# QingzhiWang/LIS-SLAM

Hardware: AMD Instinct MI355X
Metric: scan-to-submap registrations/sec (64x1800 pts, 200k submap) (higher is better)
Workload: dtype f32; 1 GPU; configs[1]: batch=64 synthetic 64x1800 scans vs one shared 200k-pt submap per GPU, semantic mask off, 10 fixed GN iterations, target index build inside the step; batch_per_gpu=64, submap_points=200000, gn_iters=10, parallelism=independent batches x1 + RCCL all-gather of results

## Files before the change

include/lisreg.h:

```cpp
#ifndef LISREG_H_
#define LISREG_H_

#include <stdint.h>

#ifdef __cplusplus
extern "C" {
#endif

#define LISREG_VERSION 1

#define LISREG_OK                        0
#define LISREG_NOT_ENOUGH_FEATURES       1
#define LISREG_TOO_FEW_CORRESPONDENCES   2
#define LISREG_LEAF_TOO_SMALL            3
#define LISREG_ERR_ARG                  -1
#define LISREG_ERR_HIP                  -2
#define LISREG_ERR_NO_TARGET            -3
#define LISREG_ERR_NOMEM                -4
#define LISREG_ERR_COMM                 -5

#define LISREG_FMT_XYZI    0
#define LISREG_FMT_XYZIL   1
#define LISREG_FMT_DEVICE  2
#define LISREG_FMT_DEVICE_XYZI 4
// ... 62 lines not shown
int  lisreg_create(int device, lisreg_ctx** out);
void lisreg_destroy(lisreg_ctx* ctx);
const char* lisreg_last_error(const lisreg_ctx* ctx);
int  lisreg_set_stream(lisreg_ctx* ctx, void* hip_stream);
void* lisreg_get_stream(const lisreg_ctx* ctx);

int  lisreg_default_params(int variant, lisreg_params* p);

int  lisreg_set_target(lisreg_ctx* ctx, const void* corner, int n_corner,
                       const void* surf, int n_surf, int stride_bytes, int fmt);
int  lisreg_set_target_slot(lisreg_ctx* ctx, int slot, const void* corner, int n_corner,
                            const void* surf, int n_surf, int stride_bytes, int fmt);
int  lisreg_target_from_classes(lisreg_ctx* ctx, int slot,
                                const void* pole, int n_pole, const void* ground, int n_ground,
                                const void* building, int n_building, const void* dynamic, int n_dynamic,
                                int stride_bytes, int fmt);

int  lisreg_align(lisreg_ctx* ctx,
                  const void* src_corner, int n_corner, const void* src_surf, int n_surf,
                  int stride_bytes, int fmt,
                  const lisreg_params* params, const lisreg_imu* imu ,
                  float T[6], lisreg_stats* stats );

int  lisreg_align_batch(lisreg_ctx* ctx, int n_items, const lisreg_item* items,
                        const lisreg_params* params, float* T, lisreg_stats* stats);

int  lisreg_batch_prepare(lisreg_ctx* ctx, int n_items, const lisreg_item* items,
                          const lisreg_params* params, const float* T_init);
int  lisreg_batch_run(lisreg_ctx* ctx);
int  lisreg_batch_fetch(lisreg_ctx* ctx, float* T, lisreg_stats* stats);
int  lisreg_stage_host_items(lisreg_ctx* ctx, int n_items, const lisreg_item* items, lisreg_item* items_out);

void* lisreg_batch_result_device(const lisreg_ctx* ctx);

int  lisreg_set_option(lisreg_ctx* ctx, const char* name, int value);
int  lisreg_get_option(const lisreg_ctx* ctx, const char* name, int* value);

int  lisreg_get_counters(lisreg_ctx* ctx, unsigned long long* out, int n);

int  lisreg_get_neighbors(lisreg_ctx* ctx, int* out, int n_elems);

int  lisreg_test_fit_models(lisreg_ctx* ctx, int kind, int n, const float* neighbours, const float* queries,
                            const lisreg_params* params, int exact, float* out);

int  lisreg_get_target_index(lisreg_ctx* ctx, int slot, int kind, int* dims, float* geom,
                             float* sorted_out, int sorted_capacity, int* cell_start_out, int cell_capacity);

int  lisreg_get_target_graph(lisreg_ctx* ctx, int slot, int kind, int* k, float* rows_out, float* meta_out, int capacity_points);

int  lisreg_get_target_cell_rows(lisreg_ctx* ctx, int slot, int kind, int* n_rows, int* k, int* table_out, int capacity_cells,
                                 float* rows_out, float* meta_out, int capacity_rows);

int  lisreg_get_trace(lisreg_ctx* ctx, float* buf, int max_iters);

int  lisreg_set_profiling(lisreg_ctx* ctx, int enable);
int  lisreg_get_timing(lisreg_ctx* ctx, double out[5]);

int  lisreg_voxel_downsample(lisreg_ctx* ctx, const void* in, int n, int stride_bytes, int fmt, float leaf,
                             void* out, int out_capacity, int* n_out);
int  lisreg_voxel_downsample_multi(lisreg_ctx* ctx, int k, const void* const* in, const int* n, const float* leaf, int fmt,
                                   void* const* out, const int* out_capacity, int* n_out);
int  lisreg_transform_cloud(lisreg_ctx* ctx, const void* in, int n, int stride_bytes, int fmt, const float T[6], void* out);

#define LISREG_FMT_XYZIRT  3
typedef struct lisreg_feature_params {
    int   n_scan;
    int   horizon_scan;
    int   downsample_rate;
    float min_range;
    float max_range;
    float edge_threshold;
    float surf_threshold;
} lisreg_feature_params;
typedef struct lisreg_feature_out {
    void* deskewed;      int cap_deskewed,      n_deskewed;
    void* corner;        int cap_corner,        n_corner;
    void* surface;       int cap_surface,       n_surface;
    void* corner_sharp;  int cap_corner_sharp,  n_corner_sharp;
    void* surface_sharp; int cap_surface_sharp, n_surface_sharp;
} lisreg_feature_out;
int  lisreg_extract_features(lisreg_ctx* ctx, const void* cloud, int n, int stride_bytes, int fmt,
                             const lisreg_feature_params* params, lisreg_feature_out* out);
int  lisreg_default_feature_params(lisreg_feature_params* p);
typedef struct lisreg_deskew {
    int    enabled;
    int    imu_pointer_cur;
    const double* imu_time;
    const double* imu_rot_x;
    const double* imu_rot_y;
    const double* imu_rot_z;
    double time_scan_cur;
    const float* time_device;
} lisreg_deskew;
int  lisreg_extract_features_deskew(lisreg_ctx* ctx, const void* cloud, int n, int stride_bytes, int fmt,
                                    const lisreg_feature_params* params, const lisreg_deskew* deskew, lisreg_feature_out* out);

int  lisreg_extract_features_batch(lisreg_ctx* ctx, int n_sweeps, const void* const* sweeps, const int* n,
                                   const lisreg_feature_params* params, lisreg_feature_out* outs);

#define LISREG_FMT_XYZI_PACKED 5
typedef struct lisreg_pretreat_params {
    int    n_scan;
    float  min_range;
    float  max_range;
    double scan_period;
} lisreg_pretreat_params;
// ... 267 lines not shown
```

lis-slam_amd/csrc/lisreg_api.hip:

```cpp
#include "lisreg_ctx.hpp"

#include <dlfcn.h>

#include <algorithm>
#include <chrono>
#include <cmath>
#include <cstdio>
#include <cstdlib>
#include <cstring>
#include <string>
#include <vector>

using namespace lisreg;

namespace lisreg {
thread_local std::string g_static_err;
int ctx_fail(lisreg_ctx* c, int code, const std::string& msg)
{
    if (c) c->err = msg; else g_static_err = msg;
    return code;
}

bool ensure_side_stream(lisreg_ctx* c)
{
// ... 453 lines not shown
        if (n > 0 && !(bb[0] <= bb[3] && bb[1] <= bb[4] && bb[2] <= bb[5]))
            return fail(c, LISREG_ERR_ARG, "set_target: the cloud has no finite point (every coordinate is NaN)");
        memcpy(t.bbox[k], bb, sizeof bb);
        t.grid_margin[k] = (c->search_mode == 5 || (c->search_mode == 4 && t.crow_chosen[k])) ? kCrowGridMargin : 0;
        make_grid(bb, n, &t.g[k], &t.n_cells[k], t.grid_margin[k]);
        prof_mark(c, 2);
        int rc = build_target_kind(c, t, k);
        t.graph_valid[k] = false;
        t.crow_valid[k] = false; t.crow_too_big[k] = false;
        t.g[k].crow = nullptr; t.g[k].crow_meta = nullptr; t.g[k].crow_tab = nullptr;
        if (!rc && c->search_mode == 3) rc = ensure_graph(c, t, k, true);
        if (!rc && c->search_mode == 5) rc = ensure_crows(c, t, k);
        prof_mark(c, -1);
        if (rc) return rc;
    }
    t.valid = true;
    c->grids_dirty = true;
    c->prepared = false;
    return LISREG_OK;
}

int lisreg_set_target_slot(lisreg_ctx* c, int slot, const void* corner, int n_corner, const void* surf, int n_surf,
                           int stride, int fmt)
{
    const void* clouds[2] = { corner, surf };
    const int counts[2] = { n_corner, n_surf };
    return set_target_impl(c, slot, clouds, counts, stride, fmt);
}

int lisreg_set_target(lisreg_ctx* c, const void* corner, int n_corner, const void* surf, int n_surf, int stride, int fmt)
{
    return lisreg_set_target_slot(c, 0, corner, n_corner, surf, n_surf, stride, fmt);
}

int lisreg_target_from_classes(lisreg_ctx* c, int slot, const void* pole, int n_pole, const void* ground, int n_ground,
                               const void* building, int n_building, const void* dynamic, int n_dynamic,
                               int stride, int fmt)
{
    if (!c) return LISREG_ERR_ARG;
    if (fmt == LISREG_FMT_DEVICE) return fail(c, LISREG_ERR_ARG, "target_from_classes: host clouds only");
    if (stride < 12) return fail(c, LISREG_ERR_ARG, "target_from_classes: stride < 12");
    const void* parts[3] = { ground, building, dynamic };
    const int cnt[3] = { std::max(n_ground, 0), std::max(n_building, 0), std::max(n_dynamic, 0) };
    std::vector<unsigned char> surf((size_t)(cnt[0] + cnt[1] + cnt[2]) * (size_t)stride + 1);
    size_t off = 0;
    for (int i = 0; i < 3; ++i) if (cnt[i] > 0 && parts[i]) {
        memcpy(surf.data() + off, parts[i], (size_t)cnt[i] * (size_t)stride);
        off += (size_t)cnt[i] * (size_t)stride;
    }
    return lisreg_set_target_slot(c, slot, pole, pole ? std::max(n_pole, 0) : 0, surf.data(), (int)(off / (size_t)stride), stride, fmt);
}

static bool xcd_order_wanted(const lisreg_ctx* c);

int lisreg_batch_prepare(lisreg_ctx* c, int n_items, const lisreg_item* items, const lisreg_params* params,
                         const float* T_init)
{
    if (!c) return LISREG_ERR_ARG;
    if (n_items < 0 || (n_items > 0 && (!items || !T_init)) || !params) return fail(c, LISREG_ERR_ARG, "batch_prepare: bad arguments");
    HIPCHK(c, hipSetDevice(c->device));
    c->prepared = false;
    c->params = *params;
    c->prm = make_dev_params(*params);
    c->prm.exact = c->exact ? 1 : 0;
    c->prm.ties = (c->canonical_ties || c->exact) ? 1 : 0;
    c->n_items = n_items;
    c->h_blocks.clear(); c->h_segs.clear(); c->h_items.assign((size_t)n_items, ItemState());
    c->batch_slots.clear();
    {
        long long total_src = 0;
        double t_pts = 0;
        std::vector<int> seen;
        for (int i = 0; i < n_items; ++i) {
            total_src += (long long)std::max(items[i].n_corner, 0) + (long long)std::max(items[i].n_surf, 0);
            const int sl = items[i].target;
            if (sl >= 0 && (size_t)sl < c->targets.size() && std::find(seen.begin(), seen.end(), sl) == seen.end()) {
                seen.push_back(sl);
                t_pts += (double)c->targets[(size_t)sl].n[0] + (double)c->targets[(size_t)sl].n[1];
            }
        }
        if (total_src > 2000000000LL) return fail(c, LISREG_ERR_ARG, "batch_prepare: more than 2e9 source points in one batch");
        c->mode_now = c->search_mode;
        if (c->search_mode == 4) {
            const double qi = (double)total_src * (double)c->prm.bound;
            c->mode_now = (t_pts > 0 && qi >= (double)c->graph_min_ratio * t_pts) ? 3 : 1;
            if (t_pts > 0 && qi >= (double)c->cell_min_ratio * t_pts && t_pts * 5120.0 <= (double)c->cell_rows_max_mb * 1048576.0) c->mode_now = 5;
        }
        c->lanes_q = (c->mode_now == 1 && c->lanes_per_query_auto && total_src > 0 && total_src <= 131072) ? 8 : 1;
        if (c->mode_now == 5) {
            bool declined = false;
            long long rows_left = (long long)std::max(c->cell_rows_max_mb, 1) * 1048576LL / (long long)(sizeof(float4) * kGraphK + sizeof(float2));
            for (int sl : seen)
                for (int k = 0; k < 2 && !declined; ++k) {
                    Target& t = c->targets[(size_t)sl];
                    if (!t.valid) continue;
                    const bool had = t.crow_valid[k] && t.g[k].crow_tab;
                    int rc = ensure_crows(c, t, k, c->search_mode == 4, c->search_mode == 4 ? &rows_left : nullptr);
                    if (rc) return rc;
                    if (!had) c->grids_dirty = true;
                    declined = c->search_mode == 4 && t.crow_too_big[k];
                }
            if (declined) {
                c->mode_now = 3;
                for (int sl : seen)
                    for (int k = 0; k < 2; ++k) {
                        Target& t = c->targets[(size_t)sl];
// ... 180 lines not shown
            off += (pt.bytes + 63) & ~(size_t)63;
        }
        HIPCHK(c, hipEventRecord(c->stage_done, c->stream));
    }
    c->sort_now = c->sort_sources == 1;
    if (c->sort_sources == 2 && c->n_elems >= 65536 && c->probe_items == n_items && c->probe_elems == c->n_elems && c->probe_age < 32) {
        ++c->probe_age;
        c->sort_now = c->probe_verdict;
    } else
    if (c->sort_sources == 2 && c->n_elems >= 65536) {
        launch_count_jumps(c->blocks.as<BlockDesc>(), c->n_blocks, c->segs.as<Segment>(), 1.5f, c->done_dev.as<int>(), c->stream);
        int jumps_stack = 0;
        int* jumps = c->done_host.p ? c->done_host.as<int>() : &jumps_stack;
        HIPCHK(c, hipMemcpyAsync(jumps, c->done_dev.p, sizeof(int), hipMemcpyDeviceToHost, c->stream));
        HIPCHK(c, hipStreamSynchronize(c->stream));
        c->sort_now = (double)*jumps > 0.25 * (double)c->n_elems;
        c->probe_verdict = c->sort_now; c->probe_items = n_items; c->probe_elems = c->n_elems; c->probe_age = 0;
    }
    {
        const size_t se = (size_t)std::max(c->rebuild_targets_each_run ? tflat : 1, c->sort_now ? flat : 1);
        const size_t sbk = (size_t)std::max(c->rebuild_targets_each_run ? c->t_buckets : 1, c->sort_now ? c->n_buckets : 1);
        rc = ensure_sort_scratch(c, se, sbk);
        if (rc) return rc;
    }
    launch_reset_items(c->items.as<ItemState>(), c->n_items, c->prm, c->done_dev.as<int>(), c->stream,
                       reinterpret_cast<int*>(c->results.as<float>() + (size_t)std::max(c->n_items, 1) * kResultSize));
    c->items_reset = true; c->reach_miss_seen = 0; c->runs_since_fetch = 0;
    c->reach_ready = false;
    if (c->reach_backoff > 0) --c->reach_backoff;
    else if (c->mode_now == 5 && c->rebuild_targets_each_run && c->row_reach != 0 && c->lanes_q == 1 && c->n_blocks > 0) {
        bool any = false;
        for (int slot : c->batch_slots) for (int k = 0; k < 2; ++k) any = any || (c->targets[(size_t)slot].g[k].qmark != nullptr && c->targets[(size_t)slot].n[k] > 0);
        if (any) {
            launch_query_marks(c->blocks.as<BlockDesc>(), c->n_blocks, c->segs.as<Segment>(), c->grids_dev.as<GridIndex>(), c->items.as<ItemState>(), c->stream);
            for (int slot : c->batch_slots)
                for (int k = 0; k < 2; ++k) {
                    Target& t = c->targets[(size_t)slot];
                    if (!t.g[k].qmark || t.n[k] <= 0) continue;
                    launch_reach_dilate(t.g[k], t.crow_reach[k].as<unsigned>(), c->stream);
                    HIPCHK(c, hipMemsetAsync(t.g[k].qmark, 0, sizeof(unsigned) * (size_t)t.g[k].nx * (size_t)t.g[k].ny * (size_t)t.g[k].qmark_w, c->stream));
                }
            HIPCHK(c, hipGetLastError());
            c->reach_ready = true;
        }
    }
    c->xcd_cached = false;
    if (xcd_order_wanted(c) && !c->sort_now && !c->exact && c->n_blocks > 0) {
        HIPCHK(c, c->xcd_tab.ensure(sizeof(int) * 2 * (size_t)c->n_blocks));
        launch_xcd_order(c->blocks.as<BlockDesc>(), c->n_blocks, c->segs.as<Segment>(), c->grids_dev.as<GridIndex>(), c->items.as<ItemState>(),
                         nullptr, c->batch_slots.size() >= 8 && c->xcd_order == 1, c->xcd_tab.as<int>(), c->xcd_tab.as<int>() + c->n_blocks, c->stream);
        HIPCHK(c, hipGetLastError());
        c->xcd_cached = true;
    }
    c->prepared = true;
    return LISREG_OK;
}

static int exact_pose_caches(lisreg_ctx* c)
{
    const size_t n = (size_t)c->n_items;
    if (n == 0) return LISREG_OK;
    HIPCHK(c, c->exact_trig.ensure(sizeof(float) * 6 * n));
    std::vector<float> T(6 * n), trig(6 * n);
    launch_pose_gather(c->items.as<ItemState>(), c->n_items, c->exact_trig.as<float>(), c->stream);
    HIPCHK(c, hipMemcpyAsync(T.data(), c->exact_trig.p, sizeof(float) * 6 * n, hipMemcpyDeviceToHost, c->stream));
    HIPCHK(c, hipStreamSynchronize(c->stream));
    for (size_t i = 0; i < n; ++i) {
        const float* t = &T[6 * i];
        float* g = &trig[6 * i];
        g[0] = cosf(t[2]); g[1] = sinf(t[2]); g[2] = cosf(t[1]); g[3] = sinf(t[1]); g[4] = cosf(t[0]); g[5] = sinf(t[0]);
    }
    HIPCHK(c, hipMemcpyAsync(c->exact_trig.p, trig.data(), sizeof(float) * 6 * n, hipMemcpyHostToDevice, c->stream));
    launch_pose_cache_from_trig(c->items.as<ItemState>(), c->n_items, c->exact_trig.as<float>(), c->stream);
    HIPCHK(c, hipStreamSynchronize(c->stream));
    return LISREG_OK;
}

constexpr int kWideFrom = 0, kWideFromSmall = 1, kWideUntil = 2, kGraphWideUntil = 1;
constexpr int kGraphHops = 3;

static bool xcd_order_wanted(const lisreg_ctx* c)
{
    const bool many_targets = c->batch_slots.size() >= 8 && c->xcd_order == 1;
    return c->lanes_q != 8 &&
           (((c->mode_now == 3 || c->mode_now == 5) && (c->xcd_order == 1 || (c->xcd_order == 2 && c->n_blocks >= 2048 && c->n_items >= 32))) ||
            (many_targets && c->xcd_order != 0 && c->n_blocks >= 2048));
}

static int run_impl(lisreg_ctx* c, bool early_stop)
{
    if (!c->prepared) return fail(c, LISREG_ERR_ARG, "batch_run: no prepared batch");
    HIPCHK(c, hipSetDevice(c->device));
    hipStream_t st = c->stream;
    const bool many_targets = c->batch_slots.size() >= 8 && c->xcd_order == 1;
    c->xcd_now = xcd_order_wanted(c);
    if (c->xcd_now) HIPCHK(c, c->xcd_tab.ensure(sizeof(int) * 2 * (size_t)c->n_blocks));
    const bool can_stop = early_stop && c->prm.fixed_iters <= 0 && c->done_host.p && c->early_stop_chunk != 0;
    int split_item = 0, split_blk = 0;
    if (c->interleave != 0 && !c->exact && !can_stop && c->lanes_q == 1 && c->n_items >= 2 && c->n_blocks >= c->interleave_min_blocks) {
        ensure_side_stream(c);
        if (c->side_stream && !c->ev_ab && (c->ev_ab.create(hipEventDisableTiming) != hipSuccess ||
                                            c->ev_ba.create(hipEventDisableTiming) != hipSuccess)) { c->ev_ab.reset(); c->ev_ba.reset(); }
        if (c->side_stream) {
            for (int i = 1; i < c->n_items; ++i)
                if (c->h_items[(size_t)i].blk_begin * 2 >= c->n_blocks) { split_item = i; split_blk = c->h_items[(size_t)i].blk_begin; break; }
            if (split_blk * 4 < c->n_blocks || (c->n_blocks - split_blk) * 4 < c->n_blocks) { split_item = 0; split_blk = 0; }
        }
    }
    c->reach_now = c->rebuild_targets_each_run && c->mode_now == 5 && c->reach_ready && !c->exact;
    int* const miss_dev = reinterpret_cast<int*>(c->results.as<float>() + (size_t)std::max(c->n_items, 1) * kResultSize);
    c->prm.reach_miss = c->reach_now ? miss_dev : nullptr;
    const bool reset_done = c->items_reset;
    c->items_reset = false;
    if (c->rebuild_targets_each_run) {
        prof_mark(c, 2);
        if (c->strip_now) {
            StripBuffers sl;
            sl.cnt = c->strip_tab.as<int>(); sl.fill = sl.cnt + (c->t_strips + 1); sl.start = sl.fill + (c->t_strips + 1);
            sl.scan_tmp = sl.start + (c->t_strips + 2);
            sl.tmp_pts = c->tmp_pts.as<float4>(); sl.slot_idx = c->elem_bucket.as<uint32_t>(); sl.slot_pos = c->elem_sub.as<uint32_t>();
            ensure_side_stream(c);
            sl.side = c->side_stream; sl.ev_fork = c->ev_fork; sl.ev_join = c->ev_join;
            if (launch_build_targets_strips(c->tchunk_dev.as<BlockDesc>(), (int)c->h_tchunks.size(), c->tseg_dev.as<TargetSeg>(),
                                            (int)c->h_tsegs.size(), c->t_strips, c->t_max_units, c->t_max_ucells, c->strip_cap, sl, st, &c->strip_zero_ints))
                return fail(c, LISREG_ERR_HIP, "strip index build: LDS configuration refused");
        } else
            launch_build_targets_batched(c->tblk_dev.as<BlockDesc>(), (int)c->h_tblocks.size(), c->tseg_dev.as<TargetSeg>(),
                                         (int)c->h_tsegs.size(), c->t_elems, c->t_buckets, sort_buffers(c), st);
        if (c->mode_now == 3)
            launch_build_graph(c->tblk_dev.as<BlockDesc>(), (int)c->h_tblocks.size(), c->tseg_dev.as<TargetSeg>(),
                               c->grids_dev.as<GridIndex>(), st);
        if (c->mode_now == 5) {
            for (int slot : c->batch_slots) {
                Target& t = c->targets[(size_t)slot];
                const GridIndex g2[2] = { t.g[0], t.g[1] };
                const int nc2[2] = { t.n_cells[0], t.n_cells[1] };
                const lisreg::CrowBuffers cb2[2] = { crow_buffers(t, 0, c->reach_now), crow_buffers(t, 1, c->reach_now) };
                int* oz2[2] = { &t.omask_zero[0], &t.omask_zero[1] };
                launch_crow_rows_pair(g2, nc2, cb2, st, oz2);
            }
        }
        prof_mark(c, -1);
    }
    if (!reset_done) launch_reset_items(c->items.as<ItemState>(), c->n_items, c->prm, c->done_dev.as<int>(), st);
    if (c->exact) { int rc = exact_pose_caches(c); if (rc) return rc; }
    prof_mark(c, 2);
    launch_sort_sources(c->blocks.as<BlockDesc>(), c->n_blocks, c->segs.as<Segment>(), c->n_segs, c->items.as<ItemState>(),
                        c->n_elems, c->sort_now ? c->n_buckets : 0, sort_buffers(c), c->sorted_all.as<float4>(), c->order_all.as<int>(), st);
    prof_mark(c, -1);
    if (c->xcd_now && !(c->xcd_cached && split_blk == 0)) {
        const int nb0 = split_blk ? split_blk : c->n_blocks;
        launch_xcd_order(c->blocks.as<BlockDesc>(), nb0, c->segs.as<Segment>(), c->grids_dev.as<GridIndex>(), c->items.as<ItemState>(),
                         c->sort_now ? c->sorted_all.as<float4>() : nullptr, many_targets, c->xcd_tab.as<int>(), c->xcd_tab.as<int>() + c->n_blocks, st);
        if (split_blk) {
            launch_xcd_order(c->blocks.as<BlockDesc>() + split_blk, c->n_blocks - split_blk, c->segs.as<Segment>(), c->grids_dev.as<GridIndex>(),
                             c->items.as<ItemState>(), c->sort_now ? c->sorted_all.as<float4>() : nullptr, many_targets,
                             c->xcd_tab.as<int>() + split_blk, c->xcd_tab.as<int>() + c->n_blocks + split_blk, st);
            c->xcd_cached = false;
        }
    }
    const int chunk = c->early_stop_chunk > 0 ? c->early_stop_chunk : (c->n_blocks <= 1024 ? 6 : 3);
    int next_check = chunk;
    if (c->early_stop_chunk <= 0 && c->last_launches > 0) next_check = std::max(2, std::min(c->last_launches, chunk));
    c->prm.cell_anchor_until = c->cell_anchor_until;
    auto iteration = [&](int it, int i0, int ni, int b0, int nb, hipStream_t s_, int sidx, hipEvent_t after_assoc) {
        if (!after_assoc) prof_mark(c, 0, sidx);
        (c->exact ? launch_assoc_exact : launch_assoc)(
                     c->blocks.as<BlockDesc>() + b0, nb, c->segs.as<Segment>(), c->grids_dev.as<GridIndex>(),
                     c->items.as<ItemState>(), c->prm, c->sort_now ? c->sorted_all.as<float4>() : nullptr, c->partials.as<double>() + (size_t)b0 * kNumAcc,
                     c->mode_now, c->nn.as<int>(), c->n_elems, c->first_pass_r * c->first_pass_r,
                     c->mode_now != 5 && it >= (c->lanes_q == 8 ? kWideFromSmall : kWideFrom) && it <= (c->mode_now == 3 ? kGraphWideUntil : kWideUntil), kGraphHops,
                     c->count_searches ? c->counters.as<unsigned long long>() : nullptr,
                     c->dump_neighbors ? c->dbg_nn.as<int>() : nullptr, c->lanes_q,
                     c->blocks_q.as<BlockDesc>(), (int)c->h_blocks_q.size(), c->coef.as<float4>(), c->coef_ok.as<int>(),
                     c->xcd_now ? c->xcd_tab.as<int>() + c->n_blocks + b0 : nullptr, s_);
        if (after_assoc) (void)hipEventRecord(after_assoc, s_);
        prof_mark(c, 1, sidx);
        launch_solve(c->items.as<ItemState>() + i0, ni, c->prm, c->partials.as<double>(),
                     c->trace_cap > 0 ? c->trace.as<float>() + (size_t)i0 * (size_t)c->trace_cap * kTraceStride : nullptr, c->trace_cap, c->done_dev.as<int>(), s_);
        prof_mark(c, -1, sidx);
    };
    c->interleaved_now = false;
    if (split_blk > 0 && hipEventRecord(c->ev_fork, st) == hipSuccess && hipStreamWaitEvent(c->side_stream, c->ev_fork, 0) == hipSuccess) {
        c->interleaved_now = true;
        const bool alternate = c->interleave == 1 && c->ev_ab && c->ev_ba;
        hipError_t ie = hipSuccess;
        for (int it = 0; it < c->prm.bound && ie == hipSuccess; ++it) {
            if (alternate && it > 0) ie = hipStreamWaitEvent(st, c->ev_ba, 0);
            if (ie != hipSuccess) break;
            if (alternate) prof_mark(c, 0, 0);
            iteration(it, 0, split_item, 0, split_blk, st, 0, alternate ? c->ev_ab : nullptr);
            if (alternate) ie = hipStreamWaitEvent(c->side_stream, c->ev_ab, 0);
            if (ie != hipSuccess) break;
            if (alternate) prof_mark(c, 0, 1);
            iteration(it, split_item, c->n_items - split_item, split_blk, c->n_blocks - split_blk, c->side_stream, 1, alternate ? c->ev_ba : nullptr);
        }
        if (ie == hipSuccess) ie = hipEventRecord(c->ev_join, c->side_stream);
        if (ie == hipSuccess) ie = hipStreamWaitEvent(st, c->ev_join, 0);
        if (ie != hipSuccess) {
            (void)hipStreamSynchronize(c->side_stream);
            c->interleaved_now = false;
            return lisreg::ctx_fail(c, LISREG_ERR_HIP, std::string("interleaved run: ") + hipGetErrorString(ie));
        }
    } else
    for (int it = 0; it < c->prm.bound; ++it) {
        iteration(it, 0, c->n_items, 0, c->n_blocks, st, 0, nullptr);
        if (c->exact && it + 1 < c->prm.bound) { int rc = exact_pose_caches(c); if (rc) return rc; }
        if (can_stop && it + 1 == next_check && it + 1 < c->prm.bound) {
            HIPCHK(c, hipMemcpyAsync(c->done_host.p, c->done_dev.p, sizeof(int), hipMemcpyDeviceToHost, st));
            HIPCHK(c, hipStreamSynchronize(st));
            if (*c->done_host.as<int>() >= c->n_items) break;
            next_check += c->early_stop_chunk > 0 ? chunk : std::min(chunk, 3);
        }
    }
    launch_finalize(c->items.as<ItemState>(), c->n_items, c->prm, c->results.as<float>(), st, c->done_dev.as<int>());
    c->items_reset = true; ++c->runs_since_fetch;
    HIPCHK(c, hipGetLastError());
    if (c->pack_in_use >= 0 && c->pack_free[c->pack_in_use])
        HIPCHK(c, hipEventRecord(c->pack_free[c->pack_in_use], st));
    return LISREG_OK;
}

int lisreg_batch_run(lisreg_ctx* c)
{
    if (!c) return LISREG_ERR_ARG;
    return run_impl(c, false);
}

int lisreg_batch_fetch(lisreg_ctx* c, float* T, lisreg_stats* stats)
{
    if (!c) return LISREG_ERR_ARG;
    if (!c->prepared) return fail(c, LISREG_ERR_ARG, "batch_fetch: no prepared batch");
    HIPCHK(c, hipSetDevice(c->device));
    const size_t res_floats = ((size_t)std::max(c->n_items, 1) + 1) * kResultSize;
    const size_t trace_floats = c->fetch_trace_records > 0 ? (size_t)kTraceStride * (size_t)c->fetch_trace_records : 0;
    const size_t fetch_bytes = (res_floats + trace_floats) * sizeof(float);
    HIPCHK(c, c->fetch_host.ensure(fetch_bytes, fetch_bytes * 2 + 4096));
    float* fetched = c->fetch_host.as<float>();
    const bool with_miss = c->n_items > 0 && c->reach_now;
    if (c->n_items) HIPCHK(c, hipMemcpyAsync(fetched, c->results.p, sizeof(float) * kResultSize * ((size_t)c->n_items + (with_miss ? 1 : 0)), hipMemcpyDeviceToHost, c->stream));
    if (trace_floats && c->trace.p) HIPCHK(c, hipMemcpyAsync(fetched + res_floats, c->trace.p, sizeof(float) * trace_floats, hipMemcpyDeviceToHost, c->stream));
    HIPCHK(c, hipStreamSynchronize(c->stream));
    c->h_results.assign(fetched, fetched + res_floats);
    if (with_miss) {
        int cum; memcpy(&cum, fetched + (size_t)c->n_items * kResultSize, sizeof cum);
        const int miss = cum - c->reach_miss_seen;
        c->reach_miss_seen = cum;
        c->reach_miss_last = miss;
        if ((long long)miss * 1000LL > (long long)c->n_elems * (long long)std::max(c->prm.bound, 1) * (long long)std::max(c->runs_since_fetch, 1)) { c->reach_ready = false; c->reach_backoff = 32; }
    }
    if (!c->ev.empty()) prof_collect(c);
    c->last_launches = 0;
    for (int i = 0; i < c->n_items; ++i) {
        const float* r = &c->h_results[(size_t)i * kResultSize];
        c->last_launches = std::max(c->last_launches, (int)r[6] + 1);
        if (T) memcpy(T + 6 * (size_t)i, r, 24);
        if (stats) {
            stats[i].iters = (int)r[6]; stats[i].deltaR = r[7]; stats[i].deltaT = r[8];
            stats[i].degenerate = (int)r[9]; stats[i].n_corr_last = (int)r[10]; stats[i].status = (int)r[11];
        }
    }
    c->runs_since_fetch = 0;
    return LISREG_OK;
}

void* lisreg_batch_result_device(const lisreg_ctx* c) { return c ? c->results.p : nullptr; }

int lisreg_set_option(lisreg_ctx* c, const char* name, int value)
{
    if (!c || !name) return LISREG_ERR_ARG;
    if (!strcmp(name, "rebuild_targets_each_run")) {
        c->rebuild_targets_each_run = value != 0;
        if (c->prepared && c->rebuild_targets_each_run) {
            int rc = ensure_sort_scratch(c, (size_t)std::max(c->t_elems, 1), (size_t)std::max(c->t_buckets, 1));
            if (rc) return rc;
        }
        return LISREG_OK;
    }
    if (!strcmp(name, "sort_sources")) { c->sort_sources = value; c->probe_items = -1; return LISREG_OK; }
    if (!strcmp(name, "cell_anchor_until")) { c->cell_anchor_until = std::max(value, 0); return LISREG_OK; }
    if (!strcmp(name, "search_mode")) {
        if (value < 1 || value > 5 || value == 2) return fail(c, LISREG_ERR_ARG, "search_mode: 1 cell walk, 3 k-NN graph scan, 4 auto, 5 cell rows");
        c->search_mode = value; c->prepared = false; return LISREG_OK;
    }
    if (!strcmp(name, "graph_min_ratio")) { c->graph_min_ratio = value; c->prepared = false; return LISREG_OK; }
    if (!strcmp(name, "cell_min_ratio")) { c->cell_min_ratio = value; c->prepared = false; return LISREG_OK; }
    if (!strcmp(name, "row_reach")) { c->row_reach = value; c->reach_backoff = 0; c->prepared = false; return LISREG_OK; }
    if (!strcmp(name, "cell_rows_max_mb")) {
        c->cell_rows_max_mb = value; c->prepared = false;
        for (auto& t : c->targets) for (int k = 0; k < 2; ++k) {
            t.crow_too_big[k] = false;
            if (t.crow_valid[k]) { t.crow_valid[k] = false; c->grids_dirty = true; }
        }
        return LISREG_OK;
    }
    if (!strcmp(name, "early_stop_chunk")) { c->early_stop_chunk = value; return LISREG_OK; }
    if (!strcmp(name, "xcd_order")) { if (value < 0 || value > 2) return fail(c, LISREG_ERR_ARG, "xcd_order: 0 off, 1 on, 2 auto"); c->xcd_order = value; c->xcd_cached = false; return LISREG_OK; }
    if (!strcmp(name, "index_build")) {
        if (value < 0 || value > 2) return fail(c, LISREG_ERR_ARG, "index_build: 0 bucket sort, 1 strip form, 2 auto");
        c->index_build = value; c->prepared = false;
        return LISREG_OK;
    }
    if (!strcmp(name, "index_strip_cells")) { c->strip_cells = std::max(value, 0); c->prepared = false; return LISREG_OK; }
    if (!strcmp(name, "index_strip_cap")) { c->strip_cap = std::min(std::max(value, 64), 16384); c->prepared = false; return LISREG_OK; }
    if (!strcmp(name, "count_searches")) {
        c->count_searches = value != 0;
        if (c->count_searches) { HIPCHK(c, c->counters.ensure(128 * 8)); HIPCHK(c, hipMemset(c->counters.p, 0, 128 * 8)); }
        return LISREG_OK;
    }
    if (!strcmp(name, "lanes_per_query")) { c->lanes_per_query_auto = value != 1; c->prepared = false; return LISREG_OK; }
    if (!strcmp(name, "dump_neighbors")) { c->dump_neighbors = value != 0; c->prepared = false; return LISREG_OK; }
    if (!strcmp(name, "exact_arithmetic")) { c->exact = value != 0; c->prepared = false; return LISREG_OK; }
    if (!strcmp(name, "feeder_copy_engine")) { c->feeder_engine = value; return LISREG_OK; }
    if (!strcmp(name, "canonical_ties")) { c->canonical_ties = value != 0; c->prepared = false; return LISREG_OK; }
    if (!strcmp(name, "first_pass_mm")) {
        if (value < 0) return fail(c, LISREG_ERR_ARG, "first_pass_mm: a radius in millimetres, >= 0");
        c->first_pass_r = 1e-3f * (float)value; return LISREG_OK;
    }
    if (!strcmp(name, "trace_cap")) { c->trace_cap = std::max(0, value); c->prepared = false; return LISREG_OK; }
    if (!strcmp(name, "feeder_threads")) { c->feeder_threads = std::min(std::max(value, 0), 64); return LISREG_OK; }
    if (!strcmp(name, "feeder_numa")) { c->feeder_numa = value != 0; return LISREG_OK; }
    if (!strcmp(name, "interleave_min_blocks")) { c->interleave_min_blocks = std::max(value, 2); return LISREG_OK; }
    if (!strcmp(name, "interleave")) { if (value < 0 || value > 2) return fail(c, LISREG_ERR_ARG, "interleave: 0 off, 1 alternating halves, 2 free-running halves"); c->interleave = value; return LISREG_OK; }
    return fail(c, LISREG_ERR_ARG, std::string("set_option: unknown option ") + name);
}

int lisreg_get_option(const lisreg_ctx* c, const char* name, int* value)
{
    if (!c || !name || !value) return LISREG_ERR_ARG;
    if (!strcmp(name, "search_mode")) { *value = c->search_mode; return LISREG_OK; }
    if (!strcmp(name, "exact_arithmetic")) { *value = c->exact ? 1 : 0; return LISREG_OK; }
    if (!strcmp(name, "feeder_chunks_by_copy_engine")) { *value = c->pack_stolen; return LISREG_OK; }
    if (!strcmp(name, "feeder_chunks")) { *value = c->pack_chunks_n; return LISREG_OK; }
    if (!strcmp(name, "canonical_ties")) { *value = (c->canonical_ties || c->exact) ? 1 : 0; return LISREG_OK; }
    if (!strcmp(name, "index_build")) { *value = c->index_build; return LISREG_OK; }
    if (!strcmp(name, "index_build_now")) { *value = c->strip_now ? 1 : 0; return LISREG_OK; }
    if (!strcmp(name, "front_end")) { *value = c->mode_now; return LISREG_OK; }
    if (!strcmp(name, "lanes_per_query")) { *value = c->lanes_q; return LISREG_OK; }
    if (!strcmp(name, "sort_sources")) { *value = c->sort_sources; return LISREG_OK; }
    if (!strcmp(name, "cell_anchor_until")) { *value = c->cell_anchor_until; return LISREG_OK; }
    if (!strcmp(name, "feeder_threads")) { *value = c->feeder_threads; return LISREG_OK; }
    if (!strcmp(name, "feeder_numa_node")) { *value = c->feeder_node; return LISREG_OK; }
    if (!strcmp(name, "feeder_numa_cpus")) { *value = c->feeder_cpus; return LISREG_OK; }
    if (!strcmp(name, "comm_nranks")) { *value = c->comm ? c->comm_nranks : 0; return LISREG_OK; }
    if (!strcmp(name, "sorted_now")) { *value = c->sort_now ? 1 : 0; return LISREG_OK; }
    if (!strcmp(name, "rebuild_targets_each_run")) { *value = c->rebuild_targets_each_run ? 1 : 0; return LISREG_OK; }
    if (!strcmp(name, "graph_min_ratio")) { *value = c->graph_min_ratio; return LISREG_OK; }
    if (!strcmp(name, "cell_min_ratio")) { *value = c->cell_min_ratio; return LISREG_OK; }
    if (!strcmp(name, "row_reach")) { *value = c->row_reach; return LISREG_OK; }
    if (!strcmp(name, "row_reach_now")) { *value = c->reach_now ? 1 : 0; return LISREG_OK; }
    if (!strcmp(name, "row_reach_misses")) { *value = c->reach_miss_last; return LISREG_OK; }
    if (!strcmp(name, "cell_rows_max_mb")) { *value = c->cell_rows_max_mb; return LISREG_OK; }
    if (!strcmp(name, "xcd_order")) { *value = c->xcd_order; return LISREG_OK; }
    if (!strcmp(name, "xcd_order_now")) { *value = c->xcd_now ? 1 : 0; return LISREG_OK; }
    if (!strcmp(name, "interleave")) { *value = c->interleave; return LISREG_OK; }
    if (!strcmp(name, "interleaved_now")) { *value = c->interleaved_now ? 1 : 0; return LISREG_OK; }
    if (!strcmp(name, "index_kib_front_end_built")) {
        if (c->mode_now != 5) return lisreg_get_option(c, "index_kib_front_end", value);
        unsigned long long fe = 0;
        for (int slot : c->batch_slots) {
            if (slot < 0 || (size_t)slot >= c->targets.size()) continue;
            const lisreg::Target& t = c->targets[(size_t)slot];
            for (int k = 0; k < 2; ++k) {
                if (t.n[k] <= 0 || !t.crow_scan[k].p) continue;
                int rows = 0;
                if (hipSetDevice(c->device) != hipSuccess || hipStreamSynchronize(c->stream) != hipSuccess ||
                    hipMemcpy(&rows, t.crow_scan[k].as<int>() + t.n_cells[k], sizeof(int), hipMemcpyDeviceToHost) != hipSuccess) return LISREG_ERR_HIP;
                rows = std::min(std::max(rows, 0), t.crow_cap[k]);
                fe += (unsigned long long)rows * (sizeof(float4) * lisreg::kGraphK + sizeof(float2)) + (unsigned long long)t.n_cells[k] * sizeof(int);
            }
        }
        *value = (int)std::min<unsigned long long>((fe + 1023) / 1024, 0x7fffffffULL);
        return LISREG_OK;
    }
    if (!strcmp(name, "index_kib_grid") || !strcmp(name, "index_kib_front_end") || !strcmp(name, "index_target_points")) {
        unsigned long long grid = 0, fe = 0, pts = 0;
        for (int slot : c->batch_slots) {
            if (slot < 0 || (size_t)slot >= c->targets.size()) continue;
            const lisreg::Target& t = c->targets[(size_t)slot];
            for (int k = 0; k < 2; ++k) {
                if (t.n[k] <= 0) continue;
                pts += (unsigned long long)t.n[k];
                grid += (unsigned long long)t.n[k] * sizeof(float4) + ((unsigned long long)t.n_cells[k] + 1) * sizeof(int);
                if (c->mode_now == 3) fe += (unsigned long long)t.n[k] * (sizeof(float4) * lisreg::kGraphK + sizeof(float2));
                if (c->mode_now == 5) fe += (unsigned long long)t.crow_cap[k] * (sizeof(float4) * lisreg::kGraphK + sizeof(float2)) +
                                            (unsigned long long)t.n_cells[k] * sizeof(int);
            }
        }
        const unsigned long long v = !strcmp(name, "index_target_points") ? pts : ((!strcmp(name, "index_kib_grid") ? grid : fe) + 1023) / 1024;
        *value = (int)std::min<unsigned long long>(v, 0x7fffffffULL);
        return LISREG_OK;
    }
    return LISREG_ERR_ARG;
}

int lisreg_align_batch(lisreg_ctx* c, int n_items, const lisreg_item* items, const lisreg_params* params, float* T,
                       lisreg_stats* stats)
{
    if (!c) return LISREG_ERR_ARG;
    if (n_items < 0 || (n_items > 0 && (!items || !T)) || !params) return fail(c, LISREG_ERR_ARG, "align_batch: bad arguments");
    const auto t_in = std::chrono::steady_clock::now();
    HIPCHK(c, hipSetDevice(c->device));
    size_t total = 0;
    for (int i = 0; i < n_items; ++i) {
        const lisreg_item& in = items[i];
        if (in.n_corner < 0 || in.n_surf < 0) return fail(c, LISREG_ERR_ARG, "align_batch: negative count");
        if (in.fmt != LISREG_FMT_DEVICE) {
            if (in.stride_bytes < 12 || (in.fmt == LISREG_FMT_XYZIL && in.stride_bytes < 22)) return fail(c, LISREG_ERR_ARG, "align_batch: bad stride");
            if ((in.n_corner > 0 && !in.src_corner) || (in.n_surf > 0 && !in.src_surf)) return fail(c, LISREG_ERR_ARG, "align_batch: NULL cloud");
            total += (size_t)in.n_corner + (size_t)in.n_surf;
        }
    }
    std::vector<lisreg_item> dev_items((size_t)n_items);
    if (total >= 262144 && c->feeder_threads > 0) {
        int rc = lisreg_stage_host_items(c, n_items, items, dev_items.data());
        if (rc) return rc;
        rc = lisreg_batch_prepare(c, n_items, dev_items.data(), params, T);
        if (rc) { (void)hipStreamSynchronize(c->stream); return rc; }
        rc = run_impl(c, true);
        if (rc) { (void)hipStreamSynchronize(c->stream); return rc; }
        return lisreg_batch_fetch(c, T, stats);
    }
    HIPCHK(c, c->src_upload.ensure(sizeof(lisreg_dpoint) * std::max<size_t>(total, 1)));
    size_t raw_bytes = 0;
    for (int i = 0; i < n_items; ++i)
        if (items[i].fmt != LISREG_FMT_DEVICE) raw_bytes += ((size_t)items[i].n_corner + (size_t)items[i].n_surf) * (size_t)items[i].stride_bytes + 32;
    HIPCHK(c, c->raw_upload.ensure(std::max<size_t>(raw_bytes, 16)));
    size_t off = 0, roff = 0;
    for (int i = 0; i < n_items; ++i) {
        dev_items[(size_t)i] = items[i];
        const lisreg_item& in = items[i];
        if (in.fmt == LISREG_FMT_DEVICE) continue;
        lisreg_item& d = dev_items[(size_t)i];
        const void* srcs[2] = { in.src_corner, in.src_surf };
        const int cnts[2] = { in.n_corner, in.n_surf };
        const void** dsts[2] = { &d.src_corner, &d.src_surf };
        for (int k = 0; k < 2; ++k) {
            lisreg_dpoint* dst = c->src_upload.as<lisreg_dpoint>() + off;
            *dsts[k] = dst;
            if (cnts[k] > 0) {
                unsigned char* rdst = static_cast<unsigned char*>(c->raw_upload.p) + roff;
                const size_t bytes = (size_t)cnts[k] * (size_t)in.stride_bytes;
                HIPCHK(c, hipMemcpyAsync(rdst, srcs[k], bytes, hipMemcpyHostToDevice, c->stream));
                launch_pack_cloud(rdst, (size_t)cnts[k], in.stride_bytes, in.fmt == LISREG_FMT_XYZIL, reinterpret_cast<float4*>(dst), c->stream);
                roff += (bytes + 15) & ~(size_t)15;
// ... 13 lines not shown
    if (rc) { (void)hipStreamSynchronize(c->stream); return rc; }
    const auto t2 = now();
    rc = lisreg_batch_fetch(c, T, stats);
    if (host_prof) {
        auto us = [](auto a, auto b) { return std::chrono::duration<double, std::micro>(b - a).count(); };
        fprintf(stderr, "[lisreg host] upload %.1f us, prepare %.1f us, enqueue %.1f us, fetch (incl. GPU wait) %.1f us\n",
                us(t_in, t0), us(t0, t1), us(t1, t2), us(t2, now()));
    }
    return rc;
}

int lisreg_align(lisreg_ctx* c, const void* src_corner, int n_corner, const void* src_surf, int n_surf, int stride,
                 int fmt, const lisreg_params* params, const lisreg_imu* imu, float T[6], lisreg_stats* stats)
{
    if (!c) return LISREG_ERR_ARG;
    if (!params || !T) return fail(c, LISREG_ERR_ARG, "align: params/T NULL");
    if (c->targets.empty() || !c->targets[0].valid) return fail(c, LISREG_ERR_NO_TARGET, "align: call lisreg_set_target first");
    lisreg_item item;
    memset(&item, 0, sizeof item);
    item.src_corner = src_corner; item.n_corner = n_corner;
    item.src_surf = src_surf; item.n_surf = n_surf;
    item.stride_bytes = stride; item.fmt = fmt; item.target = 0;
    item.degenerate_in = c->degenerate;
    if (imu) item.imu = *imu;
    const int bound = params->fixed_iters > 0 ? params->fixed_iters : params->max_iters;
    const int saved_cap = c->trace_cap;
    c->trace_cap = std::max(bound, 1);
    lisreg_stats st;
    memset(&st, 0, sizeof st);
    c->fetch_trace_records = c->trace_cap;
    int rc = lisreg_align_batch(c, 1, &item, params, T, &st);
    c->fetch_trace_records = 0;
    if (rc == LISREG_OK) {
        c->degenerate = st.degenerate;
        c->last_trace_n = std::min(bound, st.iters + 1);
        if (st.status == LISREG_NOT_ENOUGH_FEATURES) c->last_trace_n = 0;
        c->last_trace.assign((size_t)kTraceStride * (size_t)std::max(c->last_trace_n, 1), 0.f);
        if (c->last_trace_n > 0 && c->fetch_host.p)
            memcpy(c->last_trace.data(), c->fetch_host.as<float>() + 2 * (size_t)kResultSize, sizeof(float) * kTraceStride * (size_t)c->last_trace_n);
        if (stats) *stats = st;
        rc = st.status;
    }
    c->trace_cap = saved_cap;
    c->prepared = false;
    return rc;
}

int lisreg_get_trace(lisreg_ctx* c, float* buf, int max_iters)
{
    if (!c || !buf || max_iters <= 0) return 0;
    const int n = std::min(max_iters, c->last_trace_n);
    if (n > 0) memcpy(buf, c->last_trace.data(), sizeof(float) * kTraceStride * (size_t)n);
    return n;
}

int lisreg_get_counters(lisreg_ctx* c, unsigned long long* out, int n)
{
    if (!c || !out || n < 0) return LISREG_ERR_ARG;
    for (int i = 0; i < n; ++i) out[i] = 0;
    if (!c->counters.p) return LISREG_OK;
    HIPCHK(c, hipStreamSynchronize(c->stream));
    HIPCHK(c, hipMemcpy(out, c->counters.p, sizeof(unsigned long long) * (size_t)std::min(n, 128), hipMemcpyDeviceToHost));
    if (c->mode_now == 3 || c->mode_now == 5) {
        unsigned long long tmp[64] = { 0 };
        for (int i = 0; i < 32 && 2 * i + 1 < n; ++i) { tmp[2 * i] = out[i] >> 32; tmp[2 * i + 1] = out[i] & 0xffffffffull; }
        for (int i = 0; i < std::min(n, 64); ++i) out[i] = tmp[i];
    }
    return LISREG_OK;
}

int lisreg_get_target_index(lisreg_ctx* c, int slot, int kind, int* dims , float* geom ,
                            float* sorted_out, int sorted_capacity, int* cell_start_out, int cell_capacity)
{
    if (!c || slot < 0 || (size_t)slot >= c->targets.size() || kind < 0 || kind > 1 || !c->targets[(size_t)slot].valid)
        return fail(c, LISREG_ERR_ARG, "get_target_index: no such target");
    const Target& t = c->targets[(size_t)slot];
    const GridIndex& g = t.g[kind];
    if (dims) { dims[0] = t.n[kind]; dims[1] = g.nx; dims[2] = g.ny; dims[3] = g.nz; dims[4] = t.n_cells[kind]; }
    if (geom) { geom[0] = g.ox; geom[1] = g.oy; geom[2] = g.oz; geom[3] = g.cell; }
    HIPCHK(c, hipStreamSynchronize(c->stream));
    if (sorted_out) {
        if (sorted_capacity < t.n[kind]) return fail(c, LISREG_ERR_ARG, "get_target_index: sorted_capacity too small");
        if (t.n[kind] > 0) HIPCHK(c, hipMemcpy(sorted_out, t.sorted[kind].p, sizeof(float4) * (size_t)t.n[kind], hipMemcpyDeviceToHost));
    }
    if (cell_start_out) {
        if (cell_capacity < t.n_cells[kind] + 1) return fail(c, LISREG_ERR_ARG, "get_target_index: cell_capacity too small");
        HIPCHK(c, hipMemcpy(cell_start_out, t.cell_start[kind].p, sizeof(int) * ((size_t)t.n_cells[kind] + 1), hipMemcpyDeviceToHost));
    }
    return LISREG_OK;
}

int lisreg_get_target_graph(lisreg_ctx* c, int slot, int kind, int* k_out, float* rows_out, float* meta_out, int capacity_points)
{
    if (!c || slot < 0 || (size_t)slot >= c->targets.size() || kind < 0 || kind > 1 || !c->targets[(size_t)slot].valid)
        return fail(c, LISREG_ERR_ARG, "get_target_graph: no such target");
    Target& t = c->targets[(size_t)slot];
    if (k_out) *k_out = kGraphK;
    if (!rows_out && !meta_out) return LISREG_OK;
    if (capacity_points < t.n[kind]) return fail(c, LISREG_ERR_ARG, "get_target_graph: capacity_points too small");
    HIPCHK(c, hipSetDevice(c->device));
    if (!t.graph_valid[kind] || !t.g[kind].nbr) {
        int rc = ensure_graph(c, t, kind, true);
        if (rc) return rc;
        c->grids_dirty = true;
    }
    HIPCHK(c, hipStreamSynchronize(c->stream));
// ... 716 lines not shown
```

lis-slam_amd/csrc/lisreg_assoc.hip:

```cpp
#include "lisreg_internal.hpp"

#ifndef LISREG_EXACT
#define LISREG_EXACT 0
#endif
#if LISREG_EXACT
#define LISREG_ASSOC_NS exact_arith
#define LISREG_LAUNCH_ASSOC launch_assoc_exact
#define LISREG_LAUNCH_TEST_FIT launch_test_fit_exact
#else
#define LISREG_ASSOC_NS fast_arith
#define LISREG_LAUNCH_ASSOC launch_assoc
#define LISREG_LAUNCH_TEST_FIT launch_test_fit
#endif

namespace lisreg {

namespace {
namespace LISREG_ASSOC_NS {

constexpr bool kExactArith = LISREG_EXACT != 0;
constexpr int kRedWaveFloats = 1024;
__device__ __forceinline__ float fdiv(float a, float b) { return kExactArith ? a / b : a * __builtin_amdgcn_rcpf(b); }
__device__ __forceinline__ float fsqrt(float x) { return kExactArith ? sqrtf(x) : __builtin_amdgcn_sqrtf(x); }
__device__ __forceinline__ float fdiv5(float a) { return kExactArith ? a / 5.f : a * 0.2f; }

__device__ __forceinline__ float hypot_f(float a, float b)
{
    a = fabsf(a); b = fabsf(b);
    if (kExactArith) {
        if (a > b) { b /= a; return a * sqrtf(1.f + b * b); }
        if (b > 0.f) { a /= b; return b * sqrtf(1.f + a * a); }
        return 0.f;
    }
    const float mx = fmaxf(a, b), mn = fminf(a, b);
    const float r = mn * __builtin_amdgcn_rcpf(mx);
    return mx > 0.f ? mx * __builtin_amdgcn_sqrtf(1.f + r * r) : 0.f;
}

#define LISREG_ROT(v0, v1) do { const float a0_ = (v0), b0_ = (v1); (v0) = a0_ * c - b0_ * s; (v1) = a0_ * s + b0_ * c; } while (0)
#define LISREG_JACOBI_CST(p, y) \
        float t = fabsf(y) + hypot_f((p), (y)); \
        float s = hypot_f((p), t); \
        const float c = fdiv(t, s); \
        s = fdiv((p), s); t = fdiv((p), t) * (p); \
        if ((y) < 0.f) { s = -s; t = -t; }

__device__ __forceinline__ void eigen_sym3(float a11, float a12, float a13, float a22, float a23, float a33,
                                           float& l0, float& l1, float v0[3])
{
    float w0 = a11, w1 = a22, w2 = a33;
    float v00 = 1, v01 = 0, v02 = 0, v10 = 0, v11 = 1, v12 = 0, v20 = 0, v21 = 0, v22 = 1;
    if (kExactArith) {
        int indR0 = fabsf(a12) < fabsf(a13) ? 2 : 1;
        int indC2 = fabsf(a13) < fabsf(a23) ? 1 : 0;
#pragma unroll 1
        for (int it = 0; it < 270; ++it) {
            int k = 0, l = indR0;
            float mv = fabsf(indR0 == 1 ? a12 : a13);
            { const float v = fabsf(a23); if (mv < v) { mv = v; k = 1; l = 2; } }
            { const float v = fabsf(a12); if (mv < v) { mv = v; k = 0; l = 1; } }
            { const float v = fabsf(indC2 == 0 ? a13 : a23); if (mv < v) { mv = v; k = indC2; l = 2; } }
            if (k == 0 && l == 1) {
                const float p = a12;
                if (fabsf(p) <= 1.1920929e-7f) break;
                const float y = (w1 - w0) * 0.5f;
// ... 769 lines not shown
                const float thr_ = __builtin_amdgcn_sqrtf(b4) * 1.0001f + da_; thr2_ = thr_ * thr_; \
                if (l3_ > thr2_) stop_ = true; \
            } else { \
                LISREG_LIST_INIT(); \
                const float thr_ = __builtin_amdgcn_sqrtf(b4) * 1.0001f + da_; thr2_ = thr_ * thr_; \
                if (cnt_ > 0) LISREG_GRAPH_GROUP(r0_, r1_, r2_, r3_, LISREG_TRY_ND); \
            } \
            _Pragma("unroll 1") for (int g_ = 1; !stop_ && 4 * g_ < cnt_; ++g_) { \
                const v4f e0g_ = R_[4 * g_], e1g_ = R_[4 * g_ + 1], e2g_ = R_[4 * g_ + 2], e3g_ = R_[4 * g_ + 3]; \
                LISREG_GRAPH_GROUP(e0g_, e1g_, e2g_, e3g_, LISREG_TRY_ND); \
            } \
            if (!stop_) stop_ = rho2_ > thr2_;                  \
            certified = stop_; } while (0)

#define LISREG_CE5(a, b) do { const bool sw_ = sd[b] < sd[a]; const float ta_ = sd[a]; const int ia_ = sid[a]; \
                              sd[a] = sw_ ? sd[b] : ta_; sd[b] = sw_ ? ta_ : sd[b]; sid[a] = sw_ ? sid[b] : ia_; sid[b] = sw_ ? ia_ : sid[b]; } while (0)

#define LISREG_CANON_INSERT(d2_, o_, j_) do { \
        const bool c3_ = (d2_) < b3 || ((d2_) == b3 && (o_) < o3), c2_ = (d2_) < b2 || ((d2_) == b2 && (o_) < o2); \
        const bool c1_ = (d2_) < b1 || ((d2_) == b1 && (o_) < o1), c0_ = (d2_) < b0 || ((d2_) == b0 && (o_) < o0); \
        b4 = c3_ ? b3 : (d2_);               i4 = c3_ ? i3 : (j_);               o4 = c3_ ? o3 : (o_); \
        b3 = c3_ ? (c2_ ? b2 : (d2_)) : b3;  i3 = c3_ ? (c2_ ? i2 : (j_)) : i3;  o3 = c3_ ? (c2_ ? o2 : (o_)) : o3; \
        b2 = c2_ ? (c1_ ? b1 : (d2_)) : b2;  i2 = c2_ ? (c1_ ? i1 : (j_)) : i2;  o2 = c2_ ? (c1_ ? o1 : (o_)) : o2; \
        b1 = c1_ ? (c0_ ? b0 : (d2_)) : b1;  i1 = c1_ ? (c0_ ? i0 : (j_)) : i1;  o1 = c1_ ? (c0_ ? o0 : (o_)) : o1; \
        b0 = c0_ ? (d2_) : b0;               i0 = c0_ ? (j_) : i0;               o0 = c0_ ? (o_) : o0; } while (0)
#define LISREG_CANONICAL_FIVE() do { if (kTies) { \
         \
        if (kQ > 1) { _Pragma("unroll") for (int d_ = 1; d_ < kQ; d_ <<= 1) { const int o_ = __shfl_xor((int)tie, d_); tie = (int)tie | (int)(o_ != 0); } } \
        LISREG_LIST_TIES(); \
        if (tie && i4 >= 0) { \
            const float lim_ = b4; \
            const float rad_ = __builtin_amdgcn_sqrtf(lim_) * 1.0001f + kEps; \
            const int cx0_ = max(grid_coord(qx - rad_, g.ox, g.inv_cell), 0), cx1_ = min(grid_coord(qx + rad_, g.ox, g.inv_cell), g.nx - 1); \
            const int cy0_ = max(grid_coord(qy - rad_, g.oy, g.inv_cell), 0), cy1_ = min(grid_coord(qy + rad_, g.oy, g.inv_cell), g.ny - 1); \
            const int cz0_ = max(grid_coord(qz - rad_, g.oz, g.inv_cell), 0), cz1_ = min(grid_coord(qz + rad_, g.oz, g.inv_cell), g.nz - 1); \
            b0 = b1 = b2 = b3 = b4 = 3.0e38f; i0 = i1 = i2 = i3 = i4 = -1; \
            int o0 = 0x7fffffff, o1 = 0x7fffffff, o2 = 0x7fffffff, o3 = 0x7fffffff, o4 = 0x7fffffff; \
            if (cz0_ <= cz1_) \
            _Pragma("unroll 1") for (int ix_ = cx0_; ix_ <= cx1_; ++ix_) \
            _Pragma("unroll 1") for (int iy_ = cy0_; iy_ <= cy1_; ++iy_) { \
                const int base_ = (ix_ * g.ny + iy_) * g.nz; \
                const int js_ = cells[base_ + cz0_], je_ = cells[base_ + cz1_ + 1]; \
                _Pragma("unroll 1") for (int j_ = js_; j_ < je_; ++j_) { \
                    const v4f c_ = pts[j_]; \
                    const float ax_ = qx - c_.x, ay_ = qy - c_.y, az_ = qz - c_.z; \
                    const float e_ = ax_ * ax_ + ay_ * ay_ + az_ * az_; \
                    const int o_ = __float_as_int(c_.w); \
                    if (e_ <= lim_ && (e_ < b4 || (e_ == b4 && o_ < o4))) LISREG_CANON_INSERT(e_, o_, j_); \
                } \
            } \
            (void)o4; \
        } } } while (0)

template <bool kWide, int kGraph, int kQ, bool kTies, bool kShare = false>
__global__ __launch_bounds__(kBlockQ) __attribute__((amdgpu_waves_per_eu(kShare ? 4 : 8, kShare ? 4 : 8))) void k_assoc_walk(const BlockDesc* __restrict__ blocks,
                                                        const Segment* __restrict__ segs,
                                                        const GridIndex* __restrict__ grids,
                                                        const ItemState* __restrict__ items, const DevParams P,
                                                        const float4* __restrict__ sorted_all,
                                                        int* __restrict__ nn_, int n_elems, float first_pass_r2,
                                                        int graph_hops, unsigned long long* __restrict__ counters,
                                                        int* __restrict__ dbg_nn, float4* __restrict__ coef, int* __restrict__ coef_ok,
                                                        double* __restrict__ partials, const int* __restrict__ xcd_order)
{
    __shared__ __attribute__((aligned(16))) int2 s_runs_w[kBlockQ / 64][kWalkCap][64];
    static_assert(sizeof(int2) * kWalkCap * 64 == sizeof(float) * kRedWaveFloats, "one region per wavefront");
    float* s_red = reinterpret_cast<float*>(&s_runs_w[0][0][0]);
#define s_runs_at(r_, t_) s_runs_w[(t_) >> 6][(r_)][(t_) & 63]
    constexpr float kEps = 1e-3f;

    const int tid = threadIdx.x;
    int bid = blockIdx.x;
    if (xcd_order) {
        const int m = gridDim.x >> 3, t = gridDim.x & 7, x = blockIdx.x & 7;
        bid = xcd_order[x * m + min(x, t) + (int)(blockIdx.x >> 3)];
    }
    const BlockDesc bd = blocks[bid];
    const ItemState* it = &items[bd.item];
    if (it->done) return;
    const Segment sg = segs[bd.seg];
    const GridIndex g = grids[sg.target];
    double* out = partials + (size_t)bid * kNumAcc;
    if (g.n < 5) {
        if (kQ == 1 && tid < kNumAcc) out[tid] = 0.0;
        return;
    }
    const gptr_f4 pts = (gptr_f4)g.pts;
    const gptr_i32 cells = (gptr_i32)g.cell_start;
    const gptr_i32w nn = (gptr_i32w)nn_;
    const gptr_i4w nn4 = (gptr_i4w)nn_;
    const float* M = it->M;

    const int sub_q = tid & (kQ - 1); (void)sub_q;
    const bool valid = tid / kQ < bd.count;
    const int qflat = sg.flat_base + bd.start + tid / kQ;
    const float4* qsrc = sorted_all ? sorted_all : (const float4*)((uintptr_t)sg.src - (uintptr_t)sg.flat_base * sizeof(float4));
    float4 q0 = make_float4(0.f, 0.f, 0.f, 0.f);
    if (valid) q0 = qsrc[qflat];
    float qx = M[0] * q0.x + M[1] * q0.y + M[2] * q0.z + M[3];
    float qy = M[4] * q0.x + M[5] * q0.y + M[6] * q0.z + M[7];
    float qz = M[8] * q0.x + M[9] * q0.y + M[10] * q0.z + M[11];

    float b0, b1, b2, b3, b4;
    int   i0, i1, i2, i3, i4;
    bool  tie = false;
#define LISREG_LIST_INIT() do { b0 = b1 = b2 = b3 = b4 = P.tau; i0 = i1 = i2 = i3 = i4 = -1; } while (0)
    if (kGraph) {
        bool need_walk = valid, scanned = false;
        if (kGraph == 2) {
            int row_ = -1;
            float mx_ = 0.f, my_ = 0.f, mz_ = 0.f;
            if (valid && g.crow_tab) {
                const float tx = (qx - g.ox) * g.inv_cell, ty = (qy - g.oy) * g.inv_cell, tz = (qz - g.oz) * g.inv_cell;
                const int gx = (int)floorf(tx), gy = (int)floorf(ty), gz = (int)floorf(tz);
                const int hx = min(max(gx, 0), g.nx - 1), hy = min(max(gy, 0), g.ny - 1), hz = min(max(gz, 0), g.nz - 1);
                const int v = ((gptr_i32)g.crow_tab)[(hx * g.ny + hy) * g.nz + hz];
                if (P.reach_miss) {
                    const unsigned long long mm = __ballot(v == -1);
                    if (mm != 0ull && (int)(__ffsll((long long)mm) - 1) == (tid & 63)) atomicAdd(P.reach_miss, __popcll(mm));
                }
                if (v >= 0) {
                    float fx = 0.5f, fy = 0.5f, fz = 0.5f;
                    row_ = v >> 8;
                    {
                        const bool ux = tx - (float)hx >= 0.5f, uy = ty - (float)hy >= 0.5f, uz = tz - (float)hz >= 0.5f;
// ... 263 lines not shown
#pragma unroll
        for (int u = 0; u < kU; ++u) if (k[u] >= 0) atomicAdd(&s_cnt[k[u]], 1);
    }
    __syncthreads();
    const int lane = tid & 63, wave = tid >> 6;
    const int mine = s_cnt[tid];
    int v = mine;
#pragma unroll
    for (int d = 1; d < 64; d <<= 1) { const int o = __shfl_up(v, d); if (lane >= d) v += o; }
    if (lane == 63) s_tmp[wave] = v;
    __syncthreads();
    if (tid < 16) {
        int w = s_tmp[tid];
#pragma unroll
        for (int d = 1; d < 16; d <<= 1) { const int o = __shfl_up(w, d); if (tid >= d) w += o; }
        s_tmp[16 + tid] = w - s_tmp[tid];
    }
    __syncthreads();
    v += s_tmp[16 + wave];
    s_cnt[tid] = v - mine;
    __syncthreads();
    for (int base = 0; base < n_blocks; base += kU * 1024) {
        int k[kU];
#pragma unroll
        for (int u = 0; u < kU; ++u) { const int b = base + u * 1024 + tid; k[u] = b < n_blocks ? keys[b] : -1; }
#pragma unroll
        for (int u = 0; u < kU; ++u) {
            if (k[u] < 0) continue;
            const int r = atomicAdd(&s_cnt[k[u]], 1);
            order[r] = base + u * 1024 + tid;
        }
    }
}

#endif

}

#if !LISREG_EXACT
void launch_xcd_order(const BlockDesc* blocks, int n_blocks, const Segment* segs, const GridIndex* grids, const ItemState* items,
                      const float4* sorted_all, bool by_target, int* keys, int* order, hipStream_t st)
{
    if (n_blocks <= 0) return;
    k_xcd_keys<<<(n_blocks + 255) / 256, 256, 0, st>>>(blocks, n_blocks, segs, grids, items, sorted_all, by_target ? 1 : 0, keys);
    k_xcd_order<<<1, 1024, 0, st>>>(n_blocks, keys, order);
}
#endif

template <bool kTies>
static void launch_assoc_impl(const BlockDesc* blocks, int n_blocks, const Segment* segs, const GridIndex* grids,
                              const ItemState* items, DevParams prm, const float4* sorted_all, double* partials,
                              int mode, int* nn, int n_elems, float first_pass_r2, bool wide, int graph_hops,
                              unsigned long long* counters, int* dbg_nn, int lanes_q,
                              const BlockDesc* blocks_q, int n_blocks_q, float4* coef, int* coef_ok, const int* xcd_order, hipStream_t st)
{
    using namespace LISREG_ASSOC_NS;
    if (mode == 1 && lanes_q == 8) {
        const bool share = n_blocks_q <= 2048;
        if (wide && share)
            k_assoc_walk<true, 0, 8, kTies, true><<<n_blocks_q, kBlockQ, 0, st>>>(blocks_q, segs, grids, items, prm, sorted_all, nn, n_elems,
                                                                                      first_pass_r2, graph_hops, counters, dbg_nn, coef, coef_ok, partials, nullptr);
        else if (share)
            k_assoc_walk<false, 0, 8, kTies, true><<<n_blocks_q, kBlockQ, 0, st>>>(blocks_q, segs, grids, items, prm, sorted_all, nn, n_elems,
                                                                                       first_pass_r2, graph_hops, counters, dbg_nn, coef, coef_ok, partials, nullptr);
        else if (wide)
            k_assoc_walk<true, 0, 8, kTies><<<n_blocks_q, kBlockQ, 0, st>>>(blocks_q, segs, grids, items, prm, sorted_all, nn, n_elems,
                                                                                first_pass_r2, graph_hops, counters, dbg_nn, coef, coef_ok, partials, nullptr);
        else
            k_assoc_walk<false, 0, 8, kTies><<<n_blocks_q, kBlockQ, 0, st>>>(blocks_q, segs, grids, items, prm, sorted_all, nn, n_elems,
                                                                                 first_pass_r2, graph_hops, counters, dbg_nn, coef, coef_ok, partials, nullptr);
        k_rows_reduce<<<n_blocks, kBlockQ, 0, st>>>(blocks, segs, grids, items, prm, sorted_all, coef, coef_ok, partials);
        return;
    }
    if (mode == 1) {
        if (wide)
            k_assoc_walk<true, 0, 1, kTies><<<n_blocks, kBlockQ, 0, st>>>(blocks, segs, grids, items, prm, sorted_all, nn, n_elems,
                                                                              first_pass_r2, graph_hops, counters, dbg_nn, coef, coef_ok, partials, xcd_order);
        else
            k_assoc_walk<false, 0, 1, kTies><<<n_blocks, kBlockQ, 0, st>>>(blocks, segs, grids, items, prm, sorted_all, nn, n_elems,
                                                                               first_pass_r2, graph_hops, counters, dbg_nn, coef, coef_ok, partials, xcd_order);
    } else if (mode == 5) {
        k_assoc_walk<false, 2, 1, kTies><<<n_blocks, kBlockQ, 0, st>>>(blocks, segs, grids, items, prm, sorted_all, nn, n_elems,
                                                                       first_pass_r2, graph_hops, counters, dbg_nn, coef, coef_ok, partials, xcd_order);
    } else {
        if (wide)
            k_assoc_walk<true, 1, 1, kTies><<<n_blocks, kBlockQ, 0, st>>>(blocks, segs, grids, items, prm, sorted_all, nn, n_elems,
                                                                          first_pass_r2, graph_hops, counters, dbg_nn, coef, coef_ok, partials, xcd_order);
        else
            k_assoc_walk<false, 1, 1, kTies><<<n_blocks, kBlockQ, 0, st>>>(blocks, segs, grids, items, prm, sorted_all, nn, n_elems,
                                                                           first_pass_r2, graph_hops, counters, dbg_nn, coef, coef_ok, partials, xcd_order);
    }
}

void LISREG_LAUNCH_TEST_FIT(int kind, int n, const float* nb15, const float* q3, DevParams prm, float* out, hipStream_t st)
{
    using namespace LISREG_ASSOC_NS;
    if (n > 0) k_test_fit_models<<<(n + 63) / 64, 64, 0, st>>>(kind, n, nb15, q3, prm, out);
}

void LISREG_LAUNCH_ASSOC(const BlockDesc* blocks, int n_blocks, const Segment* segs, const GridIndex* grids,
                         const ItemState* items, DevParams prm, const float4* sorted_all, double* partials,
                         int mode, int* nn, int n_elems, float first_pass_r2, bool wide, int graph_hops,
                         unsigned long long* counters, int* dbg_nn, int lanes_q,
                         const BlockDesc* blocks_q, int n_blocks_q, float4* coef, int* coef_ok, const int* xcd_order, hipStream_t st)
{
    if (n_blocks <= 0) return;
#if LISREG_EXACT
    launch_assoc_impl<true>(blocks, n_blocks, segs, grids, items, prm, sorted_all, partials, mode, nn, n_elems, first_pass_r2, wide, graph_hops,
                            counters, dbg_nn, lanes_q, blocks_q, n_blocks_q, coef, coef_ok, xcd_order, st);
#else
    if (prm.ties)
        launch_assoc_impl<true>(blocks, n_blocks, segs, grids, items, prm, sorted_all, partials, mode, nn, n_elems, first_pass_r2, wide, graph_hops,
                                counters, dbg_nn, lanes_q, blocks_q, n_blocks_q, coef, coef_ok, xcd_order, st);
    else
        launch_assoc_impl<false>(blocks, n_blocks, segs, grids, items, prm, sorted_all, partials, mode, nn, n_elems, first_pass_r2, wide, graph_hops,
                                 counters, dbg_nn, lanes_q, blocks_q, n_blocks_q, coef, coef_ok, xcd_order, st);
#endif
}

}
```

lis-slam_amd/csrc/lisreg_ctx.hpp:

```cpp
#pragma once
#include <algorithm>
#include "lisreg_internal.hpp"

#include <atomic>
#include <map>
#include <memory>
#include <string>
#include <vector>

namespace lisreg {

template <hipError_t (*Free)(void*)>
struct OwnedMem {
    void*  p = nullptr;
    size_t cap = 0;
    OwnedMem() = default;
    OwnedMem(const OwnedMem&) = delete;
    OwnedMem& operator=(const OwnedMem&) = delete;
    OwnedMem(OwnedMem&& o) noexcept : p(o.p), cap(o.cap) { o.p = nullptr; o.cap = 0; }
    OwnedMem& operator=(OwnedMem&& o) noexcept { if (this != &o) { release(); p = o.p; cap = o.cap; o.p = nullptr; o.cap = 0; } return *this; }
    ~OwnedMem() { release(); }
    void release() { if (p) (void)Free(p); p = nullptr; cap = 0; }
    template <class T> T* as() const { return reinterpret_cast<T*>(p); }
};
// ... 74 lines not shown
};

struct LocalMap {
    bool   valid = false;
    DevBuf cls[5];
    int    n[5] = { 0, 0, 0, 0, 0 };
    DevBuf tgt[2];
    int    n_tgt[2] = { 0, 0 };
    int    feature_point_num = 0;
    double bound[6] = { 0, 0, 0, 0, 0, 0 };
};

struct KeyframeRing {
    bool valid = false;
    bool payload_is_label = false;
    struct Frame { DevBuf cloud[2]; int n[2] = { 0, 0 }; };
    std::vector<Frame> frames;
    DevBuf cat[2], tgt[2];
    int    n_tgt[2] = { 0, 0 };
    bool   built = false;
    float  built_leaf[2] = { 0.f, 0.f };
    int    built_slot = -1;
    unsigned long long built_gen = 0;
};

struct PackPool;
struct LoopDet;
struct PackPoolDelete { void operator()(PackPool* p) const; };
struct LoopDetDelete { void operator()(LoopDet* p) const; };
struct PackChunk { const unsigned char* src; lisreg_dpoint* dst; int n, stride, fmt; int pinned; };

struct RcclApi {
    void* handle = nullptr;
    int (*GetUniqueId)(void*) = nullptr;
    int (*CommInitRank)(void**, int, const void* , int) = nullptr;
    int (*AllGather)(const void*, void*, size_t, int, void*, hipStream_t) = nullptr;
    int (*CommDestroy)(void*) = nullptr;
};

}

struct lisreg_ctx {
    int          device = 0;
    lisreg::Stream own_stream;
    hipStream_t  stream = nullptr;
    std::string  err;
    std::vector<lisreg::Target> targets;
    unsigned long long   target_gen = 0;
    lisreg::DevBuf       grids_dev;
    bool         grids_dirty = true;
    lisreg::PinnedBuf grids_host;
    lisreg::Event grids_done;
    lisreg::DevBuf hist, bucket_start, scan_tmp, elem_bucket, elem_sub, tmp_bucket, tmp_sub, tmp_idx, tmp_pts, bbox_dev, bbox_scratch;
    lisreg::DevBuf blocks, segs, items, sorted_all, order_all, partials, results, trace, src_upload, raw_upload, dbg_nn, blocks_q, coef, coef_ok, nn, counters, tseg_dev, tblk_dev, tchunk_dev, strip_tab, done_dev, xcd_tab,
           vox_in, vox_lab, vox_order, vox_sidx, vox_head, vox_slot, vox_start, vox_out, vox_outlab, vox_M,
           ft_owner, ft_flag, ft_pos, ft_scan, ft_col, ft_range, ft_src, ft_curv, ft_picked, ft_label, ft_rlists, ft_rcounts,
           ft_lists, ft_counts, ft_rings, ft_gather, ft_cat, ft_bounds, ft_dsk_tab, ft_dsk_pts, ft_dsk_misc, ft_dsk_time;
    lisreg::DevBuf pt_ends, pt_ring, pt_ori, pt_blk, pt_hdr, pt_tab, pt_in, pt_out, pt_time;
    lisreg::PinnedBuf pt_hdr_host;
    lisreg::DevBuf rn_keys, rn_blk, rn_hdr, rn_tab, rn_in, rn_img;
    lisreg::PinnedBuf rn_hdr_host;
    bool         rn_keys_clean = false;
    std::unique_ptr<lisreg::PackPool, lisreg::PackPoolDelete> pack_pool;
    int          feeder_threads = 8;
    lisreg::PinnedBuf pack_host[2];
    lisreg::DevBuf pack_dev[2];
    int            feeder_engine = 1;
    int            pack_stolen = 0, pack_chunks_n = 0;
    lisreg::DevBuf pack_raw[2];
    lisreg::PinnedBuf up_host;
    lisreg::Event pack_copied[2];
    lisreg::Event pack_free[2];
    hipEvent_t   pack_pending = nullptr;
    lisreg::Event pack_raw_done;
    int          pack_flip = 0, pack_last = -1, pack_in_use = -1;
    lisreg::Stream copy_stream;
    lisreg::Stream pack_stream;
    lisreg::Event pack_kernels_done;
    std::vector<lisreg::PackChunk> pack_chunks;
    std::vector<std::atomic<int>> pack_done;
    std::map<int, lisreg::MapIndex> maps;
    std::vector<lisreg::LocalMap> localmaps;
    std::vector<lisreg::KeyframeRing> keyrings;
    lisreg::DevBuf lm_in, lm_tmp, lm_bbox, exact_trig;
    lisreg::DevBuf map_stage;
    lisreg::DevBuf mp_pts, mp_flag, mp_pos, mp_idx, mp_cnt, mp_d2, mp_out, icp_state, icp_partials, icp_cur, icp_items, map_tab, map_tsegs, map_tblocks;
    lisreg::PinnedBuf done_host;
    lisreg::PinnedBuf stage_host;
    lisreg::Event stage_done;
    lisreg::PinnedBuf fetch_host;
    int       early_stop_chunk = -1;
    int       fetch_trace_records = 0;
    std::vector<lisreg::TargetSeg> h_tsegs;
    std::vector<lisreg::BlockDesc> h_tblocks;
    std::vector<lisreg::BlockDesc> h_tchunks;
    int       t_strips = 0, t_max_units = 0, t_max_ucells = 0;
    int       index_build = 2;
    int       strip_cells = 0, strip_cap = 2048;
    bool      strip_now = false;
    int         row_reach = 1;
    bool        reach_ready = false;
    bool        xcd_cached = false;
    int         reach_backoff = 0;
    int         strip_zero_ints = 0;
    bool        items_reset = false;
    int         reach_miss_seen = 0, runs_since_fetch = 0;
    int         reach_miss_last = 0;
    bool        reach_now = false;
    lisreg::Stream side_stream;
    lisreg::Event ev_fork, ev_join;
    lisreg::Event ev_ab, ev_ba;
    int       t_elems = 0, t_buckets = 0;
    bool      count_searches = false;
    bool      dump_neighbors = false;
    int       search_mode = 4;
    int       mode_now = 1;
    int       lanes_q = 1;
    bool      lanes_per_query_auto = true;
    int       cell_min_ratio = 110;
    int       cell_rows_max_mb = 16384;
    int       graph_min_ratio = 60;
    int       interleave = 0;
    bool      interleaved_now = false;
    int       interleave_min_blocks = 8192;
    int       xcd_order = 2;
    bool      xcd_now = false;
    int       feeder_numa = 1;
    int       feeder_node = -1, feeder_cpus = 0;
    int       cell_anchor_until = 1;
    bool      canonical_ties = false;
    bool      exact = false;
    int       sort_sources = 2;
    bool      sort_now = false;
    int       probe_items = -1, probe_elems = -1, probe_age = 0; bool probe_verdict = false;
    float     first_pass_r = 0.45f;
    int       last_launches = 0;
    std::vector<lisreg::BlockDesc> h_blocks;
    std::vector<lisreg::BlockDesc> h_blocks_q;
    std::vector<lisreg::Segment>   h_segs;
    std::vector<lisreg::ItemState> h_items;
    std::vector<float>     h_results;
    int       n_items = 0, n_blocks = 0, n_segs = 0, n_elems = 0, n_buckets = 0, trace_cap = 0;
    lisreg::DevParams prm;
    lisreg_params params;
    bool      prepared = false;
    bool      rebuild_targets_each_run = false;
    std::vector<int> batch_slots;
    int       degenerate = 0;
    bool      profiling = false;
    std::vector<lisreg::Event> ev;
    std::vector<int>        ev_kind;
    std::vector<int>        ev_sidx;
    double    timing[5] = { 0, 0, 0, 0, 0 };
    std::vector<float> last_trace;
    int       last_trace_n = 0;
    lisreg::RcclApi   rccl;
    void*     comm = nullptr;
    int       comm_nranks = 0;
    std::unique_ptr<lisreg::LoopDet, lisreg::LoopDetDelete> loopdet;
};

namespace lisreg {
void feeder_stop(lisreg_ctx* c);
int  ctx_fail(lisreg_ctx* c, int code, const std::string& msg);
bool ensure_side_stream(lisreg_ctx* c);
void pack_cloud(const void* cloud, int n, int stride, int fmt, lisreg_dpoint* out);
constexpr int kPackIntensity = 0x100;
int  upload_records(lisreg_ctx* c, const void* cloud, int n, int stride_bytes, int fmt, void* dev_out);
void make_grid(const float bb[6], int n, GridIndex* g, int* n_cells, int margin_cells = 0);
SortBuffers sort_buffers(lisreg_ctx* c);
int  ensure_sort_scratch(lisreg_ctx* c, size_t n_elems, size_t n_buckets);
void ctx_prof_mark(lisreg_ctx* c, int kind_of_next_interval);
void ctx_prof_collect(lisreg_ctx* c);
}

#define HIPCHK(c, expr) do { hipError_t e_ = (expr); if (e_ != hipSuccess) \
// ... 2 lines not shown
```

lis-slam_amd/csrc/lisreg_internal.hpp:

```cpp
#pragma once
#include <hip/hip_runtime.h>
#include <stdint.h>
#include "../../include/lisreg.h"

namespace lisreg {

constexpr int kBlockQ     = 256;
constexpr int kNumAcc     = 28;
constexpr int kResultSize = 12;
constexpr int kTraceStride = LISREG_TRACE_STRIDE;
constexpr int kGraphK     = 64;

struct GridIndex {
    const float4* pts;
    const int*    cell_start;
    int   n;
    float ox, oy, oz;
    float cell, inv_cell;
    int   nx, ny, nz;
    const float4* nbr;
    const float2* nbr_meta;
    const float4* crow;
    const float2* crow_meta;
    const int*    crow_tab;
// ... 83 lines not shown
    int       k;
    int       off[kVoxelMultiMax + 1];
    int       bucket_base[kVoxelMultiMax + 1];
    uint32_t  idx_base[kVoxelMultiMax + 1];
    VoxelDesc d[kVoxelMultiMax];
};

struct SortBuffers {
    int*      hist;
    int*      bucket_start;
    int*      scan_tmp;
    uint32_t* elem_bucket;
    uint32_t* elem_sub;
    uint32_t* tmp_bucket;
    uint32_t* tmp_sub;
    int*      tmp_idx;
    float4*   tmp_pts;
};

void launch_bbox(const float4* pts, int n, float* bbox6, float* scratch , hipStream_t st);
void launch_build_target(const float4* pts, int n, GridIndex g, float4* sorted_out, int* cell_start_out,
                         int n_cells, SortBuffers sb, hipStream_t st);
void launch_build_targets_batched(const BlockDesc* blocks, int n_blocks, const TargetSeg* tsegs, int n_tsegs,
                                  int n_elems, int n_buckets, SortBuffers sb, hipStream_t st);
constexpr int    kPartChunkHost = 4096;
constexpr int    kMaxStrips     = 8192;
constexpr size_t kStripLdsLarge = 150 * 1024;
struct StripBuffers {
    int*      cnt;
    int*      fill;
    int*      start;
    int*      scan_tmp;
    float4*   tmp_pts;
    uint32_t* slot_idx;
    uint32_t* slot_pos;
    hipStream_t side;
    hipEvent_t  ev_fork, ev_join;
};
int  launch_build_targets_strips(const BlockDesc* chunks, int n_chunks, const TargetSeg* tsegs, int n_tsegs, int n_strips, int max_units,
                                 int max_strip_cells, int cap_small, StripBuffers sb, hipStream_t st, int* zero_ints_known = nullptr);
void launch_build_graph(const BlockDesc* blocks, int n_blocks, const TargetSeg* tsegs, const GridIndex* grids, hipStream_t st);
void launch_build_graph_one(GridIndex g, hipStream_t st);
struct CrowBuffers { int* need; int* omask; int* scan; int* scan_tmp; int cap_rows;
                     const unsigned* reach = nullptr; };
void launch_query_marks(const BlockDesc* blocks, int n_blocks, const Segment* segs, const GridIndex* grids, const ItemState* items, hipStream_t st);
void launch_reach_dilate(GridIndex g, unsigned* reach, hipStream_t st);
void launch_crow_classify(GridIndex g, int n_cells, CrowBuffers cb, hipStream_t st, int* omask_zero_cells = nullptr);
void launch_crow_build(GridIndex g, int n_cells, CrowBuffers cb, hipStream_t st, int* omask_zero_cells = nullptr);
void launch_crow_rows_pair(const GridIndex g[2], const int n_cells[2], const CrowBuffers cb[2], hipStream_t st, int* omask_zero_cells[2]);
void launch_sort_sources(const BlockDesc* blocks, int n_blocks, const Segment* segs, int n_segs,
                         const ItemState* items, int n_elems, int n_buckets, SortBuffers sb, float4* sorted_all, int* order_all,
                         hipStream_t st);
void launch_reset_items(ItemState* items, int n_items, DevParams prm, int* done_counter, hipStream_t st, int* zero_too = nullptr);
void launch_assoc(const BlockDesc* blocks, int n_blocks, const Segment* segs, const GridIndex* grids,
                  const ItemState* items, DevParams prm, const float4* sorted_all, double* partials,
                  int mode ,
                  int* nn, int n_elems, float first_pass_r2,
                  bool wide ,
                  int graph_hops ,
                  unsigned long long* counters ,
                  int* dbg_nn ,
                  int lanes_q ,
                  const BlockDesc* blocks_q, int n_blocks_q ,
                  float4* coef, int* coef_ok ,
                  const int* xcd_order , hipStream_t st);
void launch_assoc_exact(const BlockDesc* blocks, int n_blocks, const Segment* segs, const GridIndex* grids,
                        const ItemState* items, DevParams prm, const float4* sorted_all, double* partials,
                        int mode, int* nn, int n_elems, float first_pass_r2, bool wide, int graph_hops,
                        unsigned long long* counters, int* dbg_nn, int lanes_q, const BlockDesc* blocks_q, int n_blocks_q,
                        float4* coef, int* coef_ok, const int* xcd_order, hipStream_t st);
void launch_test_fit(int kind, int n, const float* nb15, const float* q3, DevParams prm, float* out, hipStream_t st);
void launch_test_fit_exact(int kind, int n, const float* nb15, const float* q3, DevParams prm, float* out, hipStream_t st);
void launch_xcd_order(const BlockDesc* blocks, int n_blocks, const Segment* segs, const GridIndex* grids, const ItemState* items,
                      const float4* sorted_all, bool by_target, int* keys, int* order, hipStream_t st);
void launch_pose_gather(const ItemState* items, int n_items, float* T_out, hipStream_t st);
void launch_pose_cache_from_trig(ItemState* items, int n_items, const float* trig, hipStream_t st);
void launch_solve(ItemState* items, int n_items, DevParams prm, const double* partials, float* trace,
                  int trace_cap, int* done_counter, hipStream_t st);
void launch_finalize(ItemState* items, int n_items, DevParams prm, float* results, hipStream_t st, int* reset_done_counter = nullptr);

void launch_voxel_sort(const float4* pts, int n, VoxelDesc d, int n_buckets, SortBuffers sb, int* order, uint32_t* sidx,
                       int* head, int* slot , hipStream_t st);
struct VoxelHandOut { int k; int vo[kVoxelMultiMax + 1]; float4* out[kVoxelMultiMax]; };
void launch_bbox_multi(const float4* cat, const VoxelMulti& m, float* bbox_out , float* scratch , hipStream_t st);
struct BboxJobs { int k; int n[kVoxelMultiMax]; const float4* pts[kVoxelMultiMax]; };
void launch_bbox_jobs(const BboxJobs& j, float* bbox_out , float* scratch , hipStream_t st);
struct CloudRef { const float4* pts; int n; int pad_; };
void launch_bbox_refs(const CloudRef* refs_dev, int k, float* bbox_out , float* scratch , hipStream_t st);
void launch_concat_jobs(const BboxJobs& j, const VoxelMulti& m, float4* cat, hipStream_t st);
void launch_multi_bounds(const int* slot, const VoxelMulti& m, int* out , hipStream_t st);
void launch_hand_out(const float4* src, const VoxelHandOut& h, hipStream_t st);
void launch_voxel_sort_multi(const float4* pts, int n, const VoxelMulti& m, int n_buckets, SortBuffers sb, int* order, uint32_t* sidx,
                             int* head, int* slot, hipStream_t st);
void launch_voxel_centroids(int n, int n_vox, const float4* pts, const uint32_t* labels, int w_mode, const int* order,
                            const int* head, const int* slot, int* vstart , float4* out_pts,
                            uint32_t* out_labels , hipStream_t st);
void launch_pack_cloud(const void* raw_dev, size_t n, int stride, int has_label, float4* out, hipStream_t st);
void launch_transform_cloud(const float4* in, int n, const float* M12_dev, float4* out, hipStream_t st);
struct Mat12 { float m[12]; };
void launch_transform_cloud_m(const float4* in, int n, const float M12_host[12], float4* out, hipStream_t st);
void launch_count_jumps(const BlockDesc* blocks, int n_blocks, const Segment* segs, float thr, int* jumps, hipStream_t st);
void launch_exclusive_scan(const int* in, int* out, int* tmp, int n, hipStream_t st);

struct FeatureBuffers {
    int*   owner;
    int*   flag;
    int*   pos;
    int*   scan_tmp;
    int*   col;
    float* range;
    int*   src;
    float* curv;
    int*   picked;
    int*   label;
    int*   ring_lists;
    int*   ring_counts;
    int*   lists;
    int*   counts;
};
void launch_extract_features(const float4* pts, const uint32_t* rings , int n,
                             lisreg_feature_params P, FeatureBuffers fb, hipStream_t st, int n_sweeps = 1);
void launch_feature_batch_rows(const float4* cat, int n, const int* offsets , int n_sweeps, int H, int rate,
                               uint32_t* rows, hipStream_t st);
// ... 51 lines not shown
```

lis-slam_amd/csrc/lisreg_solve.hip:

```cpp
#include "lisreg_internal.hpp"

namespace lisreg {

namespace {

__device__ float hyp(float a, float b)
{
    a = fabsf(a); b = fabsf(b);
    if (a > b) { b /= a; return a * sqrtf(1.f + b * b); }
    if (b > 0.f) { a /= b; return b * sqrtf(1.f + a * a); }
    return 0.f;
}

__device__ void eigen_sym6(float* A, float* W, float* V, int* indR, int* indC)
{
    const int n = 6;
    for (int i = 0; i < n; ++i) for (int j = 0; j < n; ++j) V[i * n + j] = (i == j) ? 1.f : 0.f;
    for (int k = 0; k < n; ++k) {
        W[k] = A[k * n + k];
        if (k < n - 1) {
            int m = k + 1; float mv = fabsf(A[k * n + m]);
            for (int i = k + 2; i < n; ++i) { float v = fabsf(A[k * n + i]); if (mv < v) { mv = v; m = i; } }
            indR[k] = m;
        }
        if (k > 0) {
            int m = 0; float mv = fabsf(A[k]);
            for (int i = 1; i < k; ++i) { float v = fabsf(A[i * n + k]); if (mv < v) { mv = v; m = i; } }
            indC[k] = m;
        }
    }
    for (int it = 0; it < n * n * 30; ++it) {
        int k = 0, l; float mv = fabsf(A[indR[0]]);
        for (int i = 1; i < n - 1; ++i) { float v = fabsf(A[i * n + indR[i]]); if (mv < v) { mv = v; k = i; } }
        l = indR[k];
        for (int i = 1; i < n; ++i) { float v = fabsf(A[indC[i] * n + i]); if (mv < v) { mv = v; k = indC[i]; l = i; } }
        const float p = A[k * n + l];
        if (fabsf(p) <= 1.1920929e-7f) break;
        const float y = (W[l] - W[k]) * 0.5f;
        float t = fabsf(y) + hyp(p, y);
        float s = hyp(p, t);
        const float c = t / s;
        s = p / s; t = (p / t) * p;
        if (y < 0.f) { s = -s; t = -t; }
        A[k * n + l] = 0.f;
        W[k] -= t; W[l] += t;
#define LR(v0, v1) do { const float a0_ = (v0), b0_ = (v1); (v0) = a0_ * c - b0_ * s; (v1) = a0_ * s + b0_ * c; } while (0)
        for (int i = 0; i < k; ++i)      LR(A[i * n + k], A[i * n + l]);
        for (int i = k + 1; i < l; ++i)  LR(A[k * n + i], A[i * n + l]);
        for (int i = l + 1; i < n; ++i)  LR(A[k * n + i], A[l * n + i]);
        for (int i = 0; i < n; ++i)      LR(V[k * n + i], V[l * n + i]);
#undef LR
        for (int j = 0; j < 2; ++j) {
            const int idx = j == 0 ? k : l;
            if (idx < n - 1) {
                int m = idx + 1; float mv2 = fabsf(A[idx * n + m]);
                for (int i = idx + 2; i < n; ++i) { float v = fabsf(A[idx * n + i]); if (mv2 < v) { mv2 = v; m = i; } }
                indR[idx] = m;
            }
            if (idx > 0) {
                int m = 0; float mv2 = fabsf(A[idx]);
                for (int i = 1; i < idx; ++i) { float v = fabsf(A[i * n + idx]); if (mv2 < v) { mv2 = v; m = i; } }
                indC[idx] = m;
            }
        }
    }
    for (int k = 0; k < n - 1; ++k) {
        int m = k;
        for (int i = k + 1; i < n; ++i) if (W[m] < W[i]) m = i;
        if (m != k) {
            float tw = W[m]; W[m] = W[k]; W[k] = tw;
            for (int i = 0; i < n; ++i) { float tv = V[m * n + i]; V[m * n + i] = V[k * n + i]; V[k * n + i] = tv; }
        }
    }
}

__device__ __forceinline__ float lane_value(float v, int l) { return __int_as_float(__builtin_amdgcn_readlane(__float_as_int(v), l)); }
__device__ __forceinline__ bool solve6_qr_lanes(float a[6], int lane, float x[6])
{
#pragma unroll
    for (int k = 0; k < 6; ++k) {
        const float c0 = a[k];
        float tail = 0.f;
#pragma unroll
        for (int i = k + 1; i < 6; ++i) tail += a[i] * a[i];
        float beta, tau, v[6];
        if (tail <= 1.17549435e-38f) {
            tau = 0.f; beta = c0;
#pragma unroll
            for (int i = 0; i < 6; ++i) v[i] = 0.f;
        } else {
            beta = sqrtf(c0 * c0 + tail);
            if (c0 >= 0.f) beta = -beta;
#pragma unroll
            for (int i = 0; i < 6; ++i) v[i] = (i > k) ? a[i] / (c0 - beta) : 0.f;
            tau = (beta - c0) / beta;
        }
        if (lane == k) a[k] = beta;
        tau = lane_value(tau, k);
#pragma unroll
        for (int i = k + 1; i < 6; ++i) v[i] = lane_value(v[i], k);
        if (tau != 0.f && lane > k) {
            float dot = a[k];
#pragma unroll
            for (int i = k + 1; i < 6; ++i) dot += v[i] * a[i];
            dot *= tau;
            a[k] -= dot;
#pragma unroll
            for (int i = k + 1; i < 6; ++i) a[i] -= dot * v[i];
        }
    }
    float R[6][6], c[6];
#pragma unroll
    for (int i = 0; i < 6; ++i) {
        c[i] = lane_value(a[i], 6);
#pragma unroll
        for (int j = i; j < 6; ++j) R[i][j] = lane_value(a[i], j);
    }
    bool singular = false;
#pragma unroll
    for (int i = 0; i < 6; ++i) singular = singular || (fabsf(R[i][i]) <= 1.17549435e-38f);
    float y[6];
#pragma unroll
    for (int i = 5; i >= 0; --i) {
        float s_ = c[i];
#pragma unroll
        for (int j = i + 1; j < 6; ++j) s_ -= R[i][j] * y[j];
        y[i] = s_ / R[i][i];
    }
#pragma unroll
    for (int i = 0; i < 6; ++i) x[i] = singular ? 0.f : y[i];
    return !singular;
}

__device__ void inv6_lu(float* A, float* B)
{
    const int N = 6;
    for (int i = 0; i < N; ++i) for (int j = 0; j < N; ++j) B[i * N + j] = (i == j) ? 1.f : 0.f;
    for (int i = 0; i < N; ++i) {
        int k = i;
        for (int j = i + 1; j < N; ++j) if (fabsf(A[j * N + i]) > fabsf(A[k * N + i])) k = j;
        if (fabsf(A[k * N + i]) < 1.1920929e-7f * 100) { for (int j = 0; j < N * N; ++j) B[j] = 0.f; return; }
        if (k != i) for (int j = 0; j < N; ++j) {
            float t = A[i * N + j]; A[i * N + j] = A[k * N + j]; A[k * N + j] = t;
            t = B[i * N + j]; B[i * N + j] = B[k * N + j]; B[k * N + j] = t;
        }
        const float d = -1.f / A[i * N + i];
        for (int j = i + 1; j < N; ++j) {
            const float alpha = A[j * N + i] * d;
            for (int m = i + 1; m < N; ++m) A[j * N + m] += alpha * A[i * N + m];
            for (int m = 0; m < N; ++m) B[j * N + m] += alpha * B[i * N + m];
        }
    }
    for (int i = N - 1; i >= 0; --i)
        for (int j = 0; j < N; ++j) {
            float s = B[i * N + j];
            for (int k = i + 1; k < N; ++k) s -= A[i * N + k] * B[k * N + j];
            B[i * N + j] = s / A[i * N + i];
        }
}

__device__ void write_pose_cache(ItemState* it, const float* trig = nullptr)
{
    const float* T = it->T;
    float A, B, C, D, E, F;
    if (trig) { A = trig[0]; B = trig[1]; C = trig[2]; D = trig[3]; E = trig[4]; F = trig[5]; }
    else { A = cosf(T[2]); B = sinf(T[2]); C = cosf(T[1]); D = sinf(T[1]); E = cosf(T[0]); F = sinf(T[0]); }
    const float DE = D * E, DF = D * F;
    float* M = it->M;
    M[0] = A * C;  M[1] = A * DF - B * E;  M[2]  = B * F + A * DE;  M[3]  = T[3];
    M[4] = B * C;  M[5] = A * E + B * DF;  M[6]  = B * DE - A * F;  M[7]  = T[4];
    M[8] = -D;     M[9] = C * F;           M[10] = C * E;           M[11] = T[5];
    it->sc[0] = D; it->sc[1] = C;
    it->sc[2] = B; it->sc[3] = A;
    it->sc[4] = F; it->sc[5] = E;
    const float srx = D, crx = C, sry = B, cry = A, srz = F, crz = E;
    float* K = it->jk;
    K[0] = crx * sry * srz;  K[1] = crx * crz * sry;  K[2] = srx * sry;
    K[3] = -srx * srz;       K[4] = crz * srx;        K[5] = crx;
    K[6] = crx * cry * srz;  K[7] = crx * cry * crz;  K[8] = cry * srx;
    K[9] = cry * srx * srz - crz * sry;    K[10] = sry * srz + cry * crz * srx;   K[11] = crx * cry;
    K[12] = -cry * crz - srx * sry * srz;  K[13] = cry * srz - crz * srx * sry;   K[14] = crx * sry;
    K[15] = crz * srx * sry - cry * srz;   K[16] = crx * crz;                      K[17] = crx * srz;
    K[18] = crz * sry - cry * srx * srz;   K[19] = 0.f;                            K[20] = 0.f;
}

__device__ __forceinline__ void reset_item(ItemState* it, const DevParams& P)
{
    for (int k = 0; k < 6; ++k) it->T[k] = it->T_init[k];
    for (int k = 0; k < 36; ++k) it->P[k] = 0.f;
    const bool guard_ok = (it->n_sc > P.edge_min) && (it->n_ss > P.surf_min);
    it->iter = 0;
    it->guard_failed = guard_ok ? 0 : 1;
    it->done = guard_ok ? 0 : 1;
    it->iters_out = 0;
    it->deltaR = 100.f; it->deltaT = 100.f;
    it->degenerate = it->degenerate_in;
    it->n_corr = 0;
    it->any_solved = 0;
    write_pose_cache(it);
}

__global__ __launch_bounds__(64) void k_reset_items(ItemState* __restrict__ items, int n_items, const DevParams P,
                                                    int* __restrict__ done_counter, int* __restrict__ zero_too)
{
    const int i = blockIdx.x * 64 + threadIdx.x;
    if (i == 0) { *done_counter = P.n_guard_failed; if (zero_too) *zero_too = 0; }
    if (i >= n_items) return;
    reset_item(&items[i], P);
}

constexpr int kSolveThreads = 512;

__global__ __launch_bounds__(kSolveThreads) void k_solve(ItemState* __restrict__ items, const DevParams P,
                                                         const double* __restrict__ partials,
                                                         float* __restrict__ trace, int trace_cap,
                                                         int* __restrict__ done_counter)
{
    __shared__ float s_AtA[36], s_AtB[6], s_X[6], s_A[36];
    __shared__ float s_E[6], s_V[36], s_V2[36], s_Vi[36];
    __shared__ int   s_ind[12];
    __shared__ double s_part[kSolveThreads / 32][32];
    __shared__ double s_sum[kNumAcc];
    __shared__ double s_L[36];

    ItemState* it = &items[blockIdx.x];
    if (it->done) return;
    {
        const int col = threadIdx.x & 31, grp = threadIdx.x >> 5;
        double s = 0.0;
        if (col < kNumAcc) {
            const double* p = partials + (size_t)it->blk_begin * kNumAcc + col;
            const int nb = it->blk_count;
            constexpr int kG = kSolveThreads / 32;
            for (int b = grp; b < nb; b += 32 * kG) {
                double v[32];
#pragma unroll
                for (int u = 0; u < 32; ++u) v[u] = (b + u * kG < nb) ? p[(size_t)(b + u * kG) * kNumAcc] : 0.0;
#pragma unroll
                for (int u = 0; u < 32; ++u) s += v[u];
            }
        }
        s_part[grp][col] = s;
    }
    __syncthreads();
    if (threadIdx.x < kNumAcc) {
        double s = 0.0;
#pragma unroll
        for (int g = 0; g < kSolveThreads / 32; ++g) s += s_part[g][threadIdx.x];
        s_sum[threadIdx.x] = s;
    }
    __syncthreads();
    if (threadIdx.x >= 64) return;
    const int lane = threadIdx.x;
    const bool l0 = lane == 0;

    const int iter = it->iter;
    const int n_sel = (int)(s_sum[27] + 0.5);
    float* tr = (trace && iter < trace_cap) ? trace + ((size_t)blockIdx.x * trace_cap + iter) * kTraceStride : nullptr;
    if (l0) {
        it->n_corr = n_sel;
        if (tr) {
            for (int k = 0; k < kTraceStride; ++k) tr[k] = 0.f;
            tr[0] = (float)n_sel;
            for (int k = 0; k < 6; ++k) tr[49 + k] = it->T[k];
        }
    }
    bool finished = false;
    if (n_sel >= P.min_corr) {
        if (lane < 36) {
            const int r_ = lane / 6, c_ = lane % 6, lo = min(r_, c_), hi = max(r_, c_);
            s_AtA[lane] = (float)s_sum[lo * 6 - (lo * (lo - 1)) / 2 + (hi - lo)];
        } else if (lane < 42) s_AtB[lane - 36] = (float)s_sum[21 + lane - 36];
        __builtin_amdgcn_fence(__ATOMIC_RELEASE, "wavefront");
        __builtin_amdgcn_wave_barrier();
        __builtin_amdgcn_fence(__ATOMIC_ACQUIRE, "wavefront");
        {
            float a[6], xs[6];
#pragma unroll
            for (int i = 0; i < 6; ++i) a[i] = lane < 6 ? s_AtA[i * 6 + lane] : (lane == 6 ? s_AtB[i] : 0.f);
            solve6_qr_lanes(a, lane, xs);
            if (l0) {
#pragma unroll
                for (int i = 0; i < 6; ++i) s_X[i] = xs[i];
            }
        }
        int isDeg = 0;
        float Tn[6] = { 0.f, 0.f, 0.f, 0.f, 0.f, 0.f };
        if (l0) {
            isDeg = it->degenerate;
            bool well_conditioned = false;
            if (iter == 0) {
                double* L = s_L;
                double trace = 0.0;
                for (int i = 0; i < 6; ++i) trace += (double)s_AtA[i * 6 + i];
                const double shift = (double)P.eig_thresh + 2e-5 * trace;
                well_conditioned = trace > 0.0;
                for (int r = 0; r < 6 && well_conditioned; ++r)
                    for (int c = 0; c <= r; ++c) {
                        double v = (double)s_AtA[r * 6 + c] - (r == c ? shift : 0.0);
                        for (int k = 0; k < c; ++k) v -= L[r * 6 + k] * L[c * 6 + k];
                        if (r == c) { if (!(v > 0.0)) { well_conditioned = false; break; } L[r * 6 + r] = sqrt(v); }
                        else L[r * 6 + c] = v / L[c * 6 + c];
                    }
            }
            if (iter == 0 && well_conditioned) {
                isDeg = 0;
                for (int i = 0; i < 36; ++i) it->P[i] = (i % 7 == 0) ? 1.f : 0.f;
            } else if (iter == 0) {
                for (int i = 0; i < 36; ++i) s_A[i] = s_AtA[i];
                eigen_sym6(s_A, s_E, s_V, s_ind, s_ind + 6);
                for (int i = 0; i < 36; ++i) s_V2[i] = s_V[i];
                isDeg = 0;
                for (int i = 5; i >= 0; --i) {
                    if (s_E[i] < P.eig_thresh) { for (int j = 0; j < 6; ++j) s_V2[i * 6 + j] = 0.f; isDeg = 1; }
                    else break;
                }
                for (int i = 0; i < 36; ++i) s_A[i] = s_V[i];
                inv6_lu(s_A, s_Vi);
                for (int r = 0; r < 6; ++r) for (int c = 0; c < 6; ++c) {
                    double s = 0; for (int m = 0; m < 6; ++m) s += (double)s_Vi[r * 6 + m] * (double)s_V2[m * 6 + c];
                    it->P[r * 6 + c] = (float)s;
                }
            } else if (P.emulate_shadow) {
                for (int i = 0; i < 36; ++i) it->P[i] = 0.f;
            }
            if (isDeg) {
                float X2[6];
                for (int r = 0; r < 6; ++r) X2[r] = s_X[r];
                for (int r = 0; r < 6; ++r) {
                    double s = 0; for (int m = 0; m < 6; ++m) s += (double)it->P[r * 6 + m] * (double)X2[m];
                    s_X[r] = (float)s;
                }
            }
#pragma unroll
            for (int m = 0; m < 6; ++m) { Tn[m] = it->T[m] + s_X[m]; it->T[m] = Tn[m]; }
        }
        const float ang = lane == 0 ? lane_value(Tn[2], 0) : (lane == 1 ? lane_value(Tn[1], 0) : lane_value(Tn[0], 0));
        const float cs = cosf(ang), sn = sinf(ang);
        const float trig[6] = { lane_value(cs, 0), lane_value(sn, 0), lane_value(cs, 1), lane_value(sn, 1), lane_value(cs, 2), lane_value(sn, 2) };
        if (l0) write_pose_cache(it, trig);
        if (l0) {
            const double r0 = (double)(s_X[0] * 57.29578f), r1 = (double)(s_X[1] * 57.29578f), r2 = (double)(s_X[2] * 57.29578f);
            const double t0 = (double)(s_X[3] * 100.f), t1 = (double)(s_X[4] * 100.f), t2 = (double)(s_X[5] * 100.f);
            const float dR = (float)sqrt(r0 * r0 + r1 * r1 + r2 * r2);
            const float dT = (float)sqrt(t0 * t0 + t1 * t1 + t2 * t2);
            it->deltaR = dR; it->deltaT = dT;
            it->degenerate = isDeg;
            it->any_solved = 1;
            if (tr) {
                for (int i = 0; i < 36; ++i) tr[1 + i] = s_AtA[i];
                for (int i = 0; i < 6; ++i) { tr[37 + i] = s_AtB[i]; tr[43 + i] = s_X[i]; tr[49 + i] = it->T[i]; }
                tr[55] = 1.f;
            }
            if (dR < P.conv_deg && dT < P.conv_cm && P.fixed_iters <= 0) {
                it->iters_out = iter;
                finished = true;
            }
        }
    }
    if (l0) {
        it->iter = iter + 1;
        if (!finished && iter + 1 >= P.bound) { it->iters_out = P.bound; finished = true; }
        if (finished) { it->done = 1; atomicAdd(done_counter, 1); }
    }
}

struct Quat { double x, y, z, w; };
__device__ Quat q_rpy(double roll, double pitch, double yaw)
{
    const double hy = yaw * 0.5, hp = pitch * 0.5, hr = roll * 0.5;
    const double cy = cos(hy), sy = sin(hy), cp = cos(hp), sp = sin(hp), cr = cos(hr), sr = sin(hr);
    return Quat{ sr * cp * cy - cr * sp * sy, cr * sp * cy + sr * cp * sy, cr * cp * sy - sr * sp * cy,
                 cr * cp * cy + sr * sp * sy };
}
__device__ double q_dot(Quat a, Quat b) { return a.x * b.x + a.y * b.y + a.z * b.z + a.w * b.w; }
__device__ Quat q_slerp(Quat a, Quat b, double t)
{
    const double s = sqrt(q_dot(a, a) * q_dot(b, b));
    const double d = q_dot(a, b);
    const double theta = (d < 0 ? acos(-d / s) * 2.0 : acos(d / s) * 2.0) / 2.0;
    if (theta != 0.0) {
        const double dd = 1.0 / sin(theta), s0 = sin((1.0 - t) * theta), s1 = sin(t * theta);
        const double sg = d < 0 ? -1.0 : 1.0;
        return Quat{ (a.x * s0 + sg * b.x * s1) * dd, (a.y * s0 + sg * b.y * s1) * dd,
                     (a.z * s0 + sg * b.z * s1) * dd, (a.w * s0 + sg * b.w * s1) * dd };
    }
    return a;
}
__device__ void q_get_rpy(Quat q, double& roll, double& pitch, double& yaw)
{
    const double d = q_dot(q, q), s = 2.0 / d;
    const double xs = q.x * s, ys = q.y * s, zs = q.z * s;
    const double wx = q.w * xs, wy = q.w * ys, wz = q.w * zs;
    const double xx = q.x * xs, xy = q.x * ys, xz = q.x * zs, yy = q.y * ys, yz = q.y * zs, zz = q.z * zs;
    const double m00 = 1.0 - (yy + zz), m10 = xy + wz, m20 = xz - wy, m21 = yz + wx, m22 = 1.0 - (xx + yy);
    if (fabs(m20) >= 1) {
        yaw = 0;
        roll = atan2(m21, m22);
        pitch = m20 < 0 ? 1.5707963267948966 : -1.5707963267948966;
    } else {
        pitch = -asin(m20);
        const double cp = cos(pitch);
        roll = atan2(m21 / cp, m22 / cp);
        yaw = atan2(m10 / cp, m00 / cp);
    }
}
__device__ float clampf(float v, float lim) { v = v < -lim ? -lim : v; return v > lim ? lim : v; }

__global__ __launch_bounds__(64) void k_finalize(ItemState* __restrict__ items, int n_items, const DevParams P,
                                                 float* __restrict__ results, int* __restrict__ reset_done_counter)
{
    const int i = blockIdx.x * 64 + threadIdx.x;
    if (i == 0 && reset_done_counter) *reset_done_counter = P.n_guard_failed;
    if (i >= n_items) return;
    ItemState* it = &items[i];
    float T[6];
    for (int k = 0; k < 6; ++k) T[k] = it->T[k];
// ... 65 lines not shown
```

lis-slam_amd/lisreg/__init__.py:

```python
from __future__ import annotations

import ctypes as C
import os
import subprocess

import numpy as np

_PKG = os.path.dirname(os.path.dirname(os.path.abspath(__file__)))
LIB_PATH = os.path.join(_PKG, "lib", "liblisreg.so")
CSRC = os.path.join(_PKG, "csrc")

OK, NOT_ENOUGH_FEATURES, TOO_FEW_CORRESPONDENCES, LEAF_TOO_SMALL = 0, 1, 2, 3
ERR_ARG, ERR_HIP, ERR_NO_TARGET, ERR_NOMEM, ERR_COMM = -1, -2, -3, -4, -5
FMT_XYZI, FMT_XYZIL, FMT_DEVICE, FMT_XYZIRT, FMT_DEVICE_XYZI, FMT_XYZI_PACKED = 0, 1, 2, 3, 4, 5
VARIANT_ODOM, VARIANT_KEYFRAME, VARIANT_SUBMAP = 1, 2, 3
TRACE_STRIDE = 56
RESULT_SIZE = 12

ABI_SYMBOLS = [
    "lisreg_device_count", "lisreg_create", "lisreg_destroy", "lisreg_last_error", "lisreg_set_stream",
    "lisreg_get_stream", "lisreg_default_params", "lisreg_set_target", "lisreg_set_target_slot",
    "lisreg_target_from_classes", "lisreg_align", "lisreg_align_batch", "lisreg_batch_prepare", "lisreg_batch_run",
    "lisreg_batch_fetch", "lisreg_stage_host_items", "lisreg_upload_cloud", "lisreg_concat_device", "lisreg_batch_result_device", "lisreg_set_option", "lisreg_get_option", "lisreg_get_counters", "lisreg_get_neighbors", "lisreg_test_fit_models", "lisreg_get_target_index", "lisreg_get_target_graph", "lisreg_get_target_cell_rows", "lisreg_keyframes_reset", "lisreg_keyframes_push", "lisreg_keyframes_target", "lisreg_get_trace",
    "lisreg_set_profiling", "lisreg_get_timing", "lisreg_pose_to_matrix", "lisreg_transform_update",
    "lisreg_comm_unique_id", "lisreg_comm_init", "lisreg_gather_results", "lisreg_comm_destroy",
    "lisreg_voxel_downsample", "lisreg_voxel_downsample_multi", "lisreg_transform_cloud",
    "lisreg_extract_features", "lisreg_extract_features_deskew", "lisreg_extract_features_batch", "lisreg_default_feature_params", "lisreg_semantic_split",
    "lisreg_map_index_set", "lisreg_map_index_set_batch", "lisreg_nearest", "lisreg_dynamic_filter", "lisreg_bbx_filter", "lisreg_cloud_bounds",
    "lisreg_localmap_default_params", "lisreg_localmap_reset", "lisreg_localmap_insert", "lisreg_localmap_extract",
    "lisreg_localmap_get", "lisreg_predict_pose", "lisreg_guess_state_init", "lisreg_update_initial_guess", "lisreg_submap_insert", "lisreg_submap_extract", "lisreg_submap_crop_boxes",
    "lisreg_icp_default_params", "lisreg_icp_align", "lisreg_icp_align_batch", "lisreg_icp_gn_match",
    "lisreg_loopdet_default_params", "lisreg_loopdet_reset", "lisreg_loopdet_detect", "lisreg_loopdet_candidates",
    "lisreg_loopdet_get", "lisreg_loop_descriptor",
    "lisreg_loopdet_configure", "lisreg_loopdet_matches", "lisreg_loopdet_candidate_scores", "lisreg_loopdet_get_descriptor",
    "lisreg_loop_descriptor_kind",
    "lisreg_default_pretreat_params", "lisreg_pretreat", "lisreg_pretreat_batch",
    "lisreg_default_rangenet_params", "lisreg_rangenet_project", "lisreg_rangenet_project_batch", "lisreg_rangenet_label",
    "lisreg_rangenet_label_batch",
]


ICP_NOT_CONVERGED, ICP_ITERATIONS, ICP_TRANSFORM, ICP_ABS_MSE, ICP_REL_MSE, ICP_NO_CORRESPONDENCES = range(6)


class IcpParams(C.Structure):
    _fields_ = [("max_corr_dist", C.c_double), ("max_iters", C.c_int), ("reserved", C.c_int),
                ("transformation_epsilon", C.c_double), ("euclidean_fitness_epsilon", C.c_double), ("prev_mse", C.c_double)]


class IcpResult(C.Structure):
    _fields_ = [("final_transform", C.c_float * 16), ("converged", C.c_int), ("iters", C.c_int), ("state", C.c_int),
                ("n_corr_last", C.c_int), ("fitness", C.c_double), ("prev_mse", C.c_double)]

    def as_dict(self):
        return dict(T=np.array(list(self.final_transform), np.float32).reshape(4, 4), converged=bool(self.converged),
                    iters=self.iters, state=self.state, n_corr_last=self.n_corr_last, fitness=self.fitness, prev_mse=self.prev_mse)


class GuessInput(C.Structure):
    _fields_ = [("odom_available", C.c_int), ("imu_available", C.c_int),
                ("imu_roll_init", C.c_float), ("imu_pitch_init", C.c_float), ("imu_yaw_init", C.c_float),
                ("initial_guess_x", C.c_float), ("initial_guess_y", C.c_float), ("initial_guess_z", C.c_float),
                ("initial_guess_roll", C.c_float), ("initial_guess_pitch", C.c_float), ("initial_guess_yaw", C.c_float)]


class GuessState(C.Structure):
    _fields_ = [("first_trans_available", C.c_int), ("last_imu_pre_trans_available", C.c_int), ("first", C.c_int), ("reserved", C.c_int),
                ("last_imu_transformation", C.c_float * 12), ("last_imu_pre_transformation", C.c_float * 12),
                ("last_transform_tobe_mapped", C.c_float * 6)]


class IcpItem(C.Structure):
    _fields_ = [("source", C.c_void_p), ("n", C.c_int), ("slot", C.c_int), ("guess", C.POINTER(C.c_float))]


LOOPDET_MAX_DB = 16
# ... 178 lines not shown
        self.code = code


def build(verbose: bool = False) -> str:
    subprocess.check_call(["make", "-C", CSRC] + ([] if verbose else ["-s"]))
    return LIB_PATH


_lib = None


def lib():
    global _lib
    if _lib is None:
        if not os.path.exists(LIB_PATH):
            raise FileNotFoundError(f"{LIB_PATH} not built — run `make -C {CSRC}` (there is no fallback path)")
        L = C.CDLL(LIB_PATH)
        vp, fp, ip = C.c_void_p, C.POINTER(C.c_float), C.POINTER(C.c_int)
        L.lisreg_device_count.restype = C.c_int
        L.lisreg_create.argtypes = [C.c_int, C.POINTER(vp)]
        L.lisreg_destroy.argtypes = [vp]
        L.lisreg_destroy.restype = None
        L.lisreg_last_error.argtypes = [vp]
        L.lisreg_last_error.restype = C.c_char_p
        L.lisreg_set_stream.argtypes = [vp, vp]
        L.lisreg_get_stream.argtypes = [vp]
        L.lisreg_get_stream.restype = vp
        L.lisreg_default_params.argtypes = [C.c_int, C.POINTER(Params)]
        L.lisreg_set_target.argtypes = [vp, vp, C.c_int, vp, C.c_int, C.c_int, C.c_int]
        L.lisreg_set_target_slot.argtypes = [vp, C.c_int, vp, C.c_int, vp, C.c_int, C.c_int, C.c_int]
        L.lisreg_target_from_classes.argtypes = [vp, C.c_int, vp, C.c_int, vp, C.c_int, vp, C.c_int, vp, C.c_int,
                                                 C.c_int, C.c_int]
        L.lisreg_align.argtypes = [vp, vp, C.c_int, vp, C.c_int, C.c_int, C.c_int, C.POINTER(Params),
                                   C.POINTER(Imu), fp, C.POINTER(Stats)]
        L.lisreg_align_batch.argtypes = [vp, C.c_int, C.POINTER(Item), C.POINTER(Params), fp, C.POINTER(Stats)]
        L.lisreg_batch_prepare.argtypes = [vp, C.c_int, C.POINTER(Item), C.POINTER(Params), fp]
        L.lisreg_stage_host_items.argtypes = [vp, C.c_int, C.POINTER(Item), C.POINTER(Item)]
        L.lisreg_batch_run.argtypes = [vp]
        L.lisreg_batch_fetch.argtypes = [vp, fp, C.POINTER(Stats)]
        L.lisreg_batch_result_device.argtypes = [vp]
        L.lisreg_batch_result_device.restype = vp
        L.lisreg_set_option.argtypes = [vp, C.c_char_p, C.c_int]
        L.lisreg_upload_cloud.argtypes = [vp, vp, C.c_int, C.c_int, C.c_int, vp]
        L.lisreg_concat_device.argtypes = [vp, C.c_int, C.POINTER(C.c_void_p), C.POINTER(C.c_int), vp, C.POINTER(C.c_int)]
        L.lisreg_get_option.argtypes = [vp, C.c_char_p, C.POINTER(C.c_int)]
        L.lisreg_get_neighbors.argtypes = [vp, C.POINTER(C.c_int), C.c_int]
        if hasattr(L, "lisreg_test_fit_models"): L.lisreg_test_fit_models.argtypes = [vp, C.c_int, C.c_int, C.POINTER(C.c_float), C.POINTER(C.c_float), C.POINTER(Params), C.c_int, C.POINTER(C.c_float)]
        L.lisreg_get_target_index.argtypes = [vp, C.c_int, C.c_int, C.POINTER(C.c_int), C.POINTER(C.c_float), C.c_void_p, C.c_int, C.c_void_p, C.c_int]
        L.lisreg_get_target_graph.argtypes = [vp, C.c_int, C.c_int, C.POINTER(C.c_int), C.POINTER(C.c_float), C.POINTER(C.c_float), C.c_int]
        L.lisreg_get_target_cell_rows.argtypes = [vp, C.c_int, C.c_int, C.POINTER(C.c_int), C.POINTER(C.c_int), C.POINTER(C.c_int), C.c_int,
                                                  C.POINTER(C.c_float), C.POINTER(C.c_float), C.c_int]
        L.lisreg_get_counters.argtypes = [vp, C.POINTER(C.c_ulonglong), C.c_int]
        L.lisreg_get_trace.argtypes = [vp, fp, C.c_int]
        L.lisreg_set_profiling.argtypes = [vp, C.c_int]
        L.lisreg_get_timing.argtypes = [vp, C.POINTER(C.c_double)]
        L.lisreg_pose_to_matrix.argtypes = [fp, fp]
        L.lisreg_pose_to_matrix.restype = None
        L.lisreg_transform_update.argtypes = [C.POINTER(Params), C.POINTER(Imu), fp]
        L.lisreg_transform_update.restype = None
        L.lisreg_comm_unique_id.argtypes = [C.POINTER(C.c_ubyte)]
        L.lisreg_comm_init.argtypes = [vp, C.c_int, C.c_int, C.POINTER(C.c_ubyte)]
        L.lisreg_gather_results.argtypes = [vp, vp, C.c_int, vp]
        L.lisreg_comm_destroy.argtypes = [vp]
        L.lisreg_comm_destroy.restype = None
        L.lisreg_voxel_downsample_multi.argtypes = [vp, C.c_int, C.POINTER(C.c_void_p), C.POINTER(C.c_int), C.POINTER(C.c_float), C.c_int,
                                                    C.POINTER(C.c_void_p), C.POINTER(C.c_int), C.POINTER(C.c_int)]
        L.lisreg_voxel_downsample.argtypes = [vp, vp, C.c_int, C.c_int, C.c_int, C.c_float, vp, C.c_int, ip]
        L.lisreg_transform_cloud.argtypes = [vp, vp, C.c_int, C.c_int, C.c_int, fp, vp]
        L.lisreg_extract_features.argtypes = [vp, vp, C.c_int, C.c_int, C.c_int, C.POINTER(FeatureParams), C.POINTER(FeatureOut)]
        L.lisreg_default_feature_params.argtypes = [C.POINTER(FeatureParams)]
        L.lisreg_extract_features_batch.argtypes = [vp, C.c_int, C.POINTER(C.c_void_p), C.POINTER(C.c_int), C.POINTER(FeatureParams),
                                                    C.POINTER(FeatureOut)]
        L.lisreg_extract_features_deskew.argtypes = [vp, vp, C.c_int, C.c_int, C.c_int, C.POINTER(FeatureParams), C.POINTER(Deskew),
                                                     C.POINTER(FeatureOut)]
        L.lisreg_default_pretreat_params.argtypes = [C.POINTER(PretreatParams)]
        L.lisreg_pretreat.argtypes = [vp, vp, C.c_int, C.c_int, C.c_int, C.POINTER(PretreatParams), C.POINTER(PretreatOut)]
        L.lisreg_pretreat_batch.argtypes = [vp, C.c_int, C.POINTER(C.c_void_p), C.POINTER(C.c_int), C.POINTER(PretreatParams),
                                            C.POINTER(PretreatOut)]
        L.lisreg_default_rangenet_params.argtypes = [C.POINTER(RangenetParams)]
        L.lisreg_rangenet_project.argtypes = [vp, vp, C.c_int, C.c_int, C.c_int, C.POINTER(RangenetParams), C.POINTER(RangenetOut)]
        L.lisreg_rangenet_project_batch.argtypes = [vp, C.c_int, C.POINTER(C.c_void_p), C.POINTER(C.c_int), C.POINTER(RangenetParams),
                                                    C.POINTER(RangenetOut)]
        L.lisreg_rangenet_label.argtypes = [vp, vp, C.c_int, C.c_int, vp, vp, vp, C.POINTER(RangenetParams), vp, vp]
        L.lisreg_rangenet_label_batch.argtypes = [vp, C.c_int, C.POINTER(C.c_void_p), C.POINTER(C.c_int), C.POINTER(C.c_void_p),
                                                  C.POINTER(C.c_void_p), C.POINTER(C.c_void_p), C.POINTER(RangenetParams),
                                                  C.POINTER(C.c_void_p), C.POINTER(C.c_void_p)]
        L.lisreg_semantic_split.argtypes = [vp, vp, C.c_int, C.c_int, C.c_int, C.POINTER(C.c_uint32), C.POINTER(SemanticOut)]
        ip, dp = C.POINTER(C.c_int), C.POINTER(C.c_double)
        L.lisreg_map_index_set.argtypes = [vp, C.c_int, vp, C.c_int, C.c_int, C.c_int]
        L.lisreg_map_index_set_batch.argtypes = [vp, C.c_int, C.POINTER(C.c_int), C.POINTER(C.c_void_p), C.POINTER(C.c_int), C.c_int, C.c_int]
        L.lisreg_nearest.argtypes = [vp, C.c_int, vp, C.c_int, C.c_int, C.c_int, C.c_float, vp, vp]
        L.lisreg_dynamic_filter.argtypes = [vp, C.c_int, vp, C.c_int, C.c_int, C.c_int, C.c_float, C.c_float, C.c_float,
                                            C.c_float, vp, ip]
        L.lisreg_bbx_filter.argtypes = [vp, vp, C.c_int, C.c_int, C.c_int, dp, C.c_int, vp, ip]
        L.lisreg_cloud_bounds.argtypes = [vp, vp, C.c_int, C.c_int, C.c_int, dp]
        L.lisreg_localmap_default_params.argtypes = [C.POINTER(LocalMapParams)]
        L.lisreg_localmap_reset.argtypes = [vp, C.c_int]
        L.lisreg_keyframes_reset.argtypes = [vp, C.c_int]
        L.lisreg_keyframes_push.argtypes = [vp, C.c_int, vp, C.c_int, vp, C.c_int, C.c_int, C.c_int, C.POINTER(C.c_float), C.c_int, C.POINTER(KeyframesInfo)]
        L.lisreg_keyframes_target.argtypes = [vp, C.c_int, C.c_float, C.c_float, C.c_int, C.POINTER(KeyframesInfo)]
        L.lisreg_localmap_insert.argtypes = [vp, C.c_int, C.POINTER(C.c_void_p), C.POINTER(C.c_int), C.c_int, C.c_int, fp,
                                             C.POINTER(LocalMapParams), C.POINTER(LocalMapInfo)]
        L.lisreg_localmap_extract.argtypes = [vp, C.c_int, fp, C.POINTER(LocalMapParams), C.c_int, C.POINTER(LocalMapInfo)]
        L.lisreg_localmap_get.argtypes = [vp, C.c_int, C.c_int, vp, C.c_int, ip]
        L.lisreg_submap_insert.argtypes = [vp, C.c_int, C.POINTER(C.c_void_p), C.POINTER(C.c_int), C.c_int, C.c_int, fp, fp,
                                           C.POINTER(LocalMapParams), C.POINTER(SubmapInfo)]
# ... 167 lines not shown
        return self.get_option("front_end")

    def set_profiling_paused(self, paused: bool):
        self._chk(self._L.lisreg_set_profiling(self._h, 0 if paused else 1))

    def set_target(self, corner: np.ndarray, surf: np.ndarray, slot: int = 0):
        corner = np.ascontiguousarray(corner); surf = np.ascontiguousarray(surf)
        self._chk(self._L.lisreg_set_target_slot(self._h, slot, _vp(corner), len(corner), _vp(surf), len(surf),
                                                 corner.dtype.itemsize, _fmt_of(corner)))

    def set_target_device(self, corner_ptr: int, n_corner: int, surf_ptr: int, n_surf: int, slot: int = 0):
        self._chk(self._L.lisreg_set_target_slot(self._h, slot, C.c_void_p(corner_ptr), n_corner,
                                                 C.c_void_p(surf_ptr), n_surf, 16, FMT_DEVICE))

    def target_from_classes(self, pole, ground, building, dynamic, slot: int = 0):
        arrs = [np.ascontiguousarray(a) for a in (pole, ground, building, dynamic)]
        self._chk(self._L.lisreg_target_from_classes(self._h, slot, _vp(arrs[0]), len(arrs[0]), _vp(arrs[1]),
                                                     len(arrs[1]), _vp(arrs[2]), len(arrs[2]), _vp(arrs[3]),
                                                     len(arrs[3]), arrs[0].dtype.itemsize, _fmt_of(arrs[0])))

    def align(self, src_corner: np.ndarray, src_surf: np.ndarray, T_init, params: Params, imu: Imu | None = None):
        sc = np.ascontiguousarray(src_corner); ss = np.ascontiguousarray(src_surf)
        T = np.array(T_init, np.float32).copy()
        st = Stats()
        rc = self._L.lisreg_align(self._h, _vp(sc), len(sc), _vp(ss), len(ss), sc.dtype.itemsize, _fmt_of(sc),
                                  C.byref(params), C.byref(imu) if imu is not None else None,
                                  T.ctypes.data_as(C.POINTER(C.c_float)), C.byref(st))
        self._chk(rc, allow=(OK, NOT_ENOUGH_FEATURES, TOO_FEW_CORRESPONDENCES))
        bound = params.fixed_iters if params.fixed_iters > 0 else params.max_iters
        buf = np.zeros((max(bound, 1), TRACE_STRIDE), np.float32)
        n = self._L.lisreg_get_trace(self._h, buf.ctypes.data_as(C.POINTER(C.c_float)), max(bound, 1))
        d = stats_dict(st)
        if rc == NOT_ENOUGH_FEATURES:
            d["status"] = NOT_ENOUGH_FEATURES
        return T, d, buf[:n]

    def align_batch(self, items: list[dict], T_init: np.ndarray, params: Params):
        n = len(items)
        arr = (Item * max(n, 1))()
        keep = []
        for i, it in enumerate(items):
            sc = np.ascontiguousarray(it["src_corner"]); ss = np.ascontiguousarray(it["src_surf"])
            keep += [sc, ss]
            arr[i].src_corner = _vp(sc); arr[i].n_corner = len(sc)
            arr[i].src_surf = _vp(ss); arr[i].n_surf = len(ss)
            arr[i].stride_bytes = sc.dtype.itemsize; arr[i].fmt = _fmt_of(sc)
            arr[i].target = it.get("target", 0); arr[i].degenerate_in = it.get("degenerate_in", 0)
            if it.get("imu") is not None:
                arr[i].imu = it["imu"]
        T = np.ascontiguousarray(T_init, np.float32).reshape(n, 6).copy()
        st = (Stats * max(n, 1))()
        self._chk(self._L.lisreg_align_batch(self._h, n, arr, C.byref(params),
                                             T.ctypes.data_as(C.POINTER(C.c_float)), st))
        return T, [stats_dict(st[i]) for i in range(n)]

    def batch_prepare_device(self, items: list[dict], T_init: np.ndarray, params: Params):
        n = len(items)
        arr = (Item * max(n, 1))()
        for i, it in enumerate(items):
            arr[i].src_corner = C.c_void_p(it["corner_ptr"]) if it["n_corner"] else None
            arr[i].n_corner = it["n_corner"]
            arr[i].src_surf = C.c_void_p(it["surf_ptr"]) if it["n_surf"] else None
            arr[i].n_surf = it["n_surf"]
            arr[i].stride_bytes = 16; arr[i].fmt = FMT_DEVICE
            arr[i].target = it.get("target", 0); arr[i].degenerate_in = it.get("degenerate_in", 0)
            if it.get("imu") is not None:
                arr[i].imu = it["imu"]
        T = np.ascontiguousarray(T_init, np.float32).reshape(n, 6)
        self._n_items = n
        self._chk(self._L.lisreg_batch_prepare(self._h, n, arr, C.byref(params),
                                               T.ctypes.data_as(C.POINTER(C.c_float))))

    def batch_run(self):
        self._chk(self._L.lisreg_batch_run(self._h))

    def batch_fetch(self):
        n = self._n_items
        T = np.zeros((n, 6), np.float32)
        st = (Stats * max(n, 1))()
        self._chk(self._L.lisreg_batch_fetch(self._h, T.ctypes.data_as(C.POINTER(C.c_float)), st))
        return T, [stats_dict(st[i]) for i in range(n)]

    @property
    def result_device_ptr(self) -> int:
        return self._L.lisreg_batch_result_device(self._h) or 0

    def counters(self) -> np.ndarray:
        out = (C.c_ulonglong * 64)()
        self._chk(self._L.lisreg_get_counters(self._h, out, 64))
        return np.array(out[:], np.int64).reshape(32, 2)

    def target_index(self, slot: int = 0, kind: int = 1) -> dict:
        dims = (C.c_int * 5)(); geom = (C.c_float * 4)()
        self._chk(self._L.lisreg_get_target_index(self._h, slot, kind, dims, geom, None, 0, None, 0))
        n, nx, ny, nz, nc = [int(v) for v in dims]
        pts = np.zeros((max(n, 1), 4), np.float32); cs = np.zeros(nc + 1, np.int32)
        self._chk(self._L.lisreg_get_target_index(self._h, slot, kind, dims, geom, pts.ctypes.data, n, cs.ctypes.data, nc + 1))
        return dict(n=n, nx=nx, ny=ny, nz=nz, n_cells=nc, origin=np.array(geom[:3], np.float32), cell=float(geom[3]),
                    sorted=pts[:n], cell_start=cs)

    def target_graph(self, slot: int = 0, kind: int = 1) -> dict:
        n = self.target_index(slot, kind)["n"]
        k = C.c_int()
        self._chk(self._L.lisreg_get_target_graph(self._h, slot, kind, C.byref(k), None, None, 0))
        rows = np.zeros((max(n, 1), k.value, 4), np.float32); meta = np.zeros((max(n, 1), 2), np.float32)
        self._chk(self._L.lisreg_get_target_graph(self._h, slot, kind, C.byref(k), rows.ctypes.data_as(C.POINTER(C.c_float)),
                                                  meta.ctypes.data_as(C.POINTER(C.c_float)), n))
        return dict(k=k.value, ids=rows[:n, :, 3].copy().view(np.int32), xyz=rows[:n, :, :3], rho2=meta[:n, 0],
                    count=meta[:n, 1].copy().view(np.int32))

    def target_cell_rows(self, slot: int = 0, kind: int = 1) -> dict:
        n_rows, k = C.c_int(), C.c_int()
        self._chk(self._L.lisreg_get_target_cell_rows(self._h, slot, kind, C.byref(n_rows), C.byref(k), None, 0, None, None, 0))
        nc = self.target_index(slot, kind)["n_cells"]
        table = np.zeros(max(nc, 1), np.int32)
        rows = np.zeros((max(n_rows.value, 1), k.value, 4), np.float32); meta = np.zeros((max(n_rows.value, 1), 2), np.float32)
        self._chk(self._L.lisreg_get_target_cell_rows(self._h, slot, kind, C.byref(n_rows), C.byref(k), table.ctypes.data_as(C.POINTER(C.c_int)), nc,
                                                      rows.ctypes.data_as(C.POINTER(C.c_float)), meta.ctypes.data_as(C.POINTER(C.c_float)), n_rows.value))
        r = n_rows.value
        return dict(k=k.value, n_rows=r, table=table[:nc], ids=rows[:r, :, 3].copy().view(np.int32), xyz=rows[:r, :, :3], rho2=meta[:r, 0],
                    count=meta[:r, 1].copy().view(np.int32))

    def raw_counters(self):
        out = (C.c_ulonglong * 128)()
        self._chk(self._L.lisreg_get_counters(self._h, out, 128))
        return [int(v) for v in out]

# ... 695 lines not shown
```

Measured before the change: 30330 registrations/s.

## Fuse each half-batch's GN solve into the other half's association kernel

The batch is split into two halves of blocks. Each iteration's association launches alternate between the halves, and every launch after the first carries extra leading workgroups. Those workgroups run the Gauss-Newton solve step for the other half, so the small, serial solve kernel overlaps with association work instead of running as its own launch. XCD ordering tables are built per half so block remapping stays valid within each sub-grid. The change also adds a batch trace readback API, at the cost of more template instantiations, extra shared-memory reuse and a more complex schedule.

```diff
diff --git a/include/lisreg.h b/include/lisreg.h
--- a/include/lisreg.h
+++ b/include/lisreg.h
@@ -138,6 +138,7 @@
                                  float* rows_out, float* meta_out, int capacity_rows);
 
 int  lisreg_get_trace(lisreg_ctx* ctx, float* buf, int max_iters);
+int  lisreg_batch_trace(lisreg_ctx* ctx, float* out, int capacity_records);
 
 int  lisreg_set_profiling(lisreg_ctx* ctx, int enable);
 int  lisreg_get_timing(lisreg_ctx* ctx, double out[5]);
diff --git a/lis-slam_amd/csrc/lisreg_api.hip b/lis-slam_amd/csrc/lisreg_api.hip
--- a/lis-slam_amd/csrc/lisreg_api.hip
+++ b/lis-slam_amd/csrc/lisreg_api.hip
@@ -529,6 +529,8 @@
 }
 
 static bool xcd_order_wanted(const lisreg_ctx* c);
+static void half_cut(const lisreg_ctx* c, int* item, int* blk);
+static int make_half_tables(lisreg_ctx* c, int cut_blk, hipStream_t st);
 
 int lisreg_batch_prepare(lisreg_ctx* c, int n_items, const lisreg_item* items, const lisreg_params* params,
                          const float* T_init)
@@ -815,6 +817,12 @@
         HIPCHK(c, hipGetLastError());
         c->xcd_cached = true;
     }
+    c->xcd_half_split = 0;
+    if (c->xcd_cached && c->solve_overlap != 0 && c->interleave == 0 && c->lanes_q == 1) {
+        int cut_item = 0, cut_blk = 0;
+        half_cut(c, &cut_item, &cut_blk);
+        if (cut_blk > 0) { rc = make_half_tables(c, cut_blk, c->stream); if (rc) return rc; }
+    }
     c->prepared = true;
     return LISREG_OK;
 }
@@ -848,6 +856,32 @@
     return c->lanes_q != 8 &&
            (((c->mode_now == 3 || c->mode_now == 5) && (c->xcd_order == 1 || (c->xcd_order == 2 && c->n_blocks >= 2048 && c->n_items >= 32))) ||
             (many_targets && c->xcd_order != 0 && c->n_blocks >= 2048));
+}
+
+static void half_cut(const lisreg_ctx* c, int* item, int* blk)
+{
+    *item = 0; *blk = 0;
+    if (c->n_items < 2 || c->n_blocks < c->interleave_min_blocks) return;
+    for (int i = 1; i < c->n_items; ++i)
+        if (c->h_items[(size_t)i].blk_begin * 2 >= c->n_blocks) { *item = i; *blk = c->h_items[(size_t)i].blk_begin; break; }
+    if (*blk * 4 < c->n_blocks || (c->n_blocks - *blk) * 4 < c->n_blocks) { *item = 0; *blk = 0; }
+}
+
+static int make_half_tables(lisreg_ctx* c, int cut_blk, hipStream_t st)
+{
+    const bool many_targets = c->batch_slots.size() >= 8 && c->xcd_order == 1;
+    c->xcd_half_split = 0;
+    HIPCHK(c, c->xcd_half.ensure(sizeof(int) * 2 * (size_t)c->n_blocks));
+    int* const keys = c->xcd_half.as<int>();
+    int* const order = keys + c->n_blocks;
+    const float4* sorted = c->sort_now ? c->sorted_all.as<float4>() : nullptr;
+    launch_xcd_order(c->blocks.as<BlockDesc>(), cut_blk, c->segs.as<Segment>(), c->grids_dev.as<GridIndex>(), c->items.as<ItemState>(),
+                     sorted, many_targets, keys, order, st);
+    launch_xcd_order(c->blocks.as<BlockDesc>() + cut_blk, c->n_blocks - cut_blk, c->segs.as<Segment>(), c->grids_dev.as<GridIndex>(),
+                     c->items.as<ItemState>(), sorted, many_targets, keys + cut_blk, order + cut_blk, st);
+    HIPCHK(c, hipGetLastError());
+    if (!c->sort_now) c->xcd_half_split = cut_blk;
+    return LISREG_OK;
 }
 
 static int run_impl(lisreg_ctx* c, bool early_stop)
@@ -864,12 +898,12 @@
         ensure_side_stream(c);
         if (c->side_stream && !c->ev_ab && (c->ev_ab.create(hipEventDisableTiming) != hipSuccess ||
                                             c->ev_ba.create(hipEventDisableTiming) != hipSuccess)) { c->ev_ab.reset(); c->ev_ba.reset(); }
-        if (c->side_stream) {
-            for (int i = 1; i < c->n_items; ++i)
-                if (c->h_items[(size_t)i].blk_begin * 2 >= c->n_blocks) { split_item = i; split_blk = c->h_items[(size_t)i].blk_begin; break; }
-            if (split_blk * 4 < c->n_blocks || (c->n_blocks - split_blk) * 4 < c->n_blocks) { split_item = 0; split_blk = 0; }
-        }
-    }
+        if (c->side_stream) half_cut(c, &split_item, &split_blk);
+    }
+    int ov_item = 0, ov_blk = 0;
+    if (c->solve_overlap != 0 && c->interleave == 0 && !c->exact && !can_stop && c->lanes_q == 1 && c->prm.bound >= 1)
+        half_cut(c, &ov_item, &ov_blk);
+    const bool overlap = ov_blk > 0;
     c->reach_now = c->rebuild_targets_each_run && c->mode_now == 5 && c->reach_ready && !c->exact;
     int* const miss_dev = reinterpret_cast<int*>(c->results.as<float>() + (size_t)std::max(c->n_items, 1) * kResultSize);
     c->prm.reach_miss = c->reach_now ? miss_dev : nullptr;
@@ -911,6 +945,9 @@
     launch_sort_sources(c->blocks.as<BlockDesc>(), c->n_blocks, c->segs.as<Segment>(), c->n_segs, c->items.as<ItemState>(),
                         c->n_elems, c->sort_now ? c->n_buckets : 0, sort_buffers(c), c->sorted_all.as<float4>(), c->order_all.as<int>(), st);
     prof_mark(c, -1);
+    if (c->xcd_now && overlap) {
+        if (c->xcd_half_split != ov_blk || c->sort_now) { int rc = make_half_tables(c, ov_blk, st); if (rc) return rc; }
+    } else
     if (c->xcd_now && !(c->xcd_cached && split_blk == 0)) {
         const int nb0 = split_blk ? split_blk : c->n_blocks;
         launch_xcd_order(c->blocks.as<BlockDesc>(), nb0, c->segs.as<Segment>(), c->grids_dev.as<GridIndex>(), c->items.as<ItemState>(),
@@ -936,7 +973,7 @@
                      c->count_searches ? c->counters.as<unsigned long long>() : nullptr,
                      c->dump_neighbors ? c->dbg_nn.as<int>() : nullptr, c->lanes_q,
                      c->blocks_q.as<BlockDesc>(), (int)c->h_blocks_q.size(), c->coef.as<float4>(), c->coef_ok.as<int>(),
-                     c->xcd_now ? c->xcd_tab.as<int>() + c->n_blocks + b0 : nullptr, s_);
+                     c->xcd_now ? c->xcd_tab.as<int>() + c->n_blocks + b0 : nullptr, s_, nullptr);
         if (after_assoc) (void)hipEventRecord(after_assoc, s_);
         prof_mark(c, 1, sidx);
         launch_solve(c->items.as<ItemState>() + i0, ni, c->prm, c->partials.as<double>(),
@@ -944,6 +981,31 @@
         prof_mark(c, -1, sidx);
     };
     c->interleaved_now = false;
+    c->solve_overlap_now = false;
+    if (overlap) {
+        c->solve_overlap_now = true;
+        const int i0[2] = { 0, ov_item }, ni[2] = { ov_item, c->n_items - ov_item }, b0[2] = { 0, ov_blk }, nb[2] = { ov_blk, c->n_blocks - ov_blk };
+        FuseSolve fs[2];
+        for (int h = 0; h < 2; ++h)
+            fs[h] = FuseSolve{ c->items.as<ItemState>() + i0[h], c->partials.as<double>(),
+                               c->trace_cap > 0 ? c->trace.as<float>() + (size_t)i0[h] * (size_t)c->trace_cap * kTraceStride : nullptr,
+                               c->done_dev.as<int>(), c->trace_cap, ni[h], (ni[h] + 7) & ~7 };
+        for (int l = 0; l < 2 * c->prm.bound; ++l) {
+            const int h = l & 1, it = l >> 1;
+            prof_mark(c, 0);
+            launch_assoc(c->blocks.as<BlockDesc>() + b0[h], nb[h], c->segs.as<Segment>(), c->grids_dev.as<GridIndex>(),
+                         c->items.as<ItemState>(), c->prm, c->sort_now ? c->sorted_all.as<float4>() : nullptr, c->partials.as<double>() + (size_t)b0[h] * kNumAcc,
+                         c->mode_now, c->nn.as<int>(), c->n_elems, c->first_pass_r * c->first_pass_r,
+                         c->mode_now != 5 && it >= kWideFrom && it <= (c->mode_now == 3 ? kGraphWideUntil : kWideUntil), kGraphHops,
+                         c->count_searches ? c->counters.as<unsigned long long>() : nullptr,
+                         c->dump_neighbors ? c->dbg_nn.as<int>() : nullptr, 1,
+                         c->blocks_q.as<BlockDesc>(), (int)c->h_blocks_q.size(), c->coef.as<float4>(), c->coef_ok.as<int>(),
+                         c->xcd_now ? c->xcd_half.as<int>() + c->n_blocks + b0[h] : nullptr, st, l > 0 ? &fs[h ^ 1] : nullptr);
+        }
+        prof_mark(c, 1);
+        launch_solve(fs[1].items, fs[1].n, c->prm, fs[1].partials, fs[1].trace, c->trace_cap, c->done_dev.as<int>(), st);
+        prof_mark(c, -1);
+    } else
     if (split_blk > 0 && hipEventRecord(c->ev_fork, st) == hipSuccess && hipStreamWaitEvent(c->side_stream, c->ev_fork, 0) == hipSuccess) {
         c->interleaved_now = true;
         const bool alternate = c->interleave == 1 && c->ev_ab && c->ev_ba;
@@ -1029,6 +1091,17 @@
 
 void* lisreg_batch_result_device(const lisreg_ctx* c) { return c ? c->results.p : nullptr; }
 
+static int schedule_option(lisreg_ctx* c, const char* name, const int* set, int* get)
+{
+    if (!strcmp(name, "solve_overlap")) {
+        if (set) { if (*set < 0 || *set > 1) return fail(c, LISREG_ERR_ARG, "solve_overlap: 0 off, 1 on"); c->solve_overlap = *set; }
+        else *get = c->solve_overlap;
+        return LISREG_OK;
+    }
+    if (!set && !strcmp(name, "solve_overlap_now")) { *get = c->solve_overlap_now ? 1 : 0; return LISREG_OK; }
+    return -1;
+}
+
 int lisreg_set_option(lisreg_ctx* c, const char* name, int value)
 {
     if (!c || !name) return LISREG_ERR_ARG;
@@ -1058,7 +1131,7 @@
         return LISREG_OK;
     }
     if (!strcmp(name, "early_stop_chunk")) { c->early_stop_chunk = value; return LISREG_OK; }
-    if (!strcmp(name, "xcd_order")) { if (value < 0 || value > 2) return fail(c, LISREG_ERR_ARG, "xcd_order: 0 off, 1 on, 2 auto"); c->xcd_order = value; c->xcd_cached = false; return LISREG_OK; }
+    if (!strcmp(name, "xcd_order")) { if (value < 0 || value > 2) return fail(c, LISREG_ERR_ARG, "xcd_order: 0 off, 1 on, 2 auto"); c->xcd_order = value; c->xcd_cached = false; c->xcd_half_split = 0; return LISREG_OK; }
     if (!strcmp(name, "index_build")) {
         if (value < 0 || value > 2) return fail(c, LISREG_ERR_ARG, "index_build: 0 bucket sort, 1 strip form, 2 auto");
         c->index_build = value; c->prepared = false;
@@ -1085,6 +1158,7 @@
     if (!strcmp(name, "feeder_numa")) { c->feeder_numa = value != 0; return LISREG_OK; }
     if (!strcmp(name, "interleave_min_blocks")) { c->interleave_min_blocks = std::max(value, 2); return LISREG_OK; }
     if (!strcmp(name, "interleave")) { if (value < 0 || value > 2) return fail(c, LISREG_ERR_ARG, "interleave: 0 off, 1 alternating halves, 2 free-running halves"); c->interleave = value; return LISREG_OK; }
+    { const int rc = schedule_option(c, name, &value, nullptr); if (rc >= 0) return rc; }
     return fail(c, LISREG_ERR_ARG, std::string("set_option: unknown option ") + name);
 }
 
@@ -1154,6 +1228,7 @@
         *value = (int)std::min<unsigned long long>(v, 0x7fffffffULL);
         return LISREG_OK;
     }
+    { const int rc = schedule_option(const_cast<lisreg_ctx*>(c), name, nullptr, value); if (rc >= 0) return rc; }
     return LISREG_ERR_ARG;
 }
 
@@ -1273,6 +1348,19 @@
     const int n = std::min(max_iters, c->last_trace_n);
     if (n > 0) memcpy(buf, c->last_trace.data(), sizeof(float) * kTraceStride * (size_t)n);
     return n;
+}
+
+int lisreg_batch_trace(lisreg_ctx* c, float* out, int capacity_records)
+{
+    if (!c || !out || capacity_records < 0) return LISREG_ERR_ARG;
+    if (!c->prepared || c->trace_cap <= 0 || !c->trace.p || c->n_items <= 0) return 0;
+    const size_t n = (size_t)c->n_items * (size_t)c->trace_cap;
+    if ((size_t)capacity_records < n) { fail(c, LISREG_ERR_ARG, "batch_trace: capacity below n_items x trace_cap records"); return LISREG_ERR_ARG; }
+    if (hipSetDevice(c->device) != hipSuccess || hipStreamSynchronize(c->stream) != hipSuccess ||
+        hipMemcpy(out, c->trace.p, sizeof(float) * kTraceStride * n, hipMemcpyDeviceToHost) != hipSuccess) {
+        fail(c, LISREG_ERR_HIP, "batch_trace: copy failed"); return LISREG_ERR_HIP;
+    }
+    return c->trace_cap;
 }
 
 int lisreg_get_counters(lisreg_ctx* c, unsigned long long* out, int n)
diff --git a/lis-slam_amd/csrc/lisreg_assoc.hip b/lis-slam_amd/csrc/lisreg_assoc.hip
--- a/lis-slam_amd/csrc/lisreg_assoc.hip
+++ b/lis-slam_amd/csrc/lisreg_assoc.hip
@@ -11,6 +11,7 @@
 #define LISREG_ASSOC_NS fast_arith
 #define LISREG_LAUNCH_ASSOC launch_assoc
 #define LISREG_LAUNCH_TEST_FIT launch_test_fit
+#include "lisreg_solve_body.hpp"
 #endif
 
 namespace lisreg {
@@ -886,7 +887,7 @@
             (void)o4; \
         } } } while (0)
 
-template <bool kWide, int kGraph, int kQ, bool kTies, bool kShare = false>
+template <bool kWide, int kGraph, int kQ, bool kTies, bool kShare = false, typename... Fuse>
 __global__ __launch_bounds__(kBlockQ) __attribute__((amdgpu_waves_per_eu(kShare ? 4 : 8, kShare ? 4 : 8))) void k_assoc_walk(const BlockDesc* __restrict__ blocks,
                                                         const Segment* __restrict__ segs,
                                                         const GridIndex* __restrict__ grids,
@@ -895,7 +896,7 @@
                                                         int* __restrict__ nn_, int n_elems, float first_pass_r2,
                                                         int graph_hops, unsigned long long* __restrict__ counters,
                                                         int* __restrict__ dbg_nn, float4* __restrict__ coef, int* __restrict__ coef_ok,
-                                                        double* __restrict__ partials, const int* __restrict__ xcd_order)
+                                                        double* __restrict__ partials, const int* __restrict__ xcd_order, const Fuse... fuse)
 {
     __shared__ __attribute__((aligned(16))) int2 s_runs_w[kBlockQ / 64][kWalkCap][64];
     static_assert(sizeof(int2) * kWalkCap * 64 == sizeof(float) * kRedWaveFloats, "one region per wavefront");
@@ -905,6 +906,48 @@
 
     const int tid = threadIdx.x;
     int bid = blockIdx.x;
+#if !LISREG_EXACT
+    if constexpr (sizeof...(Fuse) > 0) {
+        static_assert(sizeof...(Fuse) == 1 && kQ == 1 && !kShare && kBlockQ == 256, "one FuseSolve, one lane per query");
+        const FuseSolve fs = (fuse, ...);
+        if ((int)blockIdx.x < fs.n_pad) {
+            if ((int)blockIdx.x >= fs.n) return;
+            constexpr int kStepThreads = kBlockQ;
+            ItemState* const sv_it = fs.items + blockIdx.x;
+            const unsigned sv_idx = blockIdx.x;
+            const double* const sv_partials = fs.partials;
+            float* const sv_trace = fs.trace;
+            const int sv_trace_cap = fs.trace_cap;
+            int* const sv_done = fs.done_counter;
+            double* const lds = reinterpret_cast<double*>(&s_runs_w[0][0][0]);
+            static_assert(sizeof(s_runs_w) >= sizeof(double) * (kSolveGroups * 32 + 32 + 36) + sizeof(float) * (36 * 5 + 6 * 3 + 12), "the step's LDS fits");
+            double (*const s_part)[32] = reinterpret_cast<double (*)[32]>(lds);
+            double* const s_sum = lds + kSolveGroups * 32;
+            double* const s_L = s_sum + 32;
+            float* const s_AtA = reinterpret_cast<float*>(s_L + 36);
+            float* const s_AtB = s_AtA + 36;
+            float* const s_X = s_AtB + 6;
+            float* const s_A = s_X + 6;
+            float* const s_E = s_A + 36;
+            float* const s_V = s_E + 6;
+            float* const s_V2 = s_V + 36;
+            float* const s_Vi = s_V2 + 36;
+            int* const s_ind = reinterpret_cast<int*>(s_Vi + 36);
+#define LISREG_STEP_CALL [[clang::always_inline]]
+#define LISREG_STEP_ROLL _Pragma("nounroll")
+#include "lisreg_solve_step.inc"
+#undef LISREG_STEP_ROLL
+#undef LISREG_STEP_CALL
+            return;
+        }
+        bid = (int)blockIdx.x - fs.n_pad;
+        if (xcd_order) {
+            const int nb = (int)gridDim.x - fs.n_pad;
+            const int m = nb >> 3, t = nb & 7, x = bid & 7;
+            bid = xcd_order[x * m + min(x, t) + (bid >> 3)];
+        }
+    } else
+#endif
     if (xcd_order) {
         const int m = gridDim.x >> 3, t = gridDim.x & 7, x = blockIdx.x & 7;
         bid = xcd_order[x * m + min(x, t) + (int)(blockIdx.x >> 3)];
@@ -1274,9 +1317,22 @@
                               const ItemState* items, DevParams prm, const float4* sorted_all, double* partials,
                               int mode, int* nn, int n_elems, float first_pass_r2, bool wide, int graph_hops,
                               unsigned long long* counters, int* dbg_nn, int lanes_q,
-                              const BlockDesc* blocks_q, int n_blocks_q, float4* coef, int* coef_ok, const int* xcd_order, hipStream_t st)
+                              const BlockDesc* blocks_q, int n_blocks_q, float4* coef, int* coef_ok, const int* xcd_order, hipStream_t st,
+                              const FuseSolve* fuse)
 {
     using namespace LISREG_ASSOC_NS;
+#if !LISREG_EXACT
+    if (fuse) {
+        const int grid = n_blocks + fuse->n_pad;
+#define LISREG_FUSED(W_, G_) k_assoc_walk<W_, G_, 1, kTies, false, FuseSolve><<<grid, kBlockQ, 0, st>>>(blocks, segs, grids, items, prm, sorted_all, nn, n_elems, \
+                                 first_pass_r2, graph_hops, counters, dbg_nn, coef, coef_ok, partials, xcd_order, *fuse)
+        if (mode == 1) { if (wide) LISREG_FUSED(true, 0); else LISREG_FUSED(false, 0); }
+        else if (mode == 5) LISREG_FUSED(false, 2);
+        else { if (wide) LISREG_FUSED(true, 1); else LISREG_FUSED(false, 1); }
+#undef LISREG_FUSED
+        return;
+    }
+#endif
     if (mode == 1 && lanes_q == 8) {
         const bool share = n_blocks_q <= 2048;
         if (wide && share)
@@ -1324,19 +1380,20 @@
                          const ItemState* items, DevParams prm, const float4* sorted_all, double* partials,
                          int mode, int* nn, int n_elems, float first_pass_r2, bool wide, int graph_hops,
                          unsigned long long* counters, int* dbg_nn, int lanes_q,
-                         const BlockDesc* blocks_q, int n_blocks_q, float4* coef, int* coef_ok, const int* xcd_order, hipStream_t st)
+                         const BlockDesc* blocks_q, int n_blocks_q, float4* coef, int* coef_ok, const int* xcd_order, hipStream_t st,
+                         const FuseSolve* fuse)
 {
     if (n_blocks <= 0) return;
 #if LISREG_EXACT
     launch_assoc_impl<true>(blocks, n_blocks, segs, grids, items, prm, sorted_all, partials, mode, nn, n_elems, first_pass_r2, wide, graph_hops,
-                            counters, dbg_nn, lanes_q, blocks_q, n_blocks_q, coef, coef_ok, xcd_order, st);
+                            counters, dbg_nn, lanes_q, blocks_q, n_blocks_q, coef, coef_ok, xcd_order, st, fuse);
 #else
     if (prm.ties)
         launch_assoc_impl<true>(blocks, n_blocks, segs, grids, items, prm, sorted_all, partials, mode, nn, n_elems, first_pass_r2, wide, graph_hops,
-                                counters, dbg_nn, lanes_q, blocks_q, n_blocks_q, coef, coef_ok, xcd_order, st);
+                                counters, dbg_nn, lanes_q, blocks_q, n_blocks_q, coef, coef_ok, xcd_order, st, fuse);
     else
         launch_assoc_impl<false>(blocks, n_blocks, segs, grids, items, prm, sorted_all, partials, mode, nn, n_elems, first_pass_r2, wide, graph_hops,
-                                 counters, dbg_nn, lanes_q, blocks_q, n_blocks_q, coef, coef_ok, xcd_order, st);
+                                 counters, dbg_nn, lanes_q, blocks_q, n_blocks_q, coef, coef_ok, xcd_order, st, fuse);
 #endif
 }
 
diff --git a/lis-slam_amd/csrc/lisreg_ctx.hpp b/lis-slam_amd/csrc/lisreg_ctx.hpp
--- a/lis-slam_amd/csrc/lisreg_ctx.hpp
+++ b/lis-slam_amd/csrc/lisreg_ctx.hpp
@@ -150,7 +150,7 @@
     lisreg::PinnedBuf grids_host;
     lisreg::Event grids_done;
     lisreg::DevBuf hist, bucket_start, scan_tmp, elem_bucket, elem_sub, tmp_bucket, tmp_sub, tmp_idx, tmp_pts, bbox_dev, bbox_scratch;
-    lisreg::DevBuf blocks, segs, items, sorted_all, order_all, partials, results, trace, src_upload, raw_upload, dbg_nn, blocks_q, coef, coef_ok, nn, counters, tseg_dev, tblk_dev, tchunk_dev, strip_tab, done_dev, xcd_tab,
+    lisreg::DevBuf blocks, segs, items, sorted_all, order_all, partials, results, trace, src_upload, raw_upload, dbg_nn, blocks_q, coef, coef_ok, nn, counters, tseg_dev, tblk_dev, tchunk_dev, strip_tab, done_dev, xcd_tab, xcd_half,
            vox_in, vox_lab, vox_order, vox_sidx, vox_head, vox_slot, vox_start, vox_out, vox_outlab, vox_M,
            ft_owner, ft_flag, ft_pos, ft_scan, ft_col, ft_range, ft_src, ft_curv, ft_picked, ft_label, ft_rlists, ft_rcounts,
            ft_lists, ft_counts, ft_rings, ft_gather, ft_cat, ft_bounds, ft_dsk_tab, ft_dsk_pts, ft_dsk_misc, ft_dsk_time;
@@ -220,6 +220,9 @@
     int       graph_min_ratio = 60;
     int       interleave = 0;
     bool      interleaved_now = false;
+    int       solve_overlap = 1;
+    bool      solve_overlap_now = false;
+    int       xcd_half_split = 0;
     int       interleave_min_blocks = 8192;
     int       xcd_order = 2;
     bool      xcd_now = false;
diff --git a/lis-slam_amd/csrc/lisreg_internal.hpp b/lis-slam_amd/csrc/lisreg_internal.hpp
--- a/lis-slam_amd/csrc/lisreg_internal.hpp
+++ b/lis-slam_amd/csrc/lisreg_internal.hpp
@@ -159,6 +159,7 @@
                          const ItemState* items, int n_elems, int n_buckets, SortBuffers sb, float4* sorted_all, int* order_all,
                          hipStream_t st);
 void launch_reset_items(ItemState* items, int n_items, DevParams prm, int* done_counter, hipStream_t st, int* zero_too = nullptr);
+struct FuseSolve { ItemState* items; const double* partials; float* trace; int* done_counter; int trace_cap, n, n_pad; };
 void launch_assoc(const BlockDesc* blocks, int n_blocks, const Segment* segs, const GridIndex* grids,
                   const ItemState* items, DevParams prm, const float4* sorted_all, double* partials,
                   int mode ,
@@ -170,12 +171,13 @@
                   int lanes_q ,
                   const BlockDesc* blocks_q, int n_blocks_q ,
                   float4* coef, int* coef_ok ,
-                  const int* xcd_order , hipStream_t st);
+                  const int* xcd_order , hipStream_t st,
+                  const FuseSolve* fuse = nullptr );
 void launch_assoc_exact(const BlockDesc* blocks, int n_blocks, const Segment* segs, const GridIndex* grids,
                         const ItemState* items, DevParams prm, const float4* sorted_all, double* partials,
                         int mode, int* nn, int n_elems, float first_pass_r2, bool wide, int graph_hops,
                         unsigned long long* counters, int* dbg_nn, int lanes_q, const BlockDesc* blocks_q, int n_blocks_q,
-                        float4* coef, int* coef_ok, const int* xcd_order, hipStream_t st);
+                        float4* coef, int* coef_ok, const int* xcd_order, hipStream_t st, const FuseSolve* fuse = nullptr );
 void launch_test_fit(int kind, int n, const float* nb15, const float* q3, DevParams prm, float* out, hipStream_t st);
 void launch_test_fit_exact(int kind, int n, const float* nb15, const float* q3, DevParams prm, float* out, hipStream_t st);
 void launch_xcd_order(const BlockDesc* blocks, int n_blocks, const Segment* segs, const GridIndex* grids, const ItemState* items,
diff --git a/lis-slam_amd/csrc/lisreg_solve.hip b/lis-slam_amd/csrc/lisreg_solve.hip
--- a/lis-slam_amd/csrc/lisreg_solve.hip
+++ b/lis-slam_amd/csrc/lisreg_solve.hip
@@ -1,188 +1,8 @@
-#include "lisreg_internal.hpp"
+#include "lisreg_solve_body.hpp"
 
 namespace lisreg {
 
 namespace {
-
-__device__ float hyp(float a, float b)
-{
-    a = fabsf(a); b = fabsf(b);
-    if (a > b) { b /= a; return a * sqrtf(1.f + b * b); }
-    if (b > 0.f) { a /= b; return b * sqrtf(1.f + a * a); }
-    return 0.f;
-}
-
-__device__ void eigen_sym6(float* A, float* W, float* V, int* indR, int* indC)
-{
-    const int n = 6;
-    for (int i = 0; i < n; ++i) for (int j = 0; j < n; ++j) V[i * n + j] = (i == j) ? 1.f : 0.f;
-    for (int k = 0; k < n; ++k) {
-        W[k] = A[k * n + k];
-        if (k < n - 1) {
-            int m = k + 1; float mv = fabsf(A[k * n + m]);
-            for (int i = k + 2; i < n; ++i) { float v = fabsf(A[k * n + i]); if (mv < v) { mv = v; m = i; } }
-            indR[k] = m;
-        }
-        if (k > 0) {
-            int m = 0; float mv = fabsf(A[k]);
-            for (int i = 1; i < k; ++i) { float v = fabsf(A[i * n + k]); if (mv < v) { mv = v; m = i; } }
-            indC[k] = m;
-        }
-    }
-    for (int it = 0; it < n * n * 30; ++it) {
-        int k = 0, l; float mv = fabsf(A[indR[0]]);
-        for (int i = 1; i < n - 1; ++i) { float v = fabsf(A[i * n + indR[i]]); if (mv < v) { mv = v; k = i; } }
-        l = indR[k];
-        for (int i = 1; i < n; ++i) { float v = fabsf(A[indC[i] * n + i]); if (mv < v) { mv = v; k = indC[i]; l = i; } }
-        const float p = A[k * n + l];
-        if (fabsf(p) <= 1.1920929e-7f) break;
-        const float y = (W[l] - W[k]) * 0.5f;
-        float t = fabsf(y) + hyp(p, y);
-        float s = hyp(p, t);
-        const float c = t / s;
-        s = p / s; t = (p / t) * p;
-        if (y < 0.f) { s = -s; t = -t; }
-        A[k * n + l] = 0.f;
-        W[k] -= t; W[l] += t;
-#define LR(v0, v1) do { const float a0_ = (v0), b0_ = (v1); (v0) = a0_ * c - b0_ * s; (v1) = a0_ * s + b0_ * c; } while (0)
-        for (int i = 0; i < k; ++i)      LR(A[i * n + k], A[i * n + l]);
-        for (int i = k + 1; i < l; ++i)  LR(A[k * n + i], A[i * n + l]);
-        for (int i = l + 1; i < n; ++i)  LR(A[k * n + i], A[l * n + i]);
-        for (int i = 0; i < n; ++i)      LR(V[k * n + i], V[l * n + i]);
-#undef LR
-        for (int j = 0; j < 2; ++j) {
-            const int idx = j == 0 ? k : l;
-            if (idx < n - 1) {
-                int m = idx + 1; float mv2 = fabsf(A[idx * n + m]);
-                for (int i = idx + 2; i < n; ++i) { float v = fabsf(A[idx * n + i]); if (mv2 < v) { mv2 = v; m = i; } }
-                indR[idx] = m;
-            }
-            if (idx > 0) {
-                int m = 0; float mv2 = fabsf(A[idx]);
-                for (int i = 1; i < idx; ++i) { float v = fabsf(A[i * n + idx]); if (mv2 < v) { mv2 = v; m = i; } }
-                indC[idx] = m;
-            }
-        }
-    }
-    for (int k = 0; k < n - 1; ++k) {
-        int m = k;
-        for (int i = k + 1; i < n; ++i) if (W[m] < W[i]) m = i;
-        if (m != k) {
-            float tw = W[m]; W[m] = W[k]; W[k] = tw;
-            for (int i = 0; i < n; ++i) { float tv = V[m * n + i]; V[m * n + i] = V[k * n + i]; V[k * n + i] = tv; }
-        }
-    }
-}
-
-__device__ __forceinline__ float lane_value(float v, int l) { return __int_as_float(__builtin_amdgcn_readlane(__float_as_int(v), l)); }
-__device__ __forceinline__ bool solve6_qr_lanes(float a[6], int lane, float x[6])
-{
-#pragma unroll
-    for (int k = 0; k < 6; ++k) {
-        const float c0 = a[k];
-        float tail = 0.f;
-#pragma unroll
-        for (int i = k + 1; i < 6; ++i) tail += a[i] * a[i];
-        float beta, tau, v[6];
-        if (tail <= 1.17549435e-38f) {
-            tau = 0.f; beta = c0;
-#pragma unroll
-            for (int i = 0; i < 6; ++i) v[i] = 0.f;
-        } else {
-            beta = sqrtf(c0 * c0 + tail);
-            if (c0 >= 0.f) beta = -beta;
-#pragma unroll
-            for (int i = 0; i < 6; ++i) v[i] = (i > k) ? a[i] / (c0 - beta) : 0.f;
-            tau = (beta - c0) / beta;
-        }
-        if (lane == k) a[k] = beta;
-        tau = lane_value(tau, k);
-#pragma unroll
-        for (int i = k + 1; i < 6; ++i) v[i] = lane_value(v[i], k);
-        if (tau != 0.f && lane > k) {
-            float dot = a[k];
-#pragma unroll
-            for (int i = k + 1; i < 6; ++i) dot += v[i] * a[i];
-            dot *= tau;
-            a[k] -= dot;
-#pragma unroll
-            for (int i = k + 1; i < 6; ++i) a[i] -= dot * v[i];
-        }
-    }
-    float R[6][6], c[6];
-#pragma unroll
-    for (int i = 0; i < 6; ++i) {
-        c[i] = lane_value(a[i], 6);
-#pragma unroll
-        for (int j = i; j < 6; ++j) R[i][j] = lane_value(a[i], j);
-    }
-    bool singular = false;
-#pragma unroll
-    for (int i = 0; i < 6; ++i) singular = singular || (fabsf(R[i][i]) <= 1.17549435e-38f);
-    float y[6];
-#pragma unroll
-    for (int i = 5; i >= 0; --i) {
-        float s_ = c[i];
-#pragma unroll
-        for (int j = i + 1; j < 6; ++j) s_ -= R[i][j] * y[j];
-        y[i] = s_ / R[i][i];
-    }
-#pragma unroll
-    for (int i = 0; i < 6; ++i) x[i] = singular ? 0.f : y[i];
-    return !singular;
-}
-
-__device__ void inv6_lu(float* A, float* B)
-{
-    const int N = 6;
-    for (int i = 0; i < N; ++i) for (int j = 0; j < N; ++j) B[i * N + j] = (i == j) ? 1.f : 0.f;
-    for (int i = 0; i < N; ++i) {
-        int k = i;
-        for (int j = i + 1; j < N; ++j) if (fabsf(A[j * N + i]) > fabsf(A[k * N + i])) k = j;
-        if (fabsf(A[k * N + i]) < 1.1920929e-7f * 100) { for (int j = 0; j < N * N; ++j) B[j] = 0.f; return; }
-        if (k != i) for (int j = 0; j < N; ++j) {
-            float t = A[i * N + j]; A[i * N + j] = A[k * N + j]; A[k * N + j] = t;
-            t = B[i * N + j]; B[i * N + j] = B[k * N + j]; B[k * N + j] = t;
-        }
-        const float d = -1.f / A[i * N + i];
-        for (int j = i + 1; j < N; ++j) {
-            const float alpha = A[j * N + i] * d;
-            for (int m = i + 1; m < N; ++m) A[j * N + m] += alpha * A[i * N + m];
-            for (int m = 0; m < N; ++m) B[j * N + m] += alpha * B[i * N + m];
-        }
-    }
-    for (int i = N - 1; i >= 0; --i)
-        for (int j = 0; j < N; ++j) {
-            float s = B[i * N + j];
-            for (int k = i + 1; k < N; ++k) s -= A[i * N + k] * B[k * N + j];
-            B[i * N + j] = s / A[i * N + i];
-        }
-}
-
-__device__ void write_pose_cache(ItemState* it, const float* trig = nullptr)
-{
-    const float* T = it->T;
-    float A, B, C, D, E, F;
-    if (trig) { A = trig[0]; B = trig[1]; C = trig[2]; D = trig[3]; E = trig[4]; F = trig[5]; }
-    else { A = cosf(T[2]); B = sinf(T[2]); C = cosf(T[1]); D = sinf(T[1]); E = cosf(T[0]); F = sinf(T[0]); }
-    const float DE = D * E, DF = D * F;
-    float* M = it->M;
-    M[0] = A * C;  M[1] = A * DF - B * E;  M[2]  = B * F + A * DE;  M[3]  = T[3];
-    M[4] = B * C;  M[5] = A * E + B * DF;  M[6]  = B * DE - A * F;  M[7]  = T[4];
-    M[8] = -D;     M[9] = C * F;           M[10] = C * E;           M[11] = T[5];
-    it->sc[0] = D; it->sc[1] = C;
-    it->sc[2] = B; it->sc[3] = A;
-    it->sc[4] = F; it->sc[5] = E;
-    const float srx = D, crx = C, sry = B, cry = A, srz = F, crz = E;
-    float* K = it->jk;
-    K[0] = crx * sry * srz;  K[1] = crx * crz * sry;  K[2] = srx * sry;
-    K[3] = -srx * srz;       K[4] = crz * srx;        K[5] = crx;
-    K[6] = crx * cry * srz;  K[7] = crx * cry * crz;  K[8] = cry * srx;
-    K[9] = cry * srx * srz - crz * sry;    K[10] = sry * srz + cry * crz * srx;   K[11] = crx * cry;
-    K[12] = -cry * crz - srx * sry * srz;  K[13] = cry * srz - crz * srx * sry;   K[14] = crx * sry;
-    K[15] = crz * srx * sry - cry * srz;   K[16] = crx * crz;                      K[17] = crx * srz;
-    K[18] = crz * sry - cry * srx * srz;   K[19] = 0.f;                            K[20] = 0.f;
-}
 
 __device__ __forceinline__ void reset_item(ItemState* it, const DevParams& P)
 {
@@ -223,146 +43,18 @@
     __shared__ double s_sum[kNumAcc];
     __shared__ double s_L[36];
 
-    ItemState* it = &items[blockIdx.x];
-    if (it->done) return;
-    {
-        const int col = threadIdx.x & 31, grp = threadIdx.x >> 5;
-        double s = 0.0;
-        if (col < kNumAcc) {
-            const double* p = partials + (size_t)it->blk_begin * kNumAcc + col;
-            const int nb = it->blk_count;
-            constexpr int kG = kSolveThreads / 32;
-            for (int b = grp; b < nb; b += 32 * kG) {
-                double v[32];
-#pragma unroll
-                for (int u = 0; u < 32; ++u) v[u] = (b + u * kG < nb) ? p[(size_t)(b + u * kG) * kNumAcc] : 0.0;
-#pragma unroll
-                for (int u = 0; u < 32; ++u) s += v[u];
-            }
-        }
-        s_part[grp][col] = s;
-    }
-    __syncthreads();
-    if (threadIdx.x < kNumAcc) {
-        double s = 0.0;
-#pragma unroll
-        for (int g = 0; g < kSolveThreads / 32; ++g) s += s_part[g][threadIdx.x];
-        s_sum[threadIdx.x] = s;
-    }
-    __syncthreads();
-    if (threadIdx.x >= 64) return;
-    const int lane = threadIdx.x;
-    const bool l0 = lane == 0;
-
-    const int iter = it->iter;
-    const int n_sel = (int)(s_sum[27] + 0.5);
-    float* tr = (trace && iter < trace_cap) ? trace + ((size_t)blockIdx.x * trace_cap + iter) * kTraceStride : nullptr;
-    if (l0) {
-        it->n_corr = n_sel;
-        if (tr) {
-            for (int k = 0; k < kTraceStride; ++k) tr[k] = 0.f;
-            tr[0] = (float)n_sel;
-            for (int k = 0; k < 6; ++k) tr[49 + k] = it->T[k];
-        }
-    }
-    bool finished = false;
-    if (n_sel >= P.min_corr) {
-        if (lane < 36) {
-            const int r_ = lane / 6, c_ = lane % 6, lo = min(r_, c_), hi = max(r_, c_);
-            s_AtA[lane] = (float)s_sum[lo * 6 - (lo * (lo - 1)) / 2 + (hi - lo)];
-        } else if (lane < 42) s_AtB[lane - 36] = (float)s_sum[21 + lane - 36];
-        __builtin_amdgcn_fence(__ATOMIC_RELEASE, "wavefront");
-        __builtin_amdgcn_wave_barrier();
-        __builtin_amdgcn_fence(__ATOMIC_ACQUIRE, "wavefront");
-        {
-            float a[6], xs[6];
-#pragma unroll
-            for (int i = 0; i < 6; ++i) a[i] = lane < 6 ? s_AtA[i * 6 + lane] : (lane == 6 ? s_AtB[i] : 0.f);
-            solve6_qr_lanes(a, lane, xs);
-            if (l0) {
-#pragma unroll
-                for (int i = 0; i < 6; ++i) s_X[i] = xs[i];
-            }
-        }
-        int isDeg = 0;
-        float Tn[6] = { 0.f, 0.f, 0.f, 0.f, 0.f, 0.f };
-        if (l0) {
-            isDeg = it->degenerate;
-            bool well_conditioned = false;
-            if (iter == 0) {
-                double* L = s_L;
-                double trace = 0.0;
-                for (int i = 0; i < 6; ++i) trace += (double)s_AtA[i * 6 + i];
-                const double shift = (double)P.eig_thresh + 2e-5 * trace;
-                well_conditioned = trace > 0.0;
-                for (int r = 0; r < 6 && well_conditioned; ++r)
-                    for (int c = 0; c <= r; ++c) {
-                        double v = (double)s_AtA[r * 6 + c] - (r == c ? shift : 0.0);
-                        for (int k = 0; k < c; ++k) v -= L[r * 6 + k] * L[c * 6 + k];
-                        if (r == c) { if (!(v > 0.0)) { well_conditioned = false; break; } L[r * 6 + r] = sqrt(v); }
-                        else L[r * 6 + c] = v / L[c * 6 + c];
-                    }
-            }
-            if (iter == 0 && well_conditioned) {
-                isDeg = 0;
-                for (int i = 0; i < 36; ++i) it->P[i] = (i % 7 == 0) ? 1.f : 0.f;
-            } else if (iter == 0) {
-                for (int i = 0; i < 36; ++i) s_A[i] = s_AtA[i];
-                eigen_sym6(s_A, s_E, s_V, s_ind, s_ind + 6);
-                for (int i = 0; i < 36; ++i) s_V2[i] = s_V[i];
-                isDeg = 0;
-                for (int i = 5; i >= 0; --i) {
-                    if (s_E[i] < P.eig_thresh) { for (int j = 0; j < 6; ++j) s_V2[i * 6 + j] = 0.f; isDeg = 1; }
-                    else break;
-                }
-                for (int i = 0; i < 36; ++i) s_A[i] = s_V[i];
-                inv6_lu(s_A, s_Vi);
-                for (int r = 0; r < 6; ++r) for (int c = 0; c < 6; ++c) {
-                    double s = 0; for (int m = 0; m < 6; ++m) s += (double)s_Vi[r * 6 + m] * (double)s_V2[m * 6 + c];
-                    it->P[r * 6 + c] = (float)s;
-                }
-            } else if (P.emulate_shadow) {
-                for (int i = 0; i < 36; ++i) it->P[i] = 0.f;
-            }
-            if (isDeg) {
-                float X2[6];
-                for (int r = 0; r < 6; ++r) X2[r] = s_X[r];
-                for (int r = 0; r < 6; ++r) {
-                    double s = 0; for (int m = 0; m < 6; ++m) s += (double)it->P[r * 6 + m] * (double)X2[m];
-                    s_X[r] = (float)s;
-                }
-            }
-#pragma unroll
-            for (int m = 0; m < 6; ++m) { Tn[m] = it->T[m] + s_X[m]; it->T[m] = Tn[m]; }
-        }
-        const float ang = lane == 0 ? lane_value(Tn[2], 0) : (lane == 1 ? lane_value(Tn[1], 0) : lane_value(Tn[0], 0));
-        const float cs = cosf(ang), sn = sinf(ang);
-        const float trig[6] = { lane_value(cs, 0), lane_value(sn, 0), lane_value(cs, 1), lane_value(sn, 1), lane_value(cs, 2), lane_value(sn, 2) };
-        if (l0) write_pose_cache(it, trig);
-        if (l0) {
-            const double r0 = (double)(s_X[0] * 57.29578f), r1 = (double)(s_X[1] * 57.29578f), r2 = (double)(s_X[2] * 57.29578f);
-            const double t0 = (double)(s_X[3] * 100.f), t1 = (double)(s_X[4] * 100.f), t2 = (double)(s_X[5] * 100.f);
-            const float dR = (float)sqrt(r0 * r0 + r1 * r1 + r2 * r2);
-            const float dT = (float)sqrt(t0 * t0 + t1 * t1 + t2 * t2);
-            it->deltaR = dR; it->deltaT = dT;
-            it->degenerate = isDeg;
-            it->any_solved = 1;
-            if (tr) {
-                for (int i = 0; i < 36; ++i) tr[1 + i] = s_AtA[i];
-                for (int i = 0; i < 6; ++i) { tr[37 + i] = s_AtB[i]; tr[43 + i] = s_X[i]; tr[49 + i] = it->T[i]; }
-                tr[55] = 1.f;
-            }
-            if (dR < P.conv_deg && dT < P.conv_cm && P.fixed_iters <= 0) {
-                it->iters_out = iter;
-                finished = true;
-            }
-        }
-    }
-    if (l0) {
-        it->iter = iter + 1;
-        if (!finished && iter + 1 >= P.bound) { it->iters_out = P.bound; finished = true; }
-        if (finished) { it->done = 1; atomicAdd(done_counter, 1); }
-    }
+    constexpr int kStepThreads = kSolveThreads;
+    ItemState* const sv_it = &items[blockIdx.x];
+    const unsigned sv_idx = blockIdx.x;
+    const double* const sv_partials = partials;
+    float* const sv_trace = trace;
+    const int sv_trace_cap = trace_cap;
+    int* const sv_done = done_counter;
+#define LISREG_STEP_CALL
+#define LISREG_STEP_ROLL
+#include "lisreg_solve_step.inc"
+#undef LISREG_STEP_ROLL
+#undef LISREG_STEP_CALL
 }
 
 struct Quat { double x, y, z, w; };
diff --git a/lis-slam_amd/csrc/lisreg_solve_body.hpp b/lis-slam_amd/csrc/lisreg_solve_body.hpp
--- /dev/null
+++ b/lis-slam_amd/csrc/lisreg_solve_body.hpp
@@ -0,0 +1,199 @@
+#pragma once
+#include "lisreg_internal.hpp"
+
+#define LISREG_NO_CONTRACT _Pragma("clang fp contract(off)")
+
+namespace lisreg {
+
+namespace {
+
+__device__ float hyp(float a, float b)
+{
+    LISREG_NO_CONTRACT
+    a = fabsf(a); b = fabsf(b);
+    if (a > b) { b /= a; return a * sqrtf(1.f + b * b); }
+    if (b > 0.f) { a /= b; return b * sqrtf(1.f + a * a); }
+    return 0.f;
+}
+
+__device__ void eigen_sym6(float* A, float* W, float* V, int* indR, int* indC)
+{
+    LISREG_NO_CONTRACT
+    const int n = 6;
+    for (int i = 0; i < n; ++i) for (int j = 0; j < n; ++j) V[i * n + j] = (i == j) ? 1.f : 0.f;
+    for (int k = 0; k < n; ++k) {
+        W[k] = A[k * n + k];
+        if (k < n - 1) {
+            int m = k + 1; float mv = fabsf(A[k * n + m]);
+            for (int i = k + 2; i < n; ++i) { float v = fabsf(A[k * n + i]); if (mv < v) { mv = v; m = i; } }
+            indR[k] = m;
+        }
+        if (k > 0) {
+            int m = 0; float mv = fabsf(A[k]);
+            for (int i = 1; i < k; ++i) { float v = fabsf(A[i * n + k]); if (mv < v) { mv = v; m = i; } }
+            indC[k] = m;
+        }
+    }
+    for (int it = 0; it < n * n * 30; ++it) {
+        int k = 0, l; float mv = fabsf(A[indR[0]]);
+        for (int i = 1; i < n - 1; ++i) { float v = fabsf(A[i * n + indR[i]]); if (mv < v) { mv = v; k = i; } }
+        l = indR[k];
+        for (int i = 1; i < n; ++i) { float v = fabsf(A[indC[i] * n + i]); if (mv < v) { mv = v; k = indC[i]; l = i; } }
+        const float p = A[k * n + l];
+        if (fabsf(p) <= 1.1920929e-7f) break;
+        const float y = (W[l] - W[k]) * 0.5f;
+        float t = fabsf(y) + hyp(p, y);
+        float s = hyp(p, t);
+        const float c = t / s;
+        s = p / s; t = (p / t) * p;
+        if (y < 0.f) { s = -s; t = -t; }
+        A[k * n + l] = 0.f;
+        W[k] -= t; W[l] += t;
+#define LR(v0, v1) do { const float a0_ = (v0), b0_ = (v1); (v0) = a0_ * c - b0_ * s; (v1) = a0_ * s + b0_ * c; } while (0)
+        for (int i = 0; i < k; ++i)      LR(A[i * n + k], A[i * n + l]);
+        for (int i = k + 1; i < l; ++i)  LR(A[k * n + i], A[i * n + l]);
+        for (int i = l + 1; i < n; ++i)  LR(A[k * n + i], A[l * n + i]);
+        for (int i = 0; i < n; ++i)      LR(V[k * n + i], V[l * n + i]);
+#undef LR
+        for (int j = 0; j < 2; ++j) {
+            const int idx = j == 0 ? k : l;
+            if (idx < n - 1) {
+                int m = idx + 1; float mv2 = fabsf(A[idx * n + m]);
+                for (int i = idx + 2; i < n; ++i) { float v = fabsf(A[idx * n + i]); if (mv2 < v) { mv2 = v; m = i; } }
+                indR[idx] = m;
+            }
+            if (idx > 0) {
+                int m = 0; float mv2 = fabsf(A[idx]);
+                for (int i = 1; i < idx; ++i) { float v = fabsf(A[i * n + idx]); if (mv2 < v) { mv2 = v; m = i; } }
+                indC[idx] = m;
+            }
+        }
+    }
+    for (int k = 0; k < n - 1; ++k) {
+        int m = k;
+        for (int i = k + 1; i < n; ++i) if (W[m] < W[i]) m = i;
+        if (m != k) {
+            float tw = W[m]; W[m] = W[k]; W[k] = tw;
+            for (int i = 0; i < n; ++i) { float tv = V[m * n + i]; V[m * n + i] = V[k * n + i]; V[k * n + i] = tv; }
+        }
+    }
+}
+
+__device__ __forceinline__ float lane_value(float v, int l) { return __int_as_float(__builtin_amdgcn_readlane(__float_as_int(v), l)); }
+__device__ __forceinline__ bool solve6_qr_lanes(float a[6], int lane, float x[6])
+{
+    LISREG_NO_CONTRACT
+#pragma unroll
+    for (int k = 0; k < 6; ++k) {
+        const float c0 = a[k];
+        float tail = 0.f;
+#pragma unroll
+        for (int i = k + 1; i < 6; ++i) tail += a[i] * a[i];
+        float beta, tau, v[6];
+        if (tail <= 1.17549435e-38f) {
+            tau = 0.f; beta = c0;
+#pragma unroll
+            for (int i = 0; i < 6; ++i) v[i] = 0.f;
+        } else {
+            beta = sqrtf(c0 * c0 + tail);
+            if (c0 >= 0.f) beta = -beta;
+#pragma unroll
+            for (int i = 0; i < 6; ++i) v[i] = (i > k) ? a[i] / (c0 - beta) : 0.f;
+            tau = (beta - c0) / beta;
+        }
+        if (lane == k) a[k] = beta;
+        tau = lane_value(tau, k);
+#pragma unroll
+        for (int i = k + 1; i < 6; ++i) v[i] = lane_value(v[i], k);
+        if (tau != 0.f && lane > k) {
+            float dot = a[k];
+#pragma unroll
+            for (int i = k + 1; i < 6; ++i) dot += v[i] * a[i];
+            dot *= tau;
+            a[k] -= dot;
+#pragma unroll
+            for (int i = k + 1; i < 6; ++i) a[i] -= dot * v[i];
+        }
+    }
+    float R[6][6], c[6];
+#pragma unroll
+    for (int i = 0; i < 6; ++i) {
+        c[i] = lane_value(a[i], 6);
+#pragma unroll
+        for (int j = i; j < 6; ++j) R[i][j] = lane_value(a[i], j);
+    }
+    bool singular = false;
+#pragma unroll
+    for (int i = 0; i < 6; ++i) singular = singular || (fabsf(R[i][i]) <= 1.17549435e-38f);
+    float y[6];
+#pragma unroll
+    for (int i = 5; i >= 0; --i) {
+        float s_ = c[i];
+#pragma unroll
+        for (int j = i + 1; j < 6; ++j) s_ -= R[i][j] * y[j];
+        y[i] = s_ / R[i][i];
+    }
+#pragma unroll
+    for (int i = 0; i < 6; ++i) x[i] = singular ? 0.f : y[i];
+    return !singular;
+}
+
+__device__ void inv6_lu(float* A, float* B)
+{
+    LISREG_NO_CONTRACT
+    const int N = 6;
+    for (int i = 0; i < N; ++i) for (int j = 0; j < N; ++j) B[i * N + j] = (i == j) ? 1.f : 0.f;
+    for (int i = 0; i < N; ++i) {
+        int k = i;
+        for (int j = i + 1; j < N; ++j) if (fabsf(A[j * N + i]) > fabsf(A[k * N + i])) k = j;
+        if (fabsf(A[k * N + i]) < 1.1920929e-7f * 100) { for (int j = 0; j < N * N; ++j) B[j] = 0.f; return; }
+        if (k != i) for (int j = 0; j < N; ++j) {
+            float t = A[i * N + j]; A[i * N + j] = A[k * N + j]; A[k * N + j] = t;
+            t = B[i * N + j]; B[i * N + j] = B[k * N + j]; B[k * N + j] = t;
+        }
+        const float d = -1.f / A[i * N + i];
+        for (int j = i + 1; j < N; ++j) {
+            const float alpha = A[j * N + i] * d;
+            for (int m = i + 1; m < N; ++m) A[j * N + m] += alpha * A[i * N + m];
+            for (int m = 0; m < N; ++m) B[j * N + m] += alpha * B[i * N + m];
+        }
+    }
+    for (int i = N - 1; i >= 0; --i)
+        for (int j = 0; j < N; ++j) {
+            float s = B[i * N + j];
+            for (int k = i + 1; k < N; ++k) s -= A[i * N + k] * B[k * N + j];
+            B[i * N + j] = s / A[i * N + i];
+        }
+}
+
+__device__ void write_pose_cache(ItemState* it, const float* trig = nullptr)
+{
+    LISREG_NO_CONTRACT
+    const float* T = it->T;
+    float A, B, C, D, E, F;
+    if (trig) { A = trig[0]; B = trig[1]; C = trig[2]; D = trig[3]; E = trig[4]; F = trig[5]; }
+    else { A = cosf(T[2]); B = sinf(T[2]); C = cosf(T[1]); D = sinf(T[1]); E = cosf(T[0]); F = sinf(T[0]); }
+    const float DE = D * E, DF = D * F;
+    float* M = it->M;
+    M[0] = A * C;  M[1] = A * DF - B * E;  M[2]  = B * F + A * DE;  M[3]  = T[3];
+    M[4] = B * C;  M[5] = A * E + B * DF;  M[6]  = B * DE - A * F;  M[7]  = T[4];
+    M[8] = -D;     M[9] = C * F;           M[10] = C * E;           M[11] = T[5];
+    it->sc[0] = D; it->sc[1] = C;
+    it->sc[2] = B; it->sc[3] = A;
+    it->sc[4] = F; it->sc[5] = E;
+    const float srx = D, crx = C, sry = B, cry = A, srz = F, crz = E;
+    float* K = it->jk;
+    K[0] = crx * sry * srz;  K[1] = crx * crz * sry;  K[2] = srx * sry;
+    K[3] = -srx * srz;       K[4] = crz * srx;        K[5] = crx;
+    K[6] = crx * cry * srz;  K[7] = crx * cry * crz;  K[8] = cry * srx;
+    K[9] = cry * srx * srz - crz * sry;    K[10] = sry * srz + cry * crz * srx;   K[11] = crx * cry;
+    K[12] = -cry * crz - srx * sry * srz;  K[13] = cry * srz - crz * srx * sry;   K[14] = crx * sry;
+    K[15] = crz * srx * sry - cry * srz;   K[16] = crx * crz;                      K[17] = crx * srz;
+    K[18] = crz * sry - cry * srx * srz;   K[19] = 0.f;                            K[20] = 0.f;
+}
+
+constexpr int kSolveGroups = 16;
+
+}
+
+}
diff --git a/lis-slam_amd/csrc/lisreg_solve_step.inc b/lis-slam_amd/csrc/lisreg_solve_step.inc
--- /dev/null
+++ b/lis-slam_amd/csrc/lisreg_solve_step.inc
@@ -0,0 +1,163 @@
+{
+    LISREG_NO_CONTRACT
+    static_assert(kStepThreads == 512 || kStepThreads == 256, "16 row groups: one or two per 32 threads");
+    if (sv_it->done) return;
+    if constexpr (kStepThreads == 512) {
+        const int col = threadIdx.x & 31, grp = threadIdx.x >> 5;
+        double s = 0.0;
+        if (col < kNumAcc) {
+            const double* p = sv_partials + (size_t)sv_it->blk_begin * kNumAcc + col;
+            const int nb = sv_it->blk_count;
+            constexpr int kG = kStepThreads / 32;
+            for (int b = grp; b < nb; b += 32 * kG) {
+                double v[32];
+#pragma unroll
+                for (int u = 0; u < 32; ++u) v[u] = (b + u * kG < nb) ? p[(size_t)(b + u * kG) * kNumAcc] : 0.0;
+#pragma unroll
+                for (int u = 0; u < 32; ++u) s += v[u];
+            }
+        }
+        s_part[grp][col] = s;
+    } else {
+        const int col = threadIdx.x & 31, grp = threadIdx.x >> 5;
+        double s0 = 0.0, s1 = 0.0;
+        if (col < kNumAcc) {
+            const double* p = sv_partials + (size_t)sv_it->blk_begin * kNumAcc + col;
+            const int nb = sv_it->blk_count;
+            constexpr int kG = kSolveGroups, kU = 4;
+            for (int b = grp; b < nb; b += kU * kG) {
+                double v0[kU], v1[kU];
+#pragma unroll
+                for (int u = 0; u < kU; ++u) {
+                    v0[u] = (b + u * kG < nb) ? p[(size_t)(b + u * kG) * kNumAcc] : 0.0;
+                    v1[u] = (b + 8 + u * kG < nb) ? p[(size_t)(b + 8 + u * kG) * kNumAcc] : 0.0;
+                }
+#pragma unroll
+                for (int u = 0; u < kU; ++u) { s0 += v0[u]; s1 += v1[u]; }
+            }
+        }
+        s_part[grp][col] = s0;
+        s_part[grp + 8][col] = s1;
+    }
+    __syncthreads();
+    if (threadIdx.x < kNumAcc) {
+        double s = 0.0;
+#pragma unroll
+        for (int g = 0; g < kSolveGroups; ++g) s += s_part[g][threadIdx.x];
+        s_sum[threadIdx.x] = s;
+    }
+    __syncthreads();
+    if (threadIdx.x >= 64) return;
+    const int lane = threadIdx.x;
+    const bool l0 = lane == 0;
+
+    const int iter = sv_it->iter;
+    const int n_sel = (int)(s_sum[27] + 0.5);
+    float* tr = (sv_trace && iter < sv_trace_cap) ? sv_trace + ((size_t)sv_idx * sv_trace_cap + iter) * kTraceStride : nullptr;
+    if (l0) {
+        sv_it->n_corr = n_sel;
+        if (tr) {
+            for (int k = 0; k < kTraceStride; ++k) tr[k] = 0.f;
+            tr[0] = (float)n_sel;
+            for (int k = 0; k < 6; ++k) tr[49 + k] = sv_it->T[k];
+        }
+    }
+    bool finished = false;
+    if (n_sel >= P.min_corr) {
+        if (lane < 36) {
+            const int r_ = lane / 6, c_ = lane % 6, lo = min(r_, c_), hi = max(r_, c_);
+            s_AtA[lane] = (float)s_sum[lo * 6 - (lo * (lo - 1)) / 2 + (hi - lo)];
+        } else if (lane < 42) s_AtB[lane - 36] = (float)s_sum[21 + lane - 36];
+        __builtin_amdgcn_fence(__ATOMIC_RELEASE, "wavefront");
+        __builtin_amdgcn_wave_barrier();
+        __builtin_amdgcn_fence(__ATOMIC_ACQUIRE, "wavefront");
+        {
+            float a[6], xs[6];
+#pragma unroll
+            for (int i = 0; i < 6; ++i) a[i] = lane < 6 ? s_AtA[i * 6 + lane] : (lane == 6 ? s_AtB[i] : 0.f);
+            solve6_qr_lanes(a, lane, xs);
+            if (l0) {
+#pragma unroll
+                for (int i = 0; i < 6; ++i) s_X[i] = xs[i];
+            }
+        }
+        int isDeg = 0;
+        float Tn[6] = { 0.f, 0.f, 0.f, 0.f, 0.f, 0.f };
+        if (l0) {
+            isDeg = sv_it->degenerate;
+            bool well_conditioned = false;
+            if (iter == 0) {
+                double* L = s_L;
+                double trace = 0.0;
+                LISREG_STEP_ROLL for (int i = 0; i < 6; ++i) trace += (double)s_AtA[i * 6 + i];
+                const double shift = (double)P.eig_thresh + 2e-5 * trace;
+                well_conditioned = trace > 0.0;
+                LISREG_STEP_ROLL for (int r = 0; r < 6 && well_conditioned; ++r)
+                    LISREG_STEP_ROLL for (int c = 0; c <= r; ++c) {
+                        double v = (double)s_AtA[r * 6 + c] - (r == c ? shift : 0.0);
+                        LISREG_STEP_ROLL for (int k = 0; k < c; ++k) v -= L[r * 6 + k] * L[c * 6 + k];
+                        if (r == c) { if (!(v > 0.0)) { well_conditioned = false; break; } L[r * 6 + r] = sqrt(v); }
+                        else L[r * 6 + c] = v / L[c * 6 + c];
+                    }
+            }
+            if (iter == 0 && well_conditioned) {
+                isDeg = 0;
+                LISREG_STEP_ROLL for (int i = 0; i < 36; ++i) sv_it->P[i] = (i % 7 == 0) ? 1.f : 0.f;
+            } else if (iter == 0) {
+                LISREG_STEP_ROLL for (int i = 0; i < 36; ++i) s_A[i] = s_AtA[i];
+                LISREG_STEP_CALL eigen_sym6(s_A, s_E, s_V, s_ind, s_ind + 6);
+                LISREG_STEP_ROLL for (int i = 0; i < 36; ++i) s_V2[i] = s_V[i];
+                isDeg = 0;
+                LISREG_STEP_ROLL for (int i = 5; i >= 0; --i) {
+                    if (s_E[i] < P.eig_thresh) { LISREG_STEP_ROLL for (int j = 0; j < 6; ++j) s_V2[i * 6 + j] = 0.f; isDeg = 1; }
+                    else break;
+                }
+                LISREG_STEP_ROLL for (int i = 0; i < 36; ++i) s_A[i] = s_V[i];
+                LISREG_STEP_CALL inv6_lu(s_A, s_Vi);
+                LISREG_STEP_ROLL for (int r = 0; r < 6; ++r) LISREG_STEP_ROLL for (int c = 0; c < 6; ++c) {
+                    double s = 0; LISREG_STEP_ROLL for (int m = 0; m < 6; ++m) s += (double)s_Vi[r * 6 + m] * (double)s_V2[m * 6 + c];
+                    sv_it->P[r * 6 + c] = (float)s;
+                }
+            } else if (P.emulate_shadow) {
+                LISREG_STEP_ROLL for (int i = 0; i < 36; ++i) sv_it->P[i] = 0.f;
+            }
+            if (isDeg) {
+                float X2[6];
+                for (int r = 0; r < 6; ++r) X2[r] = s_X[r];
+                LISREG_STEP_ROLL for (int r = 0; r < 6; ++r) {
+                    double s = 0; for (int m = 0; m < 6; ++m) s += (double)sv_it->P[r * 6 + m] * (double)X2[m];
+                    s_X[r] = (float)s;
+                }
+            }
+#pragma unroll
+            for (int m = 0; m < 6; ++m) { Tn[m] = sv_it->T[m] + s_X[m]; sv_it->T[m] = Tn[m]; }
+        }
+        const float ang = lane == 0 ? lane_value(Tn[2], 0) : (lane == 1 ? lane_value(Tn[1], 0) : lane_value(Tn[0], 0));
+        const float cs = cosf(ang), sn = sinf(ang);
+        const float trig[6] = { lane_value(cs, 0), lane_value(sn, 0), lane_value(cs, 1), lane_value(sn, 1), lane_value(cs, 2), lane_value(sn, 2) };
+        if (l0) write_pose_cache(sv_it, trig);
+        if (l0) {
+            const double r0 = (double)(s_X[0] * 57.29578f), r1 = (double)(s_X[1] * 57.29578f), r2 = (double)(s_X[2] * 57.29578f);
+            const double t0 = (double)(s_X[3] * 100.f), t1 = (double)(s_X[4] * 100.f), t2 = (double)(s_X[5] * 100.f);
+            const float dR = (float)sqrt(r0 * r0 + r1 * r1 + r2 * r2);
+            const float dT = (float)sqrt(t0 * t0 + t1 * t1 + t2 * t2);
+            sv_it->deltaR = dR; sv_it->deltaT = dT;
+            sv_it->degenerate = isDeg;
+            sv_it->any_solved = 1;
+            if (tr) {
+                LISREG_STEP_ROLL for (int i = 0; i < 36; ++i) tr[1 + i] = s_AtA[i];
+                for (int i = 0; i < 6; ++i) { tr[37 + i] = s_AtB[i]; tr[43 + i] = s_X[i]; tr[49 + i] = sv_it->T[i]; }
+                tr[55] = 1.f;
+            }
+            if (dR < P.conv_deg && dT < P.conv_cm && P.fixed_iters <= 0) {
+                sv_it->iters_out = iter;
+                finished = true;
+            }
+        }
+    }
+    if (l0) {
+        sv_it->iter = iter + 1;
+        if (!finished && iter + 1 >= P.bound) { sv_it->iters_out = P.bound; finished = true; }
+        if (finished) { sv_it->done = 1; atomicAdd(sv_done, 1); }
+    }
+}
diff --git a/lis-slam_amd/lisreg/__init__.py b/lis-slam_amd/lisreg/__init__.py
--- a/lis-slam_amd/lisreg/__init__.py
+++ b/lis-slam_amd/lisreg/__init__.py
@@ -21,7 +21,7 @@
     "lisreg_device_count", "lisreg_create", "lisreg_destroy", "lisreg_last_error", "lisreg_set_stream",
     "lisreg_get_stream", "lisreg_default_params", "lisreg_set_target", "lisreg_set_target_slot",
     "lisreg_target_from_classes", "lisreg_align", "lisreg_align_batch", "lisreg_batch_prepare", "lisreg_batch_run",
-    "lisreg_batch_fetch", "lisreg_stage_host_items", "lisreg_upload_cloud", "lisreg_concat_device", "lisreg_batch_result_device", "lisreg_set_option", "lisreg_get_option", "lisreg_get_counters", "lisreg_get_neighbors", "lisreg_test_fit_models", "lisreg_get_target_index", "lisreg_get_target_graph", "lisreg_get_target_cell_rows", "lisreg_keyframes_reset", "lisreg_keyframes_push", "lisreg_keyframes_target", "lisreg_get_trace",
+    "lisreg_batch_fetch", "lisreg_stage_host_items", "lisreg_upload_cloud", "lisreg_concat_device", "lisreg_batch_result_device", "lisreg_set_option", "lisreg_get_option", "lisreg_get_counters", "lisreg_get_neighbors", "lisreg_test_fit_models", "lisreg_get_target_index", "lisreg_get_target_graph", "lisreg_get_target_cell_rows", "lisreg_keyframes_reset", "lisreg_keyframes_push", "lisreg_keyframes_target", "lisreg_get_trace", "lisreg_batch_trace",
     "lisreg_set_profiling", "lisreg_get_timing", "lisreg_pose_to_matrix", "lisreg_transform_update",
     "lisreg_comm_unique_id", "lisreg_comm_init", "lisreg_gather_results", "lisreg_comm_destroy",
     "lisreg_voxel_downsample", "lisreg_voxel_downsample_multi", "lisreg_transform_cloud",
@@ -306,6 +306,7 @@
                                                   C.POINTER(C.c_float), C.POINTER(C.c_float), C.c_int]
         L.lisreg_get_counters.argtypes = [vp, C.POINTER(C.c_ulonglong), C.c_int]
         L.lisreg_get_trace.argtypes = [vp, fp, C.c_int]
+        L.lisreg_batch_trace.argtypes = [vp, fp, C.c_int]
         L.lisreg_set_profiling.argtypes = [vp, C.c_int]
         L.lisreg_get_timing.argtypes = [vp, C.POINTER(C.c_double)]
         L.lisreg_pose_to_matrix.argtypes = [fp, fp]
@@ -579,6 +580,7 @@
         st = (Stats * max(n, 1))()
         self._chk(self._L.lisreg_align_batch(self._h, n, arr, C.byref(params),
                                              T.ctypes.data_as(C.POINTER(C.c_float)), st))
+        self._n_items = n
         return T, [stats_dict(st[i]) for i in range(n)]
 
     def batch_prepare_device(self, items: list[dict], T_init: np.ndarray, params: Params):
@@ -600,6 +602,19 @@
 
     def batch_run(self):
         self._chk(self._L.lisreg_batch_run(self._h))
+
+    def batch_trace(self):
+        n = self._n_items
+        buf = np.zeros((max(n, 1) * 64, 56), np.float32)
+        while True:
+            cap = self._L.lisreg_batch_trace(self._h, buf.ctypes.data_as(C.POINTER(C.c_float)), buf.shape[0])
+            if cap == ERR_ARG and buf.shape[0] < max(n, 1) * 65536:
+                buf = np.zeros((buf.shape[0] * 8, 56), np.float32)
+                continue
+            break
+        if cap < 0:
+            self._chk(cap)
+        return buf[:n * cap].reshape(n, cap, 56).copy() if cap > 0 else None
 
     def batch_fetch(self):
         n = self._n_items
```

New measurement: 28900 registrations/s. 0.953x the previous value.
